# yang-song/score_sde_pytorch

Hardware: AMD Instinct MI355X
Metric: pc_sampler_images_per_sec (higher is better)
Workload: dtype f32 via 3-way bf16 split, fp32 accumulate (the 1x1 / NIN / Linear GEMMs and the attention forward as exact-fp32 products on the BF16 matrix pipe, fp32 softmax; 3x3 convolutions and the attention backward on the fp32-MFMA kernels); 1 GPU; configs/ve/cifar10_ncsnpp_continuous PC sampler (reverse_diffusion+langevin), batch 256/GPU, N=1000, 32x32; 1 step = 1 PC iteration = 2 U-Net evaluations; batch_per_gpu=256, sde_steps=1000, state_finite=True, matrix_mode=bf16x6, parallelism=replicas x1 (no collectives)

## Files before the change

include/ssde.h:

```cpp
#ifndef SSDE_H_
#define SSDE_H_

#include <stddef.h>
#include <stdint.h>

#ifdef __cplusplus
extern "C" {
#endif

#define SSDE_ABI_VERSION 13

enum {
  SSDE_PRO_NONE = 0,
  SSDE_PRO_GN = 1,
  SSDE_PRO_GN_SILU = 2,
  SSDE_PRO_SILU = 3
};

typedef struct ssde_src {
  const float* p0;
  const float* p1;
  int32_t c0, c1;
  int32_t pro_mode;
  int32_t gn_groups;
// ... 38 lines not shown
  int64_t wino_ws_floats;
} ssde_conv_args;

enum { SSDE_CONVF_V_GIVEN = 1u,
       SSDE_CONVF_BF16X6 = 2u,
       SSDE_CONVF_NO_KSPLIT = 4u,
       SSDE_CONVF_BKC8 = 8u,
       SSDE_CONVF_GEMM_PIPE = 16u,
       SSDE_CONVF_NO_GEMM_PIPE = 32u,
       SSDE_CONVF_X6_BM64 = 64u,
       SSDE_CONVF_X6_PF2 = 128u,
       SSDE_CONVF_NO_SMALL_COUT = 256u,
       SSDE_CONVF_X6_WIDE = 512u,
       SSDE_CONVF_X6_NO_WIDE = 1024u,
       SSDE_CONVF_KSPLIT2 = 2048u,
       SSDE_CONVF_KSPLIT4 = 4096u };
enum { SSDE_TILE_AUTO = 0, SSDE_TILE_256x64 = 1, SSDE_TILE_128x64 = 2, SSDE_TILE_64x64 = 3, SSDE_TILE_256x32 = 4,
       SSDE_TILE_WINOGRAD = 5,
       SSDE_TILE_WINOGRAD4 = 6,
       SSDE_TILE_WINOGRAD4R = 9,
       SSDE_TILE_WINOGRAD4P = 10 };

typedef struct ssde_gn_stats_args {
  const float* p0; const float* p1; int32_t c0, c1;
  int32_t n, hw, groups; float eps;
  float* mean; float* rstd;
  float* scratch;
  int32_t slices;
  uint32_t flags;
} ssde_gn_stats_args;
enum { SSDE_GNSTATF_ANY_WIDTH = 1u };

typedef struct ssde_gn_apply_args {
  ssde_src src;
  int32_t n, hw;
  float* dst;
} ssde_gn_apply_args;

typedef struct ssde_gn_apply_bwd_args {
  ssde_src src;
  const float* dy;
  int32_t n, hw;
  float* sums;
  float* dgamma; float* dbeta;
  float* scratch;
  int32_t slices; int32_t _pad0;
  float* g0; float* g1;
  int32_t acc0, acc1;
} ssde_gn_apply_bwd_args;

typedef struct ssde_gn_finalize_args {
  const float* part0; const float* part1;
  int32_t c0, c1, slices0, slices1;
  int32_t n, groups; float eps; int32_t _pad0;
  float* mean; float* rstd;
} ssde_gn_finalize_args;

#define SSDE_FIR_MAX_TAPS 16
enum {
  SSDE_FIRF_GENERAL = 1,
  SSDE_FIRF_TILED = 2
};
typedef struct ssde_upfirdn_args {
  ssde_src src;
  int32_t n, h_in, w_in, c;
  int32_t h_out, w_out;
  int32_t up, down, pad0, pad1;
  int32_t kh, kw;
  float k[16];
  float* dst;
  int32_t accumulate;
  uint32_t flags;
  float* dst2;
  const float* taps;
} ssde_upfirdn_args;

#define SSDE_ATTN_L_MAX 16384
typedef struct ssde_attn_args {
  const float* qkv; float* dst;
  int32_t n, l, c; float scale;
  uint32_t flags;
  int32_t _pad0;
} ssde_attn_args;
enum { SSDE_ATTNF_BF16X6 = 1u,
       SSDE_ATTNF_STREAM = 2u };
enum { SSDE_ATTN_ROUTE_F32 = 0, SSDE_ATTN_ROUTE_X6 = 1, SSDE_ATTN_ROUTE_STREAM = 2 };

typedef struct ssde_embed_args {
  const float* cond;
  const float* w;
  float* dst;
  int32_t n, dim, kind, _pad0;
} ssde_embed_args;

typedef struct ssde_to_nhwc_args {
  const float* src; float* dst; int32_t n, c, h, w, c_pad; float a, b;
  int32_t mode;
  const float* v;
} ssde_to_nhwc_args;
typedef struct ssde_to_nchw_args {
  const float* src; float* dst; int32_t n, c, h, w, c_src;
  int32_t mode;
  const float* v;
  float alpha;
  int32_t accumulate;
} ssde_to_nchw_args;

typedef struct ssde_bias_act_args {
  const float* src; const float* bias; float* dst;
  int64_t numel; int32_t channels; int32_t inner;
  int32_t act;
  float alpha, scale;
  int32_t grad;
  const float* ref;
} ssde_bias_act_args;

typedef struct ssde_sumsq_args {
  const float* a; const float* b; float* out_a; float* out_b; int32_t n, per;
} ssde_sumsq_args;
typedef struct ssde_randn_args {
  float* dst; int64_t numel; uint64_t seed; const int32_t* step_ptr; int32_t stream_id; int32_t _pad0;
  const uint64_t* seed_ptr;
} ssde_randn_args;
typedef struct ssde_langevin_args {
  float* x; float* x_mean; const float* grad; const float* noise;
  const float* grad_sumsq; const float* noise_sumsq;
  const float* alpha_tab; const int32_t* step_ptr;
  int32_t n, per; float snr; int32_t _pad0;
} ssde_langevin_args;
typedef struct ssde_predictor_args {
  float* x; float* x_mean; const float* score; const float* noise;
  const float* coef; const int32_t* step_ptr;
  int64_t numel;
} ssde_predictor_args;
typedef struct ssde_sample_update_args {
  const float* x; const float* y; const float* z; const float* a; const float* b; const float* c;
  float* x_mean; float* x_out; int32_t n; int32_t per;
} ssde_sample_update_args;
typedef struct ssde_fill_args {
  float* dst; const float* tab; const int32_t* step_ptr; int32_t n; int32_t _pad0;
} ssde_fill_args;
typedef struct ssde_step_inc_args { int32_t* step_ptr; int32_t delta; int32_t _pad0; } ssde_step_inc_args;
typedef struct ssde_project_args {
  float* x; float* x_mean; const float* data; const float* mask; const float* noise;
  const float* coef; const int32_t* step_ptr;
  int32_t n, c, hw;
  int32_t use_matrix;
  float M[9], invM[9];
} ssde_project_args;



typedef struct ssde_wgrad_args {
  ssde_src src;
  const float* g;
  int32_t g_ld, g_off;
  int32_t n, h_in, w_in, h_out, w_out;
  int32_t c_out;
  int32_t ksize;
  int32_t stride, pad;
  int32_t cin_store;
  int32_t transpose_out;
  int32_t splits;
  float scale;
  uint32_t flags;
  float* dw;
// ... 24 lines not shown
  uint32_t flags;
  int32_t _pad0;
} ssde_colsum_args;
enum { SSDE_COLSUMF_DEFER = 1u };

#define SSDE_FINISH_JOBS 16
typedef struct ssde_colsum_job {
  const float* part;
  float* per_sample;
  float* total; float* total2;
  int32_t n, slices, c, ps_ld, ps_off, _pad0;
} ssde_colsum_job;
typedef struct ssde_colsum_finish_args { int32_t count, _pad0; ssde_colsum_job job[SSDE_FINISH_JOBS]; } ssde_colsum_finish_args;
typedef struct ssde_gn_bwd_job {
  const float* scratch;
  float* dgamma; float* dbeta;
  int32_t rows, c;
} ssde_gn_bwd_job;
typedef struct ssde_gn_bwd_finish_args { int32_t count, _pad0; ssde_gn_bwd_job job[SSDE_FINISH_JOBS]; } ssde_gn_bwd_finish_args;

typedef struct ssde_gn_bwd_reduce_args {
  ssde_src src;
  const float* dp;
  int32_t n, hw;
  float* sums;
  float* dgamma; float* dbeta;
  float* scratch;
  int32_t slices;
  uint32_t flags;
  float* g0; float* g1;
  int32_t acc0, acc1;
  float scale; int32_t _pad1;
} ssde_gn_bwd_reduce_args;

enum { SSDE_GNBWDF_THREE_KERNELS = 1u,
       SSDE_GNBWDF_DEFER_PARAMS = 2u };

typedef struct ssde_prologue_bwd_args {
  ssde_src src;
  const float* dp;
  int32_t dp_ld, dp_off;
  int32_t n, hw;
  const float* sums;
  float scale;
  int32_t acc0, acc1;
  float* g0; float* g1;
} ssde_prologue_bwd_args;

typedef struct ssde_attn_bwd_args {
  const float* qkv;
  const float* o;
  const float* d_o;
  float* dqkv;
  float* stats;
  int32_t n, l, c; float scale;
} ssde_attn_bwd_args;

typedef struct ssde_perturb_args {
  const float* x; const float* z; const float* a; const float* s; float* dst; int32_t n, per;
} ssde_perturb_args;
typedef struct ssde_dsm_loss_args {
  const float* score; const float* z; const float* s; const float* g2;
  float* dscore;
  float* losses;
  float* loss;
  int32_t n, per; int32_t reduce_mean; int32_t likelihood_weighting;
  float grad_scale;
  int32_t _pad0;
} ssde_dsm_loss_args;

typedef struct ssde_sumsq_flat_args { const float* x; int64_t numel; float* partial; float* out; } ssde_sumsq_flat_args;
typedef struct ssde_adam_args {
  float* p; const float* g; float* m; float* v; float* ema;
  int64_t numel;
  const float* hyper;
  const float* gnorm_sq;
} ssde_adam_args;

typedef struct ssde_memset_args { void* dst; int64_t bytes; int32_t value; int32_t _pad0; } ssde_memset_args;

enum { SSDE_PACK_CONV3 = 1, SSDE_PACK_WINO3 = 2, SSDE_PACK_MATRIX = 3, SSDE_PACK_VECTOR = 4,
       SSDE_PACK_WINO4 = 5 ,
       SSDE_PACK_WINO4R = 6 ,
       SSDE_PACK_WINO4P = 7  };
typedef struct ssde_pack_desc {
  const float* src;
  const float* src2;
  float* dst;
  int32_t kind;
  int32_t cout, cin;
  int32_t cout_l, cin_l;
  int32_t flags;
  int32_t r_off, c_off;
  int64_t n;
} ssde_pack_desc;
typedef struct ssde_pack_args { const ssde_pack_desc* table; int32_t count; int32_t kind; int64_t max_n; } ssde_pack_args;
typedef struct ssde_axpy_args {
  const float* x; const float* gate; float* dst; int64_t numel; float alpha; int32_t acc;
} ssde_axpy_args;

typedef struct ssde_rk_coefs { double v[7]; } ssde_rk_coefs;
typedef struct ssde_rk_combine_args {
  const double* y; const double* k; int64_t n; int32_t terms; int32_t _pad0; ssde_rk_coefs coef; double* dst; float* dst32;
  int64_t n32;
} ssde_rk_combine_args;
typedef struct ssde_rk_error_args {
  const double* y; const double* y_new; const double* k; int64_t n; ssde_rk_coefs coef; double atol, rtol;
  double* partial; int32_t partial_len; int32_t _pad0; double* out;
} ssde_rk_error_args;
#define SSDE_RK_MAX_TERMS 12
#define SSDE_RK_MAX_ROWS 13
typedef struct ssde_rk_combine_rows_args {
  const double* y; const double* k; int64_t n; int32_t terms; int32_t _pad0; double coef[SSDE_RK_MAX_TERMS]; double* dst; float* dst32;
  int64_t n32;
} ssde_rk_combine_rows_args;
typedef struct ssde_rk_error_rows_args {
  const double* y; const double* y_new; const double* k; int64_t n; int32_t rows; int32_t pair;
  double coef[SSDE_RK_MAX_ROWS]; double coef2[SSDE_RK_MAX_ROWS]; double h_abs; double atol, rtol;
  double* partial; int32_t partial_len; int32_t _pad0; double* out;
} ssde_rk_error_rows_args;
typedef struct ssde_ode_dyn {
  float label, std;
  float a, g2;
  double* dst;
} ssde_ode_dyn;
typedef struct ssde_pf_drift_args {
  const float* x; const float* score; double* dst; int64_t numel; float a, g2;
  const ssde_ode_dyn* dyn;
} ssde_pf_drift_args;
typedef struct ssde_hutch_div_args {
  const float* gx; const float* eps; double* dst; int64_t dst_off; int32_t n; int32_t per; float a, g2;
  const ssde_ode_dyn* dyn;
} ssde_hutch_div_args;

int ssde_conv2d(const ssde_conv_args* a, void* stream);
int ssde_groupnorm_stats(const ssde_gn_stats_args* a, void* stream);
int ssde_gn_finalize(const ssde_gn_finalize_args* a, void* stream);
int ssde_gn_apply(const ssde_gn_apply_args* a, void* stream);
int ssde_gn_apply_bwd(const ssde_gn_apply_bwd_args* a, void* stream);
int ssde_conv_gn_slices(const ssde_conv_args* a);
int64_t ssde_conv_ws_floats(const ssde_conv_args* a);
int ssde_upfirdn2d(const ssde_upfirdn_args* a, void* stream);
int ssde_attention(const ssde_attn_args* a, void* stream);
int ssde_attention_route(const ssde_attn_args* a);
int ssde_embed(const ssde_embed_args* a, void* stream);
int ssde_to_nhwc(const ssde_to_nhwc_args* a, void* stream);
int ssde_to_nchw(const ssde_to_nchw_args* a, void* stream);
int ssde_fused_bias_act(const ssde_bias_act_args* a, void* stream);
int ssde_sumsq(const ssde_sumsq_args* a, void* stream);
int ssde_randn(const ssde_randn_args* a, void* stream);
int ssde_langevin_update(const ssde_langevin_args* a, void* stream);
int ssde_predictor_update(const ssde_predictor_args* a, void* stream);
int ssde_sample_update(const ssde_sample_update_args* a, void* stream);
int ssde_fill_from_table(const ssde_fill_args* a, void* stream);
int ssde_step_inc(const ssde_step_inc_args* a, void* stream);
int ssde_project_update(const ssde_project_args* a, void* stream);
int ssde_rk_combine(const ssde_rk_combine_args* a, void* stream);
int ssde_rk_error_norm(const ssde_rk_error_args* a, void* stream);
int ssde_rk_combine_rows(const ssde_rk_combine_rows_args* a, void* stream);
int ssde_rk_error_norm_rows(const ssde_rk_error_rows_args* a, void* stream);
int ssde_pf_drift(const ssde_pf_drift_args* a, void* stream);
int ssde_hutch_div(const ssde_hutch_div_args* a, void* stream);
int ssde_conv_wgrad(const ssde_wgrad_args* a, void* stream);
int ssde_wgrad_wants_winograd4(const ssde_wgrad_args* a);
int ssde_colsum(const ssde_colsum_args* a, void* stream);
int ssde_colsum_finish(const ssde_colsum_finish_args* a, void* stream);
int ssde_gn_bwd_finish(const ssde_gn_bwd_finish_args* a, void* stream);
int ssde_gn_bwd_scratch_rows(const ssde_gn_bwd_reduce_args* a);
int ssde_gn_bwd_reduce(const ssde_gn_bwd_reduce_args* a, void* stream);
int ssde_prologue_bwd(const ssde_prologue_bwd_args* a, void* stream);
int ssde_attention_bwd(const ssde_attn_bwd_args* a, void* stream);
int ssde_perturb(const ssde_perturb_args* a, void* stream);
int ssde_dsm_loss(const ssde_dsm_loss_args* a, void* stream);
int ssde_sumsq_flat(const ssde_sumsq_flat_args* a, void* stream);
int ssde_adam_clip_ema(const ssde_adam_args* a, void* stream);
int ssde_memset(const ssde_memset_args* a, void* stream);
int ssde_axpy(const ssde_axpy_args* a, void* stream);
int ssde_pack_weights(const ssde_pack_args* a, void* stream);

enum {
  SSDE_OP_CONV = 1, SSDE_OP_GN_STATS = 2, SSDE_OP_UPFIRDN = 3, SSDE_OP_ATTN = 4, SSDE_OP_EMBED = 5,
  SSDE_OP_TO_NHWC = 6, SSDE_OP_TO_NCHW = 7, SSDE_OP_BIAS_ACT = 8, SSDE_OP_SUMSQ = 9, SSDE_OP_RANDN = 10,
  SSDE_OP_LANGEVIN = 11, SSDE_OP_PREDICTOR = 12, SSDE_OP_FILL = 13, SSDE_OP_STEP_INC = 14,
  SSDE_OP_WGRAD = 15, SSDE_OP_COLSUM = 16, SSDE_OP_GN_BWD_REDUCE = 17, SSDE_OP_PROLOGUE_BWD = 18,
  SSDE_OP_ATTN_BWD = 19, SSDE_OP_PERTURB = 20, SSDE_OP_DSM_LOSS = 21, SSDE_OP_SUMSQ_FLAT = 22,
  SSDE_OP_ADAM = 23, SSDE_OP_MEMSET = 24, SSDE_OP_AXPY = 25, SSDE_OP_PACK = 26, SSDE_OP_PROJECT = 27,
  SSDE_OP_GN_FINALIZE = 28, SSDE_OP_PF_DRIFT = 29, SSDE_OP_HUTCH_DIV = 30, SSDE_OP_COLSUM_FINISH = 31, SSDE_OP_GN_BWD_FINISH = 32,
  SSDE_OP_GN_APPLY = 33, SSDE_OP_GN_APPLY_BWD = 34
};
typedef struct ssde_op {
  int32_t kind; int32_t flops_class;
  union {
    ssde_conv_args conv; ssde_gn_stats_args gn; ssde_upfirdn_args fir; ssde_attn_args attn;
    ssde_embed_args embed; ssde_to_nhwc_args to_nhwc; ssde_to_nchw_args to_nchw;
    ssde_bias_act_args bias_act; ssde_sumsq_args sumsq; ssde_randn_args randn;
    ssde_langevin_args langevin; ssde_predictor_args predictor; ssde_fill_args fill;
    ssde_step_inc_args step_inc;
    ssde_wgrad_args wgrad; ssde_colsum_args colsum; ssde_gn_bwd_reduce_args gn_bwd; ssde_prologue_bwd_args pro_bwd;
    ssde_attn_bwd_args attn_bwd; ssde_perturb_args perturb; ssde_dsm_loss_args dsm_loss;
    ssde_sumsq_flat_args sumsq_flat; ssde_adam_args adam; ssde_memset_args memset; ssde_axpy_args axpy;
    ssde_pack_args pack; ssde_project_args project; ssde_gn_finalize_args gn_fin;
    ssde_pf_drift_args pf_drift; ssde_hutch_div_args hutch_div;
    ssde_colsum_finish_args colsum_fin; ssde_gn_bwd_finish_args gn_bwd_fin;
    ssde_gn_apply_args gn_apply; ssde_gn_apply_bwd_args gn_apply_bwd;
  } u;
} ssde_op;

int ssde_program_run(const ssde_op* ops, int32_t n_ops, void* stream);
int ssde_program_run_timed(const ssde_op* ops, int32_t n_ops, void* stream, float* ms);
int ssde_graph_capture(const ssde_op* ops, int32_t n_ops, void* stream, void** graph_out);
int ssde_graph_launch(void* graph, void* stream);
int ssde_graph_destroy(void* graph);

enum { SSDE_REGION_ZERO = 0,
       SSDE_REGION_CONST = 1 };
enum { SSDE_RELOC_OP = 0, SSDE_RELOC_REFRESH_OP = 1, SSDE_RELOC_REGION = 2 };
enum { SSDE_PLAN_UNET = 0, SSDE_PLAN_PC = 1, SSDE_PLAN_TRAIN = 2,
       SSDE_PLAN_ODE = 3,
       SSDE_PLAN_LIKELIHOOD = 4 };
enum { SSDE_IO_X = 0, SSDE_IO_COND = 1, SSDE_IO_SIGMA = 2, SSDE_IO_STD = 3, SSDE_IO_OUT = 4, SSDE_IO_XMEAN = 5,
       SSDE_IO_STEP = 6, SSDE_IO_SEED = 7,
       SSDE_IO_BATCH = 8, SSDE_IO_Z = 9, SSDE_IO_A = 10, SSDE_IO_S = 11, SSDE_IO_G2 = 12, SSDE_IO_LOSS = 13, SSDE_IO_HYPER = 14,
       SSDE_IO_DROP_SEED = 15, SSDE_IO_GOUT = 16, SSDE_IO_GX = 17, SSDE_IO_GRAD = 18, SSDE_IO_PARAMS = 19,
       SSDE_IO_ODE_DYN = 20, SSDE_IO_ODE_K = 21, SSDE_IO_ODE_STATE = 22, SSDE_IO_ODE_PROBE = 23, SSDE_IO_SLOTS = 24 };
#define SSDE_ODE_PARTIALS 1024
typedef struct ssde_plan_header {
  char magic[8];
  int32_t abi_version, sizeof_op;
  int32_t n_regions, n_ops, n_refresh_ops, n_relocs, n_params;
  int32_t kind;
  int32_t batch, channels, height, width;
  int32_t nfe_per_iteration;
  int32_t sde_steps;
  int32_t io[SSDE_IO_SLOTS];
  int32_t seg[4];
  int64_t n_flat;
  int64_t data_bytes;
} ssde_plan_header;
typedef struct ssde_plan_region { int64_t bytes; int64_t data_offset; int32_t kind; int32_t _pad0; char name[32]; } ssde_plan_region;
typedef struct ssde_plan_reloc {
  int32_t target_kind;
  int32_t target;
  int64_t byte_offset;
  int32_t region; int32_t _pad0;
  int64_t offset;
} ssde_plan_reloc;
typedef struct ssde_plan_param_entry { char name[96]; int32_t region; int32_t _pad0; int64_t offset; int64_t numel; } ssde_plan_param_entry;
typedef struct ssde_plan ssde_plan;

int ssde_plan_load(const void* blob, size_t bytes, ssde_plan** out);
int ssde_plan_load_file(const char* path, ssde_plan** out);
int ssde_plan_destroy(ssde_plan* p);
int ssde_plan_info(const ssde_plan* p, ssde_plan_header* out);
int ssde_plan_param(const ssde_plan* p, const char* name, int32_t index, float** dev, int64_t* numel, const char** name_out);
int ssde_plan_refresh_weights(ssde_plan* p, void* stream);
int ssde_unet_forward(ssde_plan* p, const float* x, const float* cond, const float* sigma, const float* std_, float* out, void* stream);
int ssde_pc_reset(ssde_plan* p, const float* x_T, uint64_t seed, void* stream);
int ssde_pc_run(ssde_plan* p, int32_t n_iterations, int32_t use_graph, void* stream);
int ssde_train_step(ssde_plan* p, const float* batch, const float* z, const float* a, const float* s, const float* labels,
                    const float* g2, const float* hyper, uint32_t dropout_seed, float* loss_out, void* stream);
int ssde_train_forward(ssde_plan* p, const float* x, const float* cond, const float* sigma, const float* std_, uint32_t dropout_seed,
                       float* out, void* stream);
int ssde_unet_backward(ssde_plan* p, const float* dout, float* dx, float* dparams, void* stream);
int ssde_plan_copy_io(ssde_plan* p, int32_t slot, void* buf, int64_t bytes, int32_t to_plan, void* stream);
int ssde_pc_state(ssde_plan* p, float* x, float* x_mean, void* stream);
enum { SSDE_ODE_RK45 = 0, SSDE_ODE_RK23 = 1, SSDE_ODE_DOP853 = 2 };
typedef int (*ssde_ode_scalars_fn)(double t, void* user, float out[4]);
int ssde_ode_reset(ssde_plan* p, const float* x0, const float* probe, void* stream);
int ssde_ode_eval(ssde_plan* p, double t, ssde_ode_scalars_fn scalars, void* user, double* slope, void* stream);
int ssde_ode_solve(ssde_plan* p, double t0, double t1, double rtol, double atol, ssde_ode_scalars_fn scalars, void* user,
                   int32_t use_graph, int32_t max_nfev, int32_t* nfev, void* stream);
int ssde_ode_solve_method(ssde_plan* p, int32_t method, double t0, double t1, double rtol, double atol, ssde_ode_scalars_fn scalars,
                          void* user, int32_t use_graph, int32_t max_nfev, int32_t* nfev, void* stream);
int ssde_ode_state(ssde_plan* p, float* x, double* delta_logp, void* stream);

int ssde_abi_version(void);
int ssde_sizeof_op(void);
const char* ssde_last_error(void);
int ssde_conv_lds_bytes(const ssde_conv_args* a);
int64_t ssde_wgrad_scratch_floats(const ssde_wgrad_args* a);
int ssde_mfma_probe(int32_t workgroups, int32_t iters, float* sink, void* stream);

#ifdef __cplusplus
}
#endif
#endif
```

score_sde_pytorch_amd/_lib.py:

```python
import ctypes as C
import os

_HERE = os.path.dirname(os.path.abspath(__file__))
LIB_PATH = os.environ.get("SSDE_LIB_PATH") or os.path.join(_HERE, "libssde_hip.so")
ABI_VERSION = 13

PRO_NONE, PRO_GN, PRO_GN_SILU, PRO_SILU = 0, 1, 2, 3
TILE_AUTO, TILE_256x64, TILE_128x64, TILE_64x64, TILE_256x32, TILE_WINOGRAD, TILE_WINOGRAD4 = 0, 1, 2, 3, 4, 5, 6
TILE_WINOGRAD4R = 9
TILE_WINOGRAD4P = 10
TILES_WINOGRAD4 = (TILE_WINOGRAD4, TILE_WINOGRAD4R, TILE_WINOGRAD4P)
CONVF_V_GIVEN, CONVF_BF16X6, CONVF_NO_KSPLIT, CONVF_BKC8, CONVF_GEMM_PIPE, CONVF_NO_GEMM_PIPE, CONVF_X6_BM64, CONVF_X6_PF2, \
    CONVF_NO_SMALL_COUT, CONVF_X6_WIDE, CONVF_X6_NO_WIDE, CONVF_KSPLIT2, CONVF_KSPLIT4 = 1, 2, 4, 8, 16, 32, 64, 128, 256, 512, 1024, 2048, 4096
WGRADF_DIRECT, WGRADF_F2, WGRADF_F4_FORCE, WGRADF_NO_STREAMK, WGRADF_NO_XCD_ORDER, WGRADF_1X1_CHUNKED, WGRADF_XVEC1 = 1, 2, 4, 8, 16, 32, 64
GNBWDF_THREE_KERNELS, GNBWDF_DEFER_PARAMS = 1, 2
(OP_CONV, OP_GN_STATS, OP_UPFIRDN, OP_ATTN, OP_EMBED, OP_TO_NHWC, OP_TO_NCHW, OP_BIAS_ACT, OP_SUMSQ,
 OP_RANDN, OP_LANGEVIN, OP_PREDICTOR, OP_FILL, OP_STEP_INC, OP_WGRAD, OP_COLSUM, OP_GN_BWD_REDUCE, OP_PROLOGUE_BWD,
 OP_ATTN_BWD, OP_PERTURB, OP_DSM_LOSS, OP_SUMSQ_FLAT, OP_ADAM, OP_MEMSET, OP_AXPY, OP_PACK, OP_PROJECT,
 OP_GN_FINALIZE, OP_PF_DRIFT, OP_HUTCH_DIV, OP_COLSUM_FINISH, OP_GN_BWD_FINISH, OP_GN_APPLY, OP_GN_APPLY_BWD) = range(1, 35)
GNSTATF_ANY_WIDTH = 1
FIRF_GENERAL, FIRF_TILED = 1, 2
FIR_MAX_TAPS = 16
FINISH_JOBS = 16
COLSUMF_DEFER = 1
PACK_CONV3, PACK_WINO3, PACK_MATRIX, PACK_VECTOR, PACK_WINO4, PACK_WINO4R, PACK_WINO4P = 1, 2, 3, 4, 5, 6, 7

_fp = C.c_void_p


class Src(C.Structure):
    _fields_ = [("p0", _fp), ("p1", _fp), ("c0", C.c_int32), ("c1", C.c_int32),
                ("pro_mode", C.c_int32), ("gn_groups", C.c_int32),
                ("gn_mean", _fp), ("gn_rstd", _fp), ("gn_gamma", _fp), ("gn_beta", _fp),
                ("drop_thresh", C.c_uint32), ("drop_scale", C.c_float), ("drop_seed", _fp),
                ("drop_salt", C.c_uint32), ("_pad", C.c_int32)]


class ConvArgs(C.Structure):
    _fields_ = [("main", Src), ("aux", Src), ("w_main", _fp), ("w_aux", _fp),
                ("n", C.c_int32), ("h_in", C.c_int32), ("w_in", C.c_int32),
                ("h_out", C.c_int32), ("w_out", C.c_int32), ("c_out", C.c_int32),
                ("ksize", C.c_int32), ("stride", C.c_int32), ("pad", C.c_int32), ("tile", C.c_int32),
                ("bias", _fp), ("chan_add", _fp), ("chan_add_ld", C.c_int32), ("resid_post", C.c_int32),
                ("resid", _fp), ("out_scale", C.c_float), ("flags", C.c_uint32), ("dst", _fp), ("gn_part", _fp), ("wino_v", _fp),
                ("gn_in_part0", _fp), ("gn_in_part1", _fp), ("gn_in_slices0", C.c_int32), ("gn_in_slices1", C.c_int32),
                ("gn_in_eps", C.c_float), ("pad_end", C.c_int32), ("wino_ws", _fp), ("wino_ws_floats", C.c_int64)]


class GnStatsArgs(C.Structure):
    _fields_ = [("p0", _fp), ("p1", _fp), ("c0", C.c_int32), ("c1", C.c_int32),
                ("n", C.c_int32), ("hw", C.c_int32), ("groups", C.c_int32), ("eps", C.c_float),
                ("mean", _fp), ("rstd", _fp), ("scratch", _fp), ("slices", C.c_int32), ("flags", C.c_uint32)]


class GnApplyArgs(C.Structure):
    _fields_ = [("src", Src), ("n", C.c_int32), ("hw", C.c_int32), ("dst", _fp)]


class GnApplyBwdArgs(C.Structure):
    _fields_ = [("src", Src), ("dy", _fp), ("n", C.c_int32), ("hw", C.c_int32), ("sums", _fp), ("dgamma", _fp), ("dbeta", _fp),
                ("scratch", _fp), ("slices", C.c_int32), ("_pad0", C.c_int32), ("g0", _fp), ("g1", _fp),
                ("acc0", C.c_int32), ("acc1", C.c_int32)]


class RkCombineArgs(C.Structure):
    _fields_ = [("y", _fp), ("k", _fp), ("n", C.c_int64), ("terms", C.c_int32), ("_pad0", C.c_int32), ("coef", C.c_double * 7),
                ("dst", _fp), ("dst32", _fp), ("n32", C.c_int64)]


class RkErrorArgs(C.Structure):
    _fields_ = [("y", _fp), ("y_new", _fp), ("k", _fp), ("n", C.c_int64), ("coef", C.c_double * 7), ("atol", C.c_double),
                ("rtol", C.c_double), ("partial", _fp), ("partial_len", C.c_int32), ("_pad0", C.c_int32), ("out", _fp)]


class RkCombineRowsArgs(C.Structure):
    _fields_ = [("y", _fp), ("k", _fp), ("n", C.c_int64), ("terms", C.c_int32), ("_pad0", C.c_int32), ("coef", C.c_double * 12),
                ("dst", _fp), ("dst32", _fp), ("n32", C.c_int64)]


class RkErrorRowsArgs(C.Structure):
    _fields_ = [("y", _fp), ("y_new", _fp), ("k", _fp), ("n", C.c_int64), ("rows", C.c_int32), ("pair", C.c_int32),
                ("coef", C.c_double * 13), ("coef2", C.c_double * 13), ("h_abs", C.c_double), ("atol", C.c_double), ("rtol", C.c_double),
                ("partial", _fp), ("partial_len", C.c_int32), ("_pad0", C.c_int32), ("out", _fp)]


class PfDriftArgs(C.Structure):
    _fields_ = [("x", _fp), ("score", _fp), ("dst", _fp), ("numel", C.c_int64), ("a", C.c_float), ("g2", C.c_float), ("dyn", _fp)]


class OdeDyn(C.Structure):
    _fields_ = [("label", C.c_float), ("std", C.c_float), ("a", C.c_float), ("g2", C.c_float), ("dst", _fp)]


class HutchDivArgs(C.Structure):
    _fields_ = [("gx", _fp), ("eps", _fp), ("dst", _fp), ("dst_off", C.c_int64), ("n", C.c_int32), ("per", C.c_int32),
                ("a", C.c_float), ("g2", C.c_float), ("dyn", _fp)]


class GnFinalizeArgs(C.Structure):
    _fields_ = [("part0", _fp), ("part1", _fp), ("c0", C.c_int32), ("c1", C.c_int32), ("slices0", C.c_int32), ("slices1", C.c_int32),
                ("n", C.c_int32), ("groups", C.c_int32), ("eps", C.c_float), ("_pad0", C.c_int32), ("mean", _fp), ("rstd", _fp)]


class UpfirdnArgs(C.Structure):
    _fields_ = [("src", Src), ("n", C.c_int32), ("h_in", C.c_int32), ("w_in", C.c_int32), ("c", C.c_int32),
                ("h_out", C.c_int32), ("w_out", C.c_int32),
                ("up", C.c_int32), ("down", C.c_int32), ("pad0", C.c_int32), ("pad1", C.c_int32),
                ("kh", C.c_int32), ("kw", C.c_int32), ("k", C.c_float * 16), ("dst", _fp),
                ("accumulate", C.c_int32), ("flags", C.c_uint32), ("dst2", _fp), ("taps", _fp)]


class AttnArgs(C.Structure):
    _fields_ = [("qkv", _fp), ("dst", _fp), ("n", C.c_int32), ("l", C.c_int32), ("c", C.c_int32), ("scale", C.c_float),
                ("flags", C.c_uint32), ("_pad0", C.c_int32)]


class EmbedArgs(C.Structure):
    _fields_ = [("cond", _fp), ("w", _fp), ("dst", _fp), ("n", C.c_int32), ("dim", C.c_int32),
                ("kind", C.c_int32), ("_pad0", C.c_int32)]


class ToNhwcArgs(C.Structure):
    _fields_ = [("src", _fp), ("dst", _fp), ("n", C.c_int32), ("c", C.c_int32), ("h", C.c_int32), ("w", C.c_int32),
                ("c_pad", C.c_int32), ("a", C.c_float), ("b", C.c_float), ("mode", C.c_int32), ("v", _fp)]


class ToNchwArgs(C.Structure):
    _fields_ = [("src", _fp), ("dst", _fp), ("n", C.c_int32), ("c", C.c_int32), ("h", C.c_int32), ("w", C.c_int32),
                ("c_src", C.c_int32), ("mode", C.c_int32), ("v", _fp), ("alpha", C.c_float), ("accumulate", C.c_int32)]


class BiasActArgs(C.Structure):
    _fields_ = [("src", _fp), ("bias", _fp), ("dst", _fp), ("numel", C.c_int64), ("channels", C.c_int32),
                ("inner", C.c_int32), ("act", C.c_int32), ("alpha", C.c_float), ("scale", C.c_float), ("grad", C.c_int32),
                ("ref", _fp)]


class SumsqArgs(C.Structure):
    _fields_ = [("a", _fp), ("b", _fp), ("out_a", _fp), ("out_b", _fp), ("n", C.c_int32), ("per", C.c_int32)]


class RandnArgs(C.Structure):
    _fields_ = [("dst", _fp), ("numel", C.c_int64), ("seed", C.c_uint64), ("step_ptr", _fp),
                ("stream_id", C.c_int32), ("_pad0", C.c_int32), ("seed_ptr", _fp)]


class LangevinArgs(C.Structure):
    _fields_ = [("x", _fp), ("x_mean", _fp), ("grad", _fp), ("noise", _fp), ("grad_sumsq", _fp), ("noise_sumsq", _fp),
                ("alpha_tab", _fp), ("step_ptr", _fp), ("n", C.c_int32), ("per", C.c_int32), ("snr", C.c_float),
                ("_pad0", C.c_int32)]


class PredictorArgs(C.Structure):
    _fields_ = [("x", _fp), ("x_mean", _fp), ("score", _fp), ("noise", _fp), ("coef", _fp), ("step_ptr", _fp),
                ("numel", C.c_int64)]


class SampleUpdateArgs(C.Structure):
    _fields_ = [("x", _fp), ("y", _fp), ("z", _fp), ("a", _fp), ("b", _fp), ("c", _fp), ("x_mean", _fp), ("x_out", _fp),
                ("n", C.c_int32), ("per", C.c_int32)]


class FillArgs(C.Structure):
    _fields_ = [("dst", _fp), ("tab", _fp), ("step_ptr", _fp), ("n", C.c_int32), ("_pad0", C.c_int32)]


class StepIncArgs(C.Structure):
    _fields_ = [("step_ptr", _fp), ("delta", C.c_int32), ("_pad0", C.c_int32)]


class ProjectArgs(C.Structure):
    _fields_ = [("x", _fp), ("x_mean", _fp), ("data", _fp), ("mask", _fp), ("noise", _fp), ("coef", _fp), ("step_ptr", _fp),
                ("n", C.c_int32), ("c", C.c_int32), ("hw", C.c_int32), ("use_matrix", C.c_int32),
                ("M", C.c_float * 9), ("invM", C.c_float * 9)]


class WgradArgs(C.Structure):
    _fields_ = [("src", Src), ("g", _fp), ("g_ld", C.c_int32), ("g_off", C.c_int32),
                ("n", C.c_int32), ("h_in", C.c_int32), ("w_in", C.c_int32), ("h_out", C.c_int32), ("w_out", C.c_int32),
                ("c_out", C.c_int32), ("ksize", C.c_int32), ("stride", C.c_int32), ("pad", C.c_int32),
                ("cin_store", C.c_int32), ("transpose_out", C.c_int32), ("splits", C.c_int32), ("scale", C.c_float),
                ("flags", C.c_uint32), ("dw", _fp), ("scratch", _fp), ("scratch_floats", C.c_int64), ("v_pre", _fp),
                ("pad_end", C.c_int32), ("_pad0", C.c_int32)]


class ColsumArgs(C.Structure):
    _fields_ = [("g", _fp), ("g_ld", C.c_int32), ("g_off", C.c_int32), ("n", C.c_int32), ("hw", C.c_int32),
                ("c", C.c_int32), ("scale", C.c_float), ("per_sample", _fp), ("ps_ld", C.c_int32), ("ps_off", C.c_int32),
                ("total", _fp), ("total2", _fp), ("scratch", _fp), ("flags", C.c_uint32), ("_pad0", C.c_int32)]


class ColsumJob(C.Structure):
    _fields_ = [("part", _fp), ("per_sample", _fp), ("total", _fp), ("total2", _fp), ("n", C.c_int32), ("slices", C.c_int32),
                ("c", C.c_int32), ("ps_ld", C.c_int32), ("ps_off", C.c_int32), ("_pad0", C.c_int32)]


class ColsumFinishArgs(C.Structure):
# ... 12 lines not shown
    _fields_ = [("src", Src), ("dp", _fp), ("n", C.c_int32), ("hw", C.c_int32), ("sums", _fp),
                ("dgamma", _fp), ("dbeta", _fp), ("scratch", _fp), ("slices", C.c_int32), ("flags", C.c_uint32),
                ("g0", _fp), ("g1", _fp), ("acc0", C.c_int32), ("acc1", C.c_int32), ("scale", C.c_float), ("_pad1", C.c_int32)]


class PrologueBwdArgs(C.Structure):
    _fields_ = [("src", Src), ("dp", _fp), ("dp_ld", C.c_int32), ("dp_off", C.c_int32), ("n", C.c_int32), ("hw", C.c_int32),
                ("sums", _fp), ("scale", C.c_float), ("acc0", C.c_int32), ("acc1", C.c_int32), ("g0", _fp), ("g1", _fp)]


class AttnBwdArgs(C.Structure):
    _fields_ = [("qkv", _fp), ("o", _fp), ("d_o", _fp), ("dqkv", _fp), ("stats", _fp),
                ("n", C.c_int32), ("l", C.c_int32), ("c", C.c_int32), ("scale", C.c_float)]


class PerturbArgs(C.Structure):
    _fields_ = [("x", _fp), ("z", _fp), ("a", _fp), ("s", _fp), ("dst", _fp), ("n", C.c_int32), ("per", C.c_int32)]


class DsmLossArgs(C.Structure):
    _fields_ = [("score", _fp), ("z", _fp), ("s", _fp), ("g2", _fp), ("dscore", _fp), ("losses", _fp), ("loss", _fp),
                ("n", C.c_int32), ("per", C.c_int32), ("reduce_mean", C.c_int32), ("likelihood_weighting", C.c_int32),
                ("grad_scale", C.c_float), ("_pad0", C.c_int32)]


class SumsqFlatArgs(C.Structure):
    _fields_ = [("x", _fp), ("numel", C.c_int64), ("partial", _fp), ("out", _fp)]


class AdamArgs(C.Structure):
    _fields_ = [("p", _fp), ("g", _fp), ("m", _fp), ("v", _fp), ("ema", _fp), ("numel", C.c_int64),
                ("hyper", _fp), ("gnorm_sq", _fp)]


class MemsetArgs(C.Structure):
    _fields_ = [("dst", _fp), ("bytes", C.c_int64), ("value", C.c_int32), ("_pad0", C.c_int32)]


class AxpyArgs(C.Structure):
    _fields_ = [("x", _fp), ("gate", _fp), ("dst", _fp), ("numel", C.c_int64), ("alpha", C.c_float), ("acc", C.c_int32)]


class PackDesc(C.Structure):
    _fields_ = [("src", _fp), ("src2", _fp), ("dst", _fp), ("kind", C.c_int32), ("cout", C.c_int32), ("cin", C.c_int32),
                ("cout_l", C.c_int32), ("cin_l", C.c_int32), ("flags", C.c_int32), ("r_off", C.c_int32), ("c_off", C.c_int32),
                ("n", C.c_int64)]


class PackArgs(C.Structure):
    _fields_ = [("table", _fp), ("count", C.c_int32), ("kind", C.c_int32), ("max_n", C.c_int64)]


OPS = [(OP_CONV, "conv", ConvArgs, "ssde_conv2d"), (OP_GN_STATS, "gn", GnStatsArgs, "ssde_groupnorm_stats"),
       (OP_UPFIRDN, "fir", UpfirdnArgs, "ssde_upfirdn2d"), (OP_ATTN, "attn", AttnArgs, "ssde_attention"),
       (OP_EMBED, "embed", EmbedArgs, "ssde_embed"), (OP_TO_NHWC, "to_nhwc", ToNhwcArgs, "ssde_to_nhwc"),
       (OP_TO_NCHW, "to_nchw", ToNchwArgs, "ssde_to_nchw"), (OP_BIAS_ACT, "bias_act", BiasActArgs, "ssde_fused_bias_act"),
       (OP_SUMSQ, "sumsq", SumsqArgs, "ssde_sumsq"), (OP_RANDN, "randn", RandnArgs, "ssde_randn"),
       (OP_LANGEVIN, "langevin", LangevinArgs, "ssde_langevin_update"),
       (OP_PREDICTOR, "predictor", PredictorArgs, "ssde_predictor_update"), (OP_FILL, "fill", FillArgs, "ssde_fill_from_table"),
       (OP_STEP_INC, "step_inc", StepIncArgs, "ssde_step_inc"), (OP_WGRAD, "wgrad", WgradArgs, "ssde_conv_wgrad"),
       (OP_COLSUM, "colsum", ColsumArgs, "ssde_colsum"), (OP_GN_BWD_REDUCE, "gn_bwd", GnBwdReduceArgs, "ssde_gn_bwd_reduce"),
       (OP_PROLOGUE_BWD, "pro_bwd", PrologueBwdArgs, "ssde_prologue_bwd"), (OP_ATTN_BWD, "attn_bwd", AttnBwdArgs, "ssde_attention_bwd"),
       (OP_PERTURB, "perturb", PerturbArgs, "ssde_perturb"), (OP_DSM_LOSS, "dsm_loss", DsmLossArgs, "ssde_dsm_loss"),
       (OP_SUMSQ_FLAT, "sumsq_flat", SumsqFlatArgs, "ssde_sumsq_flat"), (OP_ADAM, "adam", AdamArgs, "ssde_adam_clip_ema"),
       (OP_MEMSET, "memset", MemsetArgs, "ssde_memset"), (OP_AXPY, "axpy", AxpyArgs, "ssde_axpy"),
       (OP_PACK, "pack", PackArgs, "ssde_pack_weights"), (OP_PROJECT, "project", ProjectArgs, "ssde_project_update"),
       (OP_GN_FINALIZE, "gn_fin", GnFinalizeArgs, "ssde_gn_finalize"), (OP_PF_DRIFT, "pf_drift", PfDriftArgs, "ssde_pf_drift"),
       (OP_HUTCH_DIV, "hutch_div", HutchDivArgs, "ssde_hutch_div"), (OP_COLSUM_FINISH, "colsum_fin", ColsumFinishArgs, "ssde_colsum_finish"),
       (OP_GN_BWD_FINISH, "gn_bwd_fin", GnBwdFinishArgs, "ssde_gn_bwd_finish"), (OP_GN_APPLY, "gn_apply", GnApplyArgs, "ssde_gn_apply"),
       (OP_GN_APPLY_BWD, "gn_apply_bwd", GnApplyBwdArgs, "ssde_gn_apply_bwd")]


class _OpUnion(C.Union):
    _fields_ = [(member, args) for _, member, args, _ in OPS]


class Op(C.Structure):
    _fields_ = [("kind", C.c_int32), ("flops_class", C.c_int32), ("u", _OpUnion)]


_UNION_FIELD = {kind: member for kind, member, _, _ in OPS}
ARGS = {kind: args for kind, _, args, _ in OPS}

EXPORTS = ["ssde_conv2d", "ssde_groupnorm_stats", "ssde_upfirdn2d", "ssde_attention", "ssde_attention_route", "ssde_embed", "ssde_to_nhwc",
           "ssde_to_nchw", "ssde_fused_bias_act", "ssde_sumsq", "ssde_randn", "ssde_langevin_update",
           "ssde_predictor_update", "ssde_fill_from_table", "ssde_step_inc", "ssde_program_run",
           "ssde_program_run_timed", "ssde_graph_capture", "ssde_graph_launch", "ssde_graph_destroy",
           "ssde_abi_version", "ssde_sizeof_op", "ssde_last_error", "ssde_conv_lds_bytes",
           "ssde_conv_wgrad", "ssde_colsum", "ssde_gn_bwd_reduce", "ssde_prologue_bwd", "ssde_attention_bwd",
           "ssde_perturb", "ssde_dsm_loss", "ssde_sumsq_flat", "ssde_adam_clip_ema", "ssde_memset", "ssde_axpy",
           "ssde_wgrad_scratch_floats", "ssde_wgrad_wants_winograd4", "ssde_pack_weights", "ssde_project_update", "ssde_gn_finalize", "ssde_conv_gn_slices", "ssde_conv_ws_floats", "ssde_rk_combine", "ssde_rk_error_norm", "ssde_rk_combine_rows", "ssde_rk_error_norm_rows", "ssde_pf_drift", "ssde_hutch_div", "ssde_sample_update", "ssde_mfma_probe", "ssde_colsum_finish", "ssde_gn_bwd_finish", "ssde_gn_bwd_scratch_rows",
           "ssde_gn_apply", "ssde_gn_apply_bwd",
           "ssde_plan_load", "ssde_plan_load_file", "ssde_plan_destroy", "ssde_plan_info", "ssde_plan_param",
           "ssde_plan_refresh_weights", "ssde_unet_forward", "ssde_pc_reset", "ssde_pc_run", "ssde_pc_state",
           "ssde_train_step", "ssde_train_forward", "ssde_unet_backward", "ssde_plan_copy_io",
           "ssde_ode_reset", "ssde_ode_eval", "ssde_ode_solve", "ssde_ode_solve_method", "ssde_ode_state"]

_lib = None


def conv_route_flags(env=None):
    e = os.environ if env is None else env
    f = 0
    if e.get("SSDE_MATRIX", "").startswith("b"):
        f |= CONVF_BF16X6
    if e.get("SSDE_CONV_KSPLIT", "1") == "0":
        f |= CONVF_NO_KSPLIT
    if e.get("SSDE_CONV_BKC64", "") == "8":
        f |= CONVF_BKC8
    if e.get("SSDE_GEMM_PIPE", "") == "0":
        f |= CONVF_NO_GEMM_PIPE
    if e.get("SSDE_GEMM_PIPE", "") == "2":
        f |= CONVF_GEMM_PIPE
    if e.get("SSDE_X6_BM", "") == "64":
        f |= CONVF_X6_BM64
    if e.get("SSDE_X6_PF", "") == "2":
        f |= CONVF_X6_PF2
    if e.get("SSDE_CONV_SMALL", "1") == "0":
        f |= CONVF_NO_SMALL_COUT
    if e.get("SSDE_X6_WIDE", "") == "1":
        f |= CONVF_X6_WIDE
    if e.get("SSDE_X6_WIDE", "") == "0":
        f |= CONVF_X6_NO_WIDE
    return f


ATTNF_BF16X6, ATTNF_STREAM = 1, 2
ATTN_ROUTE_F32, ATTN_ROUTE_X6, ATTN_ROUTE_STREAM = 0, 1, 2
ATTN_L_MAX = 16384


def attn_route_flags(env=None):
    e = os.environ if env is None else env
    x6 = ATTNF_BF16X6 if e.get("SSDE_MATRIX", "").startswith("b") and e.get("SSDE_ATTN_X6", "1") != "0" else 0
    return x6 | (ATTNF_STREAM if e.get("SSDE_ATTN_STREAM", "0") == "1" else 0)


def wgrad_route_flags(env=None):
    e = os.environ if env is None else env
    f = {"0": WGRADF_DIRECT, "2": WGRADF_F2, "44": WGRADF_F4_FORCE}.get(e.get("SSDE_WGRAD_WINOGRAD", ""), 0)
    if e.get("SSDE_WGRAD4_STREAMK", "1") == "0":
        f |= WGRADF_NO_STREAMK
    if e.get("SSDE_WGRAD4_XCD", "1") == "0":
        f |= WGRADF_NO_XCD_ORDER
    if e.get("SSDE_WGRAD_1X1_PIPELINED", "1") == "0":
        f |= WGRADF_1X1_CHUNKED
    if e.get("SSDE_WGRAD4_XVEC", "2") == "1":
        f |= WGRADF_XVEC1
    return f


def gn_bwd_route_flags(env=None):
    e = os.environ if env is None else env
    return GNBWDF_THREE_KERNELS if e.get("SSDE_GN_BWD_FUSED", "1") == "0" else 0


class SsdeError(RuntimeError):
    pass


def bind(lib):
    for name in EXPORTS:
        if not hasattr(lib, name):
            raise SsdeError("libssde_hip.so does not export %s" % name)
    lib.ssde_last_error.restype = C.c_char_p
    lib.ssde_program_run.argtypes = [C.POINTER(Op), C.c_int32, C.c_void_p]
    lib.ssde_program_run_timed.argtypes = [C.POINTER(Op), C.c_int32, C.c_void_p, C.POINTER(C.c_float)]
    lib.ssde_graph_capture.argtypes = [C.POINTER(Op), C.c_int32, C.c_void_p, C.POINTER(C.c_void_p)]
    lib.ssde_graph_launch.argtypes = [C.c_void_p, C.c_void_p]
    lib.ssde_graph_destroy.argtypes = [C.c_void_p]
    for _, _, typ, name in OPS:
        if name is not None:
            getattr(lib, name).argtypes = [C.POINTER(typ), C.c_void_p]
    lib.ssde_rk_combine.argtypes = [C.POINTER(RkCombineArgs), C.c_void_p]
    lib.ssde_rk_error_norm.argtypes = [C.POINTER(RkErrorArgs), C.c_void_p]
    lib.ssde_rk_combine_rows.argtypes = [C.POINTER(RkCombineRowsArgs), C.c_void_p]
    lib.ssde_rk_error_norm_rows.argtypes = [C.POINTER(RkErrorRowsArgs), C.c_void_p]
    lib.ssde_sample_update.argtypes = [C.POINTER(SampleUpdateArgs), C.c_void_p]
    lib.ssde_conv_lds_bytes.argtypes = [C.POINTER(ConvArgs)]
    lib.ssde_attention_route.argtypes = [C.POINTER(AttnArgs)]
    lib.ssde_conv_gn_slices.argtypes = [C.POINTER(ConvArgs)]
    lib.ssde_conv_ws_floats.argtypes = [C.POINTER(ConvArgs)]
    lib.ssde_conv_ws_floats.restype = C.c_int64
    lib.ssde_wgrad_scratch_floats.argtypes = [C.POINTER(WgradArgs)]
    lib.ssde_wgrad_scratch_floats.restype = C.c_int64
    lib.ssde_wgrad_wants_winograd4.argtypes = [C.POINTER(WgradArgs)]
    lib.ssde_gn_bwd_scratch_rows.argtypes = [C.POINTER(GnBwdReduceArgs)]
    if lib.ssde_abi_version() != ABI_VERSION:
        raise SsdeError("ABI mismatch: library %d, binding %d" % (lib.ssde_abi_version(), ABI_VERSION))
    if lib.ssde_sizeof_op() != C.sizeof(Op):
        raise SsdeError("struct layout mismatch: sizeof(ssde_op) library %d, ctypes %d" % (lib.ssde_sizeof_op(), C.sizeof(Op)))
    return lib


def load():
    global _lib
    if _lib is not None:
        return _lib
    if not os.path.exists(LIB_PATH):
        raise SsdeError(
            "libssde_hip.so not found at %s -- build it with `python -c 'import __graft_entry__ as g; g.build()'` "
            "(score_sde_pytorch_amd has no CPU/eager fallback)" % LIB_PATH)
    lib = bind(C.CDLL(LIB_PATH))
    _lib = lib
    return lib


def check(rc, what=""):
    if rc != 0:
        msg = load().ssde_last_error()
        raise SsdeError("%s failed (%d): %s" % (what or "libssde_hip call", rc, msg.decode() if msg else "?"))


def pointer_offsets(struct_cls, base=0):
    out = []
    for name, typ in struct_cls._fields_:
        off = base + getattr(struct_cls, name).offset
        if typ is C.c_void_p:
            out.append(off)
        elif isinstance(typ, type) and issubclass(typ, C.Structure):
            out.extend(pointer_offsets(typ, off))
        elif isinstance(typ, type) and issubclass(typ, C.Array) and issubclass(typ._type_, C.Structure):
            for i in range(typ._length_):
                out.extend(pointer_offsets(typ._type_, off + i * C.sizeof(typ._type_)))
    return out


_OP_PTRS = {}


def _op_pointer_offsets(kind):
    if kind not in _OP_PTRS:
        _OP_PTRS[kind] = pointer_offsets(ARGS[kind], Op.u.offset)
    return _OP_PTRS[kind]


def pointers_at(raw, offsets, base=0):
    for off in offsets:
        addr = int.from_bytes(raw[base + off:base + off + 8], "little")
        if addr:
            yield base + off, addr


def op_pointers(op):
    return pointers_at(bytes(op), _op_pointer_offsets(int(op.kind)))


def make_op(kind, args, flops_class=0):
    op = Op()
    op.kind = kind
    op.flops_class = flops_class
    setattr(op.u, _UNION_FIELD[kind], args)
    return op


def make(kind, **fields):
    args = ARGS[kind]()
    for k, v in fields.items():
        if isinstance(v, (list, tuple)):
            v = (C.c_float * len(v))(*v)
        setattr(args, k, v.data_ptr() if hasattr(v, "data_ptr") else v)
    return make_op(kind, args)

# ... 7 lines not shown
```

score_sde_pytorch_amd/csrc/attention.hip:

```cpp
#include "ssde_common.h"
#include <type_traits>

typedef float f32x16 __attribute__((ext_vector_type(16)));

namespace {

constexpr int kQB = 64;
constexpr int kLMax = 256;
constexpr int kKB = kLMax;
constexpr int kLDC = 36;
constexpr int kLDP = 260;
constexpr int kTileFloats = kQB * kLDP;
constexpr int kStageFloats = (kQB + kLMax) * kLDC;
constexpr int kFwdVch = 8;
constexpr int kAttnLdsFloats = kQB * kLDP + kFwdVch * kLDP;
constexpr int kBwdLdsFloats = kTileFloats + kStageFloats + 3 * kLMax;

__device__ __forceinline__ void zero_acc(f32x16 (&acc)[2][2]) {
#pragma unroll
  for (int a = 0; a < 2; ++a)
#pragma unroll
    for (int b = 0; b < 2; ++b)
#pragma unroll
      for (int r = 0; r < 16; ++r) acc[a][b][r] = 0.f;
// ... 131 lines not shown
}

__device__ __forceinline__ void store_acc(const f32x16 (&acc)[2][2], float* __restrict__ out, size_t ldo, int out_valid, int cp, int C,
                                          float mul) {
  const int wave = threadIdx.x >> 6, lane = threadIdx.x & 63;
  const int li = lane & 31, lh = lane >> 5;
#pragma unroll
  for (int a = 0; a < 2; ++a)
#pragma unroll
    for (int b = 0; b < 2; ++b) {
      const int col = acc_col(cp + wave * 64, b, li);
      if (col >= C) continue;
#pragma unroll
      for (int r = 0; r < 16; ++r) {
        const int row = acc_row(a, r, lh);
        if (row < out_valid) out[(size_t)row * ldo + col] = acc[a][b][r] * mul;
      }
    }
}

template <int VCH = 32>
__device__ __forceinline__ void gemm_pv(const float* Ps, int Lp, const float* __restrict__ Bm, int b_valid, size_t ldb, int C,
                                        float* Vs, float* __restrict__ out, size_t ldo, int out_valid, float out_scale) {
  f32x16 acc[2][2];
  for (int cp = 0; cp < C; cp += 256) {
    zero_acc(acc);
    pv_pass<VCH>(Ps, Lp, Bm, b_valid, ldb, cp, min(256, C - cp), Vs, acc);
    store_acc(acc, out, ldo, out_valid, cp, C, out_scale);
  }
}

__device__ __forceinline__ void acc_to_tile(const f32x16 (&acc)[2][2], float* Ps, int Lk, float mul) {
  const int wave = threadIdx.x >> 6, lane = threadIdx.x & 63;
  const int li = lane & 31, lh = lane >> 5, kb = wave * 64;
  if (kb < Lk) {
#pragma unroll
    for (int a = 0; a < 2; ++a)
#pragma unroll
      for (int b = 0; b < 2; ++b)
#pragma unroll
        for (int r = 0; r < 16; ++r) {
          const int row = acc_row(a, r, lh), col = acc_col(kb, b, li);
          Ps[row * kLDP + col] = acc[a][b][r] * mul;
        }
  }
}

template <bool kWriteP>
__device__ __forceinline__ float online_softmax(float* Ps, int Lb, float& m_run, float& l_run) {
  const int tid = threadIdx.x;
  const int row = tid >> 2, sub = tid & 3;
  float* prow = Ps + row * kLDP;
  float m = -INFINITY;
  for (int j = sub; j < Lb; j += 4) m = fmaxf(m, prow[j]);
  m = fmaxf(m, __shfl_xor(m, 1, 64));
  m = fmaxf(m, __shfl_xor(m, 2, 64));
  m = fmaxf(m, m_run);
  const float alpha = __expf(m_run - m);
  float sum = 0.f;
  for (int j = sub; j < Lb; j += 4) {
    const float e = __expf(prow[j] - m);
    if (kWriteP) prow[j] = e;
    sum += e;
  }
  sum += __shfl_xor(sum, 1, 64);
  sum += __shfl_xor(sum, 2, 64);
  if (kWriteP) {
    const int Lp = (Lb + 31) & ~31;
    for (int j = Lb + sub; j < Lp; j += 4) prow[j] = 0.f;
  }
  l_run = l_run * alpha + sum;
  m_run = m;
  return alpha;
}

__device__ __forceinline__ void softmax_rows(float* Ps, int L, float& m, float& l) {
  m = -INFINITY; l = 0.f;
  online_softmax<true>(Ps, L, m, l);
  float* prow = Ps + (threadIdx.x >> 2) * kLDP;
  const float inv = 1.0f / l;
  for (int j = threadIdx.x & 3; j < L; j += 4) prow[j] *= inv;
}

__global__ __launch_bounds__(256) void attn_kernel(const float* __restrict__ qkv, float* __restrict__ dst,
                                                   int N, int L, int C, float scale) {
  SSDE_LDS(smem);
  float* Qs = smem;
  float* Ks = smem + kQB * kLDC;
  float* Ps = smem;
  float* Vs = smem + kQB * kLDP;
  const int n = blockIdx.y, q0 = blockIdx.x * kQB;
  const int C3 = 3 * C;
  const float* base = qkv + (size_t)n * L * C3;
  const int Lk = (L + 63) & ~63;
  const int Lp = (L + 31) & ~31;

  f32x16 acc[2][2];
  gemm_nt(base + (size_t)q0 * C3, L - q0, C3, base + C, L, C3, C, Lk, Qs, Ks, acc);
  __syncthreads();
  acc_to_tile(acc, Ps, Lk, scale);
  __syncthreads();
  float m, l;
  softmax_rows(Ps, L, m, l);
  gemm_pv<kFwdVch>(Ps, Lp, base + 2 * C, L, C3, C, Vs, dst + ((size_t)n * L + q0) * C, C, L - q0, 1.0f);
}

namespace x6 {
constexpr int kT = 512, kRows = 64, kL = 256;
constexpr int kKStage = 3 * kL * 32;
constexpr int kPPlane = kL * kRows * 2;
constexpr int kMain = 3 * kPPlane;
constexpr int kLds = kMain + 2 * kKStage;
static_assert(kRows * kLDP * 4 <= kMain, "score tile");

__device__ __forceinline__ void split_hi(float x, uint32_t& a, uint32_t& b, uint32_t& c) {
  a = __builtin_bit_cast(uint32_t, x);
  const float r = x - __builtin_bit_cast(float, a & 0xffff0000u);
  b = __builtin_bit_cast(uint32_t, r);
  c = __builtin_bit_cast(uint32_t, r - __builtin_bit_cast(float, b & 0xffff0000u));
}
}

template <int kNst>
__global__ __launch_bounds__(x6::kT) void attn_x6_kernel(const float* __restrict__ qkv, float* __restrict__ dst, int N, float scale) {
  using namespace x6;
  constexpr int C = 16 * kNst;
  SSDE_LDS(smem);
  char* lds = reinterpret_cast<char*>(smem);
  char* stage0 = lds + kMain;
  char* stage1 = stage0 + kKStage;
  const int tid = threadIdx.x, lane = tid & 63;
  const int wave = __builtin_amdgcn_readfirstlane(tid >> 6);
  const int li = lane & 31, lh = lane >> 5;
  const int xcd = blockIdx.x & 7, k_in = blockIdx.x >> 3;
  const int n = (k_in >> 2) * 8 + xcd, q0 = (k_in & 3) * kRows;
  if (n >= N) return;
  const int C3 = 3 * C;
  const float* base = qkv + (size_t)n * kL * C3;
  const int qplane = C * kRows * 2;
  constexpr int nst = kNst;

  const bool consumer = wave < 4;
  f32x16 acc[2][2];
  auto zero = [&]() {
#pragma unroll
    for (int a = 0; a < 2; ++a)
#pragma unroll
      for (int b = 0; b < 2; ++b)
#pragma unroll
        for (int r = 0; r < 16; ++r) acc[a][b][r] = 0.f;
  };
  struct Frags { ssde_u32x4 A[2][3], B[2][3]; };
  auto read_frags = [&](Frags& f, const char* ap, int a_pitch, const char* bp, int b_pitch) __attribute__((always_inline)) {
#pragma unroll
    for (int q = 0; q < 3; ++q) {
#pragma unroll
      for (int a = 0; a < 2; ++a) f.A[a][q] = *reinterpret_cast<const ssde_u32x4*>(ap + q * a_pitch + (a * 32 + li) * 32 + lh * 16);
#pragma unroll
      for (int b = 0; b < 2; ++b) f.B[b][q] = *reinterpret_cast<const ssde_u32x4*>(bp + q * b_pitch + (wave * 64 + b * 32 + li) * 32 + lh * 16);
    }
  };
  auto mfmas = [&](auto Terms, const Frags& f) __attribute__((always_inline)) {
    constexpr int kTerms = decltype(Terms)::value;
    constexpr int TI[8] = {1, 2, 0, 2, 1, 0, 1, 0}, TJ[8] = {2, 1, 2, 0, 1, 1, 0, 0};
#pragma unroll
    for (int t = 8 - kTerms; t < 8; ++t)
#pragma unroll
      for (int a = 0; a < 2; ++a)
#pragma unroll
        for (int b = 0; b < 2; ++b)
          acc[a][b] = __builtin_amdgcn_mfma_f32_32x32x16_bf16(__builtin_bit_cast(ssde_bf16x8, f.A[a][TI[t]]),
                                                              __builtin_bit_cast(ssde_bf16x8, f.B[b][TJ[t]]), acc[a][b], 0, 0, 0);
  };
  using Six = std::integral_constant<int, 6>;
  using Eight = std::integral_constant<int, 8>;

  const int ptid = tid & 255;
  const float* kbase = base + C;
  const float* vbase = base + 2 * C;
  const int krow = ptid >> 2, kf = ptid & 3;
  const uint32_t koff = (uint32_t)((krow * C3 + kf * 4) * 4), kstep = (uint32_t)(64 * C3 * 4);
  const int tp = ptid & 7, fq0 = ptid >> 3;
  const bool v_on0 = fq0 * 4 < C, v_on1 = (fq0 + 32) * 4 < C;
  const uint32_t voff = (uint32_t)((2 * tp * C3 + (v_on0 ? fq0 * 4 : 0)) * 4), vtok = (uint32_t)(C3 * 4), vquad = v_on1 ? 512u : 0u;
  const int vpitch = C * 32;
  auto request = [&](int u, ssde_f32x4 (&Rs)[4]) __attribute__((always_inline)) {
    const bool is_k = u < nst;
    const float* sb = is_k ? kbase + u * 16 : vbase + (size_t)(u - nst) * 16 * C3;
    const uint32_t o0 = is_k ? koff : voff;
    const uint32_t o1 = o0 + (is_k ? kstep : vtok);
    const uint32_t o2 = is_k ? o0 + 2 * kstep : o0 + vquad;
    const uint32_t o3 = is_k ? o0 + 3 * kstep : o2 + vtok;
    SSDE_GLOAD16_I_SAFE(Rs[0], o0, sb, 0);
    SSDE_GLOAD16_I_SAFE(Rs[1], o1, sb, 0);
    SSDE_GLOAD16_I_SAFE(Rs[2], o2, sb, 0);
    SSDE_GLOAD16_I_SAFE(Rs[3], o3, sb, 0);
  };
#ifdef SSDE_EMULATED
#define SSDE_X6_WAIT(n, Rs) ((void)0)
#else
#define SSDE_X6_WAIT(n, Rs) asm volatile("s_waitcnt vmcnt(%4)" : "+v"((Rs)[0]), "+v"((Rs)[1]), "+v"((Rs)[2]), "+v"((Rs)[3]) : "n"(n) : "memory")
#endif
  auto park_k = [&](const ssde_f32x4 (&Rs)[4], char* buf) __attribute__((always_inline)) {
#pragma unroll
    for (int i = 0; i < 4; ++i) {
      uint2 p0, p1, p2;
      ssde_split3(make_float4(Rs[i].x, Rs[i].y, Rs[i].z, Rs[i].w), p0, p1, p2);
// ... 68 lines not shown
  if (consumer) {
    SSDE_LDS_BARRIER();
    for (int u = 0; u < nst; ++u) {
      Frags f;
      read_frags(f, lds + u * (kRows * 32), qplane, (u & 1) ? stage1 : stage0, kL * 32);
      mfmas(Eight{}, f);
      SSDE_LDS_BARRIER();
    }
  } else {
    SSDE_X6_WAIT(12, R[0]);
    park_k(R[0], stage0);
    SSDE_LDS_BARRIER();
#pragma unroll
    for (int u = 0; u < nst; ++u) {
      const int j = u & 3;
      request(u + 4, R[j]);
      SSDE_X6_WAIT(12, R[(j + 1) & 3]);
      if (u + 1 < nst) park_k(R[(j + 1) & 3], (j & 1) ? stage0 : stage1);
      SSDE_LDS_BARRIER();
    }
    SSDE_X6_WAIT(8, R[1]); SSDE_X6_WAIT(4, R[2]); SSDE_X6_WAIT(0, R[3]);
  }

  {
    float* tile = smem;
    if (consumer) {
#pragma unroll
      for (int a = 0; a < 2; ++a)
#pragma unroll
        for (int b = 0; b < 2; ++b)
#pragma unroll
          for (int r = 0; r < 16; ++r) {
            const int row = a * 32 + (r & 3) + 8 * (r >> 2) + 4 * lh;
            tile[row * kLDP + wave * 64 + b * 32 + li] = acc[a][b][r] * scale;
          }
    }
    SSDE_LDS_BARRIER();
    const int row = tid >> 3, sub = tid & 7;
    float x[32];
#pragma unroll
    for (int i = 0; i < 8; ++i) {
      const float4 v = *reinterpret_cast<const float4*>(tile + row * kLDP + sub * 32 + i * 4);
      x[4 * i] = v.x; x[4 * i + 1] = v.y; x[4 * i + 2] = v.z; x[4 * i + 3] = v.w;
    }
    SSDE_LDS_BARRIER();
    float m = x[0];
#pragma unroll
    for (int i = 1; i < 32; ++i) m = fmaxf(m, x[i]);
    m = fmaxf(m, __shfl_xor(m, 1, 64));
    m = fmaxf(m, __shfl_xor(m, 2, 64));
    m = fmaxf(m, __shfl_xor(m, 4, 64));
    float sum = 0.f;
#pragma unroll
    for (int i = 0; i < 32; ++i) { x[i] = __expf(x[i] - m); sum += x[i]; }
    sum += __shfl_xor(sum, 1, 64);
    sum += __shfl_xor(sum, 2, 64);
    sum += __shfl_xor(sum, 4, 64);
    const float inv = 1.0f / sum;
#pragma unroll
    for (int u = 0; u < 4; ++u) {
      uint2 a0, a1, a2, b0, b1, b2;
      ssde_split3(make_float4(x[8 * u] * inv, x[8 * u + 1] * inv, x[8 * u + 2] * inv, x[8 * u + 3] * inv), a0, a1, a2);
      ssde_split3(make_float4(x[8 * u + 4] * inv, x[8 * u + 5] * inv, x[8 * u + 6] * inv, x[8 * u + 7] * inv), b0, b1, b2);
      char* d = lds + (2 * sub + (u >> 1)) * (kRows * 32) + row * 32 + (u & 1) * 16;
      *reinterpret_cast<uint4*>(d) = make_uint4(a0.x, a0.y, b0.x, b0.y);
      *reinterpret_cast<uint4*>(d + kPPlane) = make_uint4(a1.x, a1.y, b1.x, b1.y);
      *reinterpret_cast<uint4*>(d + 2 * kPPlane) = make_uint4(a2.x, a2.y, b2.x, b2.y);
    }
  }

  if (consumer) {
    const bool w_on = wave * 64 < C;
    zero();
    SSDE_LDS_BARRIER();
    for (int v = 0; v < 16; ++v) {
      if (w_on) {
        Frags f;
        read_frags(f, lds + v * (kRows * 32), kPPlane, (v & 1) ? stage1 : stage0, vpitch);
        mfmas(Six{}, f);
      }
      SSDE_LDS_BARRIER();
    }
    if (w_on) {
#pragma unroll
      for (int b = 0; b < 2; ++b) {
        float* out = dst + ((size_t)n * kL + q0) * C + wave * 64 + b * 32 + li;
#pragma unroll
        for (int a = 0; a < 2; ++a)
#pragma unroll
          for (int r = 0; r < 16; ++r) {
            const int row = a * 32 + (r & 3) + 8 * (r >> 2) + 4 * lh;
            out[(size_t)row * C] = acc[a][b][r];
          }
      }
    }
  } else {
    park_v(R[0], stage0);
    SSDE_LDS_BARRIER();
#pragma unroll
    for (int v = 0; v < 16; ++v) {
      const int j = v & 3;
      if (v + 4 < 16) request(nst + v + 4, R[j]);
      if (v + 1 < 16) {
        if (v + 1 >= 4) {
          if (v + 4 < 16) SSDE_X6_WAIT(12, R[(j + 1) & 3]);
          else if (v + 3 < 16) SSDE_X6_WAIT(8, R[(j + 1) & 3]);
          else if (v + 2 < 16) SSDE_X6_WAIT(4, R[(j + 1) & 3]);
          else SSDE_X6_WAIT(0, R[(j + 1) & 3]);
        }
        park_v(R[(j + 1) & 3], (j & 1) ? stage0 : stage1);
      }
      SSDE_LDS_BARRIER();
    }
  }
#undef SSDE_X6_WAIT
}


__device__ __forceinline__ float row_dot(const float* __restrict__ o, const float* __restrict__ d_o, size_t first, int C, int valid) {
  const int row = threadIdx.x >> 2, sub = threadIdx.x & 3;
  float d = 0.f;
  if (row < valid) {
    const float* po = o + (first + row) * C;
    const float* pd = d_o + (first + row) * C;
    for (int c = sub * 4; c < C; c += 16) {
      const float4 a = *reinterpret_cast<const float4*>(po + c);
      const float4 b = *reinterpret_cast<const float4*>(pd + c);
      d += (a.x * b.x + a.y * b.y) + (a.z * b.z + a.w * b.w);
    }
  }
  d += __shfl_xor(d, 1, 64);
  d += __shfl_xor(d, 2, 64);
  return d;
}

__device__ __forceinline__ void load_stats(float* St, const float* __restrict__ stats, size_t first, int count) {
  const int j = threadIdx.x;
  float m = 0.f, l = 1.f, d = 0.f;
  if (j < count) { const float* st = stats + (first + j) * 4; m = st[0]; l = st[1]; d = st[2]; }
  St[j] = m; St[kKB + j] = l; St[2 * kKB + j] = d;
}

template <bool kRowStats>
__device__ __forceinline__ void acc_to_probs(const f32x16 (&acc)[2][2], float* Ps, const float* St, int Lk, int rows_valid, int cols_valid,
                                             float scale) {
  const int wave = threadIdx.x >> 6, lane = threadIdx.x & 63;
  const int li = lane & 31, lh = lane >> 5, kb = wave * 64;
  if (kb < Lk) {
#pragma unroll
    for (int a = 0; a < 2; ++a)
#pragma unroll
      for (int b = 0; b < 2; ++b)
#pragma unroll
        for (int r = 0; r < 16; ++r) {
          const int row = acc_row(a, r, lh), col = acc_col(kb, b, li);
          const int s = kRowStats ? row : col;
          float pv = 0.f;
          if (row < rows_valid && col < cols_valid) pv = __expf(acc[a][b][r] * scale - St[s]) / St[kKB + s];
          Ps[row * kLDP + col] = pv;
        }
  }
}

template <bool kRowStats>
__device__ __forceinline__ void probs_to_ds(const f32x16 (&acc)[2][2], float* Ps, const float* St, int Lk, int Lp) {
  const int wave = threadIdx.x >> 6, lane = threadIdx.x & 63;
  const int li = lane & 31, lh = lane >> 5, kb = wave * 64;
  if (kb < Lk) {
#pragma unroll
    for (int a = 0; a < 2; ++a)
#pragma unroll
      for (int b = 0; b < 2; ++b)
#pragma unroll
        for (int r = 0; r < 16; ++r) {
          const int row = acc_row(a, r, lh), col = acc_col(kb, b, li);
          if (col < Lp) Ps[row * kLDP + col] *= (acc[a][b][r] - St[2 * kKB + (kRowStats ? row : col)]);
        }
  }
}

__global__ __launch_bounds__(256) void attn_bwd_q_kernel(const float* __restrict__ qkv, const float* __restrict__ o,
                                                         const float* __restrict__ d_o, float* __restrict__ dqkv,
                                                         float* __restrict__ stats, int N, int L, int C, float scale) {
  SSDE_LDS(smem);
  float* Ps = smem;
  float* Qs = smem + kTileFloats;
  float* Ks = Qs + kQB * kLDC;
  float* Vs = Qs;
  float* St = smem + kTileFloats + kStageFloats;
  const int n = blockIdx.y, q0 = blockIdx.x * kQB, tid = threadIdx.x;
  const int C3 = 3 * C;
  const float* base = qkv + (size_t)n * L * C3;
  const int Lk = (L + 63) & ~63, Lp = (L + 31) & ~31;
  const int valid = L - q0;

  f32x16 acc[2][2];
  gemm_nt(base + (size_t)q0 * C3, valid, C3, base + C, L, C3, C, Lk, Qs, Ks, acc);
  __syncthreads();
// ... 130 lines not shown
template <int NCP>
__global__ __launch_bounds__(256) void attn_stream_bwd_q_kernel(const float* __restrict__ qkv, const float* __restrict__ d_o,
                                                                float* __restrict__ dqkv, const float* __restrict__ stats,
                                                                int N, int L, int C, float scale) {
  SSDE_LDS(smem);
  float* Ps = smem;
  float* Qs = smem + kTileFloats;
  float* Ks = Qs + kQB * kLDC;
  float* Vs = Qs;
  float* St = smem + kTileFloats + kStageFloats;
  const int n = blockIdx.y, q0 = blockIdx.x * kQB, tid = threadIdx.x;
  const int C3 = 3 * C;
  const float* base = qkv + (size_t)n * L * C3;
  const int valid = L - q0;
  if (tid < kQB) load_stats(St, stats, (size_t)n * L + q0, valid);
  f32x16 dq[NCP][2][2];
#pragma unroll
  for (int p = 0; p < NCP; ++p) zero_acc(dq[p]);
  for (int kb0 = 0; kb0 < L; kb0 += kKB) {
    const int Lb = min(kKB, L - kb0);
    const int Lk = (Lb + 63) & ~63, Lp = (Lb + 31) & ~31;
    f32x16 acc[2][2];
    gemm_nt(base + (size_t)q0 * C3, valid, C3, base + (size_t)kb0 * C3 + C, Lb, C3, C, Lk, Qs, Ks, acc);
    __syncthreads();
    acc_to_probs<true>(acc, Ps, St, Lk, valid, Lb, scale);
    gemm_nt(d_o + ((size_t)n * L + q0) * C, valid, C, base + (size_t)kb0 * C3 + 2 * C, Lb, C3, C, Lk, Qs, Ks, acc);
    __syncthreads();
    probs_to_ds<true>(acc, Ps, St, Lk, Lp);
#pragma unroll
    for (int p = 0; p < NCP; ++p)
      if (p * 256 < C) pv_pass<32>(Ps, Lp, base + (size_t)kb0 * C3 + C, Lb, C3, p * 256, min(256, C - p * 256), Vs, dq[p]);
  }
#pragma unroll
  for (int p = 0; p < NCP; ++p)
    if (p * 256 < C) store_acc(dq[p], dqkv + ((size_t)n * L + q0) * C3, C3, valid, p * 256, C, scale);
}

__global__ __launch_bounds__(256) void attn_stream_bwd_kv_kernel(const float* __restrict__ qkv, const float* __restrict__ d_o,
                                                                 float* __restrict__ dqkv, const float* __restrict__ stats,
                                                                 int N, int L, int C, float scale) {
  SSDE_LDS(smem);
  float* Ps = smem;
  float* Qs = smem + kTileFloats;
  float* Ks = Qs + kQB * kLDC;
  float* Vs = Qs;
  float* St = smem + kTileFloats + kStageFloats;
  const int n = blockIdx.y, k0 = blockIdx.x * kQB;
  const int cp = blockIdx.z * 256, Cw = min(256, C - cp);
  const int C3 = 3 * C;
  const float* base = qkv + (size_t)n * L * C3;
  const float* dob = d_o + (size_t)n * L * C;
  const int valid = L - k0;
  f32x16 dv[2][2], dk[2][2];
  zero_acc(dv);
  zero_acc(dk);
  for (int qb0 = 0; qb0 < L; qb0 += kKB) {
    const int Lb = min(kKB, L - qb0);
    const int Lk = (Lb + 63) & ~63, Lp = (Lb + 31) & ~31;
    __syncthreads();
    load_stats(St, stats, (size_t)n * L + qb0, Lb);
    f32x16 acc[2][2];
    gemm_nt(base + (size_t)k0 * C3 + C, valid, C3, base + (size_t)qb0 * C3, Lb, C3, C, Lk, Qs, Ks, acc);
    __syncthreads();
    acc_to_probs<false>(acc, Ps, St, Lk, valid, Lb, scale);
    pv_pass<32>(Ps, Lp, dob + (size_t)qb0 * C, Lb, C, cp, Cw, Vs, dv);
    gemm_nt(base + (size_t)k0 * C3 + 2 * C, valid, C3, dob + (size_t)qb0 * C, Lb, C, C, Lk, Qs, Ks, acc);
    __syncthreads();
    probs_to_ds<false>(acc, Ps, St, Lk, Lp);
    pv_pass<32>(Ps, Lp, base + (size_t)qb0 * C3, Lb, C3, cp, Cw, Vs, dk);
  }
  float* out = dqkv + ((size_t)n * L + k0) * C3;
  store_acc(dv, out + 2 * C, C3, valid, cp, C, 1.0f);
  store_acc(dk, out + C, C3, valid, cp, C, scale);
}

int check_shape(const char* what, int n, int l, int c) {
  SSDE_REQUIRE(n > 0 && l > 0 && l <= SSDE_ATTN_L_MAX, "%s: token count %d outside 1..%d", what, l, SSDE_ATTN_L_MAX);
  SSDE_REQUIRE(c > 0 && c % 32 == 0, "%s: channels must be a multiple of 32 (got %d)", what, c);
  return SSDE_OK;
}

}

static int attn_route(const ssde_attn_args* a) {
  SSDE_REQUIRE(a, "attention: null args");
  if (int rc = check_shape("attention", a->n, a->l, a->c)) return rc;
  if (a->l > kLMax || (a->flags & SSDE_ATTNF_STREAM)) {
    SSDE_REQUIRE(a->c <= kStreamCMax, "attention: the streaming kernels (more than %d tokens, or SSDE_ATTNF_STREAM) take at most %d channels (got %d)",
                 kLMax, kStreamCMax, a->c);
    return SSDE_ATTN_ROUTE_STREAM;
  }
  if ((a->flags & SSDE_ATTNF_BF16X6) && a->l == x6::kL && a->c <= 256 && a->c % 64 == 0) return SSDE_ATTN_ROUTE_X6;
  return SSDE_ATTN_ROUTE_F32;
}

extern "C" int ssde_attention_route(const ssde_attn_args* a) { return attn_route(a); }

extern "C" int ssde_attention(const ssde_attn_args* a, void* stream) {
  SSDE_REQUIRE(a && a->qkv && a->dst, "attention: null args");
  const int route = attn_route(a);
  if (route < 0) return route;
  hipStream_t st = static_cast<hipStream_t>(stream);
  const dim3 grid(ssde_cdiv(a->l, kQB), a->n);
  if (route == SSDE_ATTN_ROUTE_STREAM) {
    if (a->c <= 256) return ssde_launch_lds<attn_stream_kernel<1>>("attention", grid, 256, kStreamLdsFloats * 4, st, a->qkv, a->dst, a->n, a->l, a->c, a->scale);
    return ssde_launch_lds<attn_stream_kernel<2>>("attention", grid, 256, kStreamLdsFloats * 4, st, a->qkv, a->dst, a->n, a->l, a->c, a->scale);
  }
  if (route == SSDE_ATTN_ROUTE_X6) {
    const dim3 grid_x6(ssde_cdiv(a->n, 8) * 8 * 4);
    switch (a->c) {
      case 64: return ssde_launch_lds<attn_x6_kernel<4>>("attention", grid_x6, x6::kT, x6::kLds, st, a->qkv, a->dst, a->n, a->scale);
      case 128: return ssde_launch_lds<attn_x6_kernel<8>>("attention", grid_x6, x6::kT, x6::kLds, st, a->qkv, a->dst, a->n, a->scale);
      case 192: return ssde_launch_lds<attn_x6_kernel<12>>("attention", grid_x6, x6::kT, x6::kLds, st, a->qkv, a->dst, a->n, a->scale);
      default: return ssde_launch_lds<attn_x6_kernel<16>>("attention", grid_x6, x6::kT, x6::kLds, st, a->qkv, a->dst, a->n, a->scale);
    }
  }
  return ssde_launch_lds<attn_kernel>("attention", grid, 256, kAttnLdsFloats * 4, st, a->qkv, a->dst, a->n, a->l, a->c, a->scale);
}

extern "C" int ssde_attention_bwd(const ssde_attn_bwd_args* a, void* stream) {
  SSDE_REQUIRE(a && a->qkv && a->o && a->d_o && a->dqkv && a->stats, "attention_bwd: null args");
  if (int rc = check_shape("attention_bwd", a->n, a->l, a->c)) return rc;
  hipStream_t st = static_cast<hipStream_t>(stream);
  const dim3 grid(ssde_cdiv(a->l, kQB), a->n);
  const int lds = kBwdLdsFloats * 4;
  if (a->l > kLMax) {
    SSDE_REQUIRE(a->c <= kStreamCMax, "attention_bwd: the streaming kernels (more than %d tokens) take at most %d channels (got %d)", kLMax,
                 kStreamCMax, a->c);
    if (int rc = ssde_launch_lds<attn_stream_stats_kernel>("attention_bwd", grid, 256, kStreamLdsFloats * 4, st, a->qkv, a->o, a->d_o, a->stats, a->n, a->l,
                            a->c, a->scale))
      return rc;
    if (int rc = a->c <= 256 ? ssde_launch_lds<attn_stream_bwd_q_kernel<1>>("attention_bwd", grid, 256, lds, st, a->qkv, a->d_o, a->dqkv, a->stats, a->n, a->l, a->c, a->scale)
                             : ssde_launch_lds<attn_stream_bwd_q_kernel<2>>("attention_bwd", grid, 256, lds, st, a->qkv, a->d_o, a->dqkv, a->stats, a->n, a->l, a->c, a->scale))
      return rc;
    return ssde_launch_lds<attn_stream_bwd_kv_kernel>("attention_bwd", dim3(grid.x, grid.y, ssde_cdiv(a->c, 256)), 256, lds, st, a->qkv, a->d_o, a->dqkv,
                      a->stats, a->n, a->l, a->c, a->scale);
  }
  if (int rc = ssde_launch_lds<attn_bwd_q_kernel>("attention_bwd", grid, 256, lds, st, a->qkv, a->o, a->d_o, a->dqkv, a->stats, a->n, a->l, a->c, a->scale)) return rc;
  return ssde_launch_lds<attn_bwd_kv_kernel>("attention_bwd", grid, 256, lds, st, a->qkv, a->d_o, a->dqkv, a->stats, a->n, a->l, a->c, a->scale);
}
```

score_sde_pytorch_amd/csrc/backward.hip:

```cpp
#include "ssde_common.h"

namespace {

inline unsigned grid_for(size_t total, int block = 256, unsigned cap = 256 * 16) {
  size_t b = (total + block - 1) / block;
  if (b < 1) b = 1;
  return (unsigned)(b > cap ? cap : b);
}

__global__ __launch_bounds__(256) void colsum_kernel(const float* __restrict__ g, int g_ld, int g_off, int hw, int c,
                                                     float scale, float* __restrict__ out, int out_ld, int out_off) {
  SSDE_LDS(smem);
  float4* red = reinterpret_cast<float4*>(smem);
  const int n = blockIdx.z, slices = gridDim.y, slice = blockIdx.y;
  const int cl = blockIdx.x * 64 + (threadIdx.x & 63);
  const int pl = threadIdx.x >> 6;
  const int col = g_off + cl * 4;
  const int per_slice = (hw + slices - 1) / slices;
  const int p0 = slice * per_slice, p1 = min(hw, p0 + per_slice);
  float4 s = make_float4(0.f, 0.f, 0.f, 0.f);
  if (cl * 4 < c && col + 4 <= g_ld) {
    const float* base = g + (size_t)n * hw * g_ld + col;
    int px = p0 + pl;
    for (; px + 12 < p1; px += 16) {
// ... 819 lines not shown
      for (int k = 0; k < 3; ++k)
#pragma unroll
        for (int l = 0; l < 3; ++l) w[k][l] = pack_w3(d, co, ci, k, l);
#pragma unroll
      for (int pa = 0; pa < 4; ++pa)
#pragma unroll
        for (int pb = 0; pb < 4; ++pb) {
          float acc = 0.f;
#pragma unroll
          for (int k = 0; k < 3; ++k) {
            float t = 0.f;
#pragma unroll
            for (int l = 0; l < 3; ++l) t += w[k][l] * G[pb][l];
            acc += G[pa][k] * t;
          }
          u[e][pa * 4 + pb] = acc;
        }
    }
#pragma unroll
    for (int pos = 0; pos < 16; ++pos)
      *reinterpret_cast<float2*>(d.dst + ((((r * 16 + pos) * 4 + q) * 64 + cs) << 1)) = make_float2(u[0][pos], u[1][pos]);
  }
}

template <int kForm>
__global__ __launch_bounds__(256) void pack_wino4_kernel(const ssde_pack_desc* __restrict__ table) {
  const ssde_pack_desc d = table[blockIdx.y];
  const int ntl = (d.cout_l + 63) / 64;
  const size_t nq = (size_t)d.n / ((size_t)36 * ntl * 256);
  const double G[6][3] = {{0.25, 0.0, 0.0}, {-1.0 / 6, -1.0 / 6, -1.0 / 6}, {-1.0 / 6, 1.0 / 6, -1.0 / 6},
                          {1.0 / 24, 1.0 / 12, 1.0 / 6}, {1.0 / 24, -1.0 / 12, 1.0 / 6}, {0.0, 0.0, 1.0}};
  const size_t items = (size_t)d.n / 36;
  for (size_t it = (size_t)blockIdx.x * 256 + threadIdx.x; it < items; it += (size_t)gridDim.x * 256) {
    const int e = (int)(it & 3), cs = (int)((it >> 2) & 63);
    const size_t r = it >> 8;
    const int nt = (int)(r % ntl), c4 = (int)(r / ntl);
    const int co = nt * 64 + cs, ci = c4 * 4 + e;
    double w[3][3], t[6][3];
#pragma unroll
    for (int k = 0; k < 3; ++k)
#pragma unroll
      for (int l = 0; l < 3; ++l) w[k][l] = (double)pack_w3(d, co, ci, k, l);
#pragma unroll
    for (int a = 0; a < 6; ++a)
#pragma unroll
      for (int l = 0; l < 3; ++l) t[a][l] = G[a][0] * w[0][l] + G[a][1] * w[1][l] + G[a][2] * w[2][l];
#pragma unroll
    for (int a = 0; a < 6; ++a)
#pragma unroll
      for (int b = 0; b < 6; ++b)
      {
        const int pos = a * 6 + b, wv = (pos & 3) * 2 + (cs >> 5), j = pos >> 2;
        const float u = (float)(t[a][0] * G[b][0] + t[a][1] * G[b][1] + t[a][2] * G[b][2]);
        if (kForm == 0) {
          d.dst[(((r * 8 + wv) * 9 + j) * 32 + (cs & 31)) * 4 + e] = u;
        } else if (kForm == 2) {
          d.dst[(((size_t)pos * nq + c4) * ((size_t)ntl * 64) + co) * 4 + e] = u;
        } else {
          const int lane = (e >> 1) * 32 + (cs & 31), half = cs >> 5;
          const int w = pos < 32 ? (pos >> 2) : 2 * (pos - 32) + half;
          const size_t base = (r * 8 + w) * (size_t)(9 * 32 * 4);
          d.dst[base + (pos < 32 ? ((pos & 3) * 64 + lane) * 4 + half * 2 + (e & 1) : 1024 + lane * 2 + (e & 1))] = u;
        }
      }
  }
}

__global__ __launch_bounds__(256) void pack_matrix_kernel(const ssde_pack_desc* __restrict__ table) {
  const ssde_pack_desc d = table[blockIdx.y];
  const int ld = (d.cout_l + 63) / 64 * 64;
  for (size_t idx = (size_t)blockIdx.x * 256 + threadIdx.x; idx < (size_t)d.n; idx += (size_t)gridDim.x * 256) {
    const int i = (int)(idx / d.cin), j = (int)(idx % d.cin);
    const int row = ((d.flags & 1) ? j : i) + d.r_off, col = ((d.flags & 1) ? i : j) + d.c_off;
    d.dst[((size_t)(col >> 3) * ld + row) * 8 + (col & 7)] = d.src[idx];
  }
}

__global__ __launch_bounds__(256) void pack_vector_kernel(const ssde_pack_desc* __restrict__ table) {
  const ssde_pack_desc d = table[blockIdx.y];
  for (size_t idx = (size_t)blockIdx.x * 256 + threadIdx.x; idx < (size_t)d.n; idx += (size_t)gridDim.x * 256)
    d.dst[d.r_off + idx] = d.src[idx] + (d.src2 ? d.src2[idx] : 0.f);
}

}

extern "C" int ssde_pack_weights(const ssde_pack_args* a, void* stream) {
  SSDE_REQUIRE(a && a->table && a->count > 0 && a->max_n > 0, "pack_weights: bad args");
  size_t bx = ((size_t)a->max_n + 255) / 256;
  if (bx > 256) bx = 256;
  const dim3 grid((unsigned)bx, (unsigned)a->count);
  hipStream_t st = static_cast<hipStream_t>(stream);
  switch (a->kind) {
    case SSDE_PACK_CONV3: hipLaunchKernelGGL(pack_conv3_kernel, grid, dim3(256), 0, st, a->table); break;
    case SSDE_PACK_WINO3: hipLaunchKernelGGL(pack_wino3_kernel, grid, dim3(256), 0, st, a->table); break;
    case SSDE_PACK_WINO4: hipLaunchKernelGGL(pack_wino4_kernel<0>, grid, dim3(256), 0, st, a->table); break;
    case SSDE_PACK_WINO4R: hipLaunchKernelGGL(pack_wino4_kernel<1>, grid, dim3(256), 0, st, a->table); break;
    case SSDE_PACK_WINO4P: hipLaunchKernelGGL(pack_wino4_kernel<2>, grid, dim3(256), 0, st, a->table); break;
    case SSDE_PACK_MATRIX: hipLaunchKernelGGL(pack_matrix_kernel, grid, dim3(256), 0, st, a->table); break;
    case SSDE_PACK_VECTOR: hipLaunchKernelGGL(pack_vector_kernel, grid, dim3(256), 0, st, a->table); break;
    default: ssde_set_error("pack_weights: unknown kind %d", a->kind); return SSDE_EINVAL;
  }
  SSDE_LAUNCH_CHECK();
  return SSDE_OK;
}
```

score_sde_pytorch_amd/csrc/runtime.hip:

```cpp
#include "ssde_common.h"
#include <string.h>
#include <vector>

static thread_local char g_err[512] = "";

void ssde_set_error(const char* fmt, ...) {
  va_list ap;
  va_start(ap, fmt);
  vsnprintf(g_err, sizeof(g_err), fmt, ap);
  va_end(ap);
}

extern "C" const char* ssde_last_error(void) { return g_err; }

int ssde_num_cus() {
  if (const char* e = getenv("SSDE_NUM_CUS")) { const int v = atoi(e); if (v > 0) return v; }
  constexpr int kMaxDev = 64;
  static std::atomic<int> cus[kMaxDev];
  int dev = 0;
  if (hipGetDevice(&dev) != hipSuccess || dev < 0 || dev >= kMaxDev) dev = 0;
  int c = cus[dev].load(std::memory_order_relaxed);
  if (c <= 0) {
    int v = 0;
    if (hipDeviceGetAttribute(&v, hipDeviceAttributeMultiprocessorCount, dev) != hipSuccess || v <= 0) v = 256;
    cus[dev].store(c = v, std::memory_order_relaxed);
  }
  return c;
}
extern "C" int ssde_abi_version(void) { return SSDE_ABI_VERSION; }
extern "C" int ssde_sizeof_op(void) { return (int)sizeof(ssde_op); }

typedef float probe_f32x16 __attribute__((ext_vector_type(16)));
__global__ __launch_bounds__(256) void mfma_probe_kernel(int iters, float* sink) {
  probe_f32x16 acc[8];
#pragma unroll
  for (int j = 0; j < 8; ++j)
#pragma unroll
    for (int r = 0; r < 16; ++r) acc[j][r] = 0.f;
  const float a = 1.0f + (float)(threadIdx.x & 7) * 0.125f, b = 0.5f;
  for (int i = 0; i < iters; ++i) {
#pragma unroll
    for (int j = 0; j < 8; ++j) acc[j] = __builtin_amdgcn_mfma_f32_32x32x2f32(a, b, acc[j], 0, 0, 0);
  }
  float t = 0.f;
#pragma unroll
  for (int j = 0; j < 8; ++j) t += acc[j][0];
  if (t == -1.f) sink[threadIdx.x & 63] = t;
}

extern "C" int ssde_mfma_probe(int32_t workgroups, int32_t iters, float* sink, void* stream) {
  SSDE_REQUIRE(workgroups > 0 && iters > 0 && sink, "mfma_probe: bad args");
  hipLaunchKernelGGL(mfma_probe_kernel, dim3(workgroups), dim3(256), 0, static_cast<hipStream_t>(stream), iters, sink);
  SSDE_LAUNCH_CHECK();
  return SSDE_OK;
}

static int run_one(const ssde_op& op, void* stream) {
  switch (op.kind) {
    case SSDE_OP_CONV: return ssde_conv2d(&op.u.conv, stream);
    case SSDE_OP_GN_STATS: return ssde_groupnorm_stats(&op.u.gn, stream);
    case SSDE_OP_UPFIRDN: return ssde_upfirdn2d(&op.u.fir, stream);
    case SSDE_OP_ATTN: return ssde_attention(&op.u.attn, stream);
    case SSDE_OP_EMBED: return ssde_embed(&op.u.embed, stream);
    case SSDE_OP_TO_NHWC: return ssde_to_nhwc(&op.u.to_nhwc, stream);
    case SSDE_OP_TO_NCHW: return ssde_to_nchw(&op.u.to_nchw, stream);
    case SSDE_OP_BIAS_ACT: return ssde_fused_bias_act(&op.u.bias_act, stream);
    case SSDE_OP_SUMSQ: return ssde_sumsq(&op.u.sumsq, stream);
    case SSDE_OP_RANDN: return ssde_randn(&op.u.randn, stream);
    case SSDE_OP_LANGEVIN: return ssde_langevin_update(&op.u.langevin, stream);
    case SSDE_OP_PROJECT: return ssde_project_update(&op.u.project, stream);
    case SSDE_OP_PREDICTOR: return ssde_predictor_update(&op.u.predictor, stream);
    case SSDE_OP_FILL: return ssde_fill_from_table(&op.u.fill, stream);
    case SSDE_OP_STEP_INC: return ssde_step_inc(&op.u.step_inc, stream);
    case SSDE_OP_WGRAD: return ssde_conv_wgrad(&op.u.wgrad, stream);
    case SSDE_OP_COLSUM: return ssde_colsum(&op.u.colsum, stream);
    case SSDE_OP_GN_BWD_REDUCE: return ssde_gn_bwd_reduce(&op.u.gn_bwd, stream);
    case SSDE_OP_PROLOGUE_BWD: return ssde_prologue_bwd(&op.u.pro_bwd, stream);
    case SSDE_OP_ATTN_BWD: return ssde_attention_bwd(&op.u.attn_bwd, stream);
    case SSDE_OP_PERTURB: return ssde_perturb(&op.u.perturb, stream);
    case SSDE_OP_DSM_LOSS: return ssde_dsm_loss(&op.u.dsm_loss, stream);
    case SSDE_OP_SUMSQ_FLAT: return ssde_sumsq_flat(&op.u.sumsq_flat, stream);
    case SSDE_OP_ADAM: return ssde_adam_clip_ema(&op.u.adam, stream);
    case SSDE_OP_MEMSET: return ssde_memset(&op.u.memset, stream);
    case SSDE_OP_AXPY: return ssde_axpy(&op.u.axpy, stream);
    case SSDE_OP_PACK: return ssde_pack_weights(&op.u.pack, stream);
    case SSDE_OP_GN_FINALIZE: return ssde_gn_finalize(&op.u.gn_fin, stream);
    case SSDE_OP_PF_DRIFT: return ssde_pf_drift(&op.u.pf_drift, stream);
    case SSDE_OP_HUTCH_DIV: return ssde_hutch_div(&op.u.hutch_div, stream);
    case SSDE_OP_COLSUM_FINISH: return ssde_colsum_finish(&op.u.colsum_fin, stream);
    case SSDE_OP_GN_BWD_FINISH: return ssde_gn_bwd_finish(&op.u.gn_bwd_fin, stream);
    case SSDE_OP_GN_APPLY: return ssde_gn_apply(&op.u.gn_apply, stream);
    case SSDE_OP_GN_APPLY_BWD: return ssde_gn_apply_bwd(&op.u.gn_apply_bwd, stream);
  }
  ssde_set_error("program: unknown op kind %d", op.kind);
  return SSDE_EINVAL;
}

extern "C" int ssde_program_run(const ssde_op* ops, int32_t n_ops, void* stream) {
  SSDE_REQUIRE(ops && n_ops >= 0, "program: null ops");
  for (int i = 0; i < n_ops; ++i) {
    if (int rc = run_one(ops[i], stream)) {
      char tmp[400];
      strncpy(tmp, g_err, sizeof(tmp) - 1); tmp[sizeof(tmp) - 1] = 0;
      ssde_set_error("op %d (kind %d): %s", i, ops[i].kind, tmp);
      return rc;
    }
  }
  return SSDE_OK;
}

extern "C" int ssde_program_run_timed(const ssde_op* ops, int32_t n_ops, void* stream, float* ms) {
  SSDE_REQUIRE(ops && n_ops >= 0 && ms, "program: null args");
  hipStream_t st = static_cast<hipStream_t>(stream);
  std::vector<hipEvent_t> ev(n_ops + 1);
  for (auto& e : ev) SSDE_HIP_CHECK(hipEventCreate(&e));
  int rc = SSDE_OK;
  SSDE_HIP_CHECK(hipEventRecord(ev[0], st));
  for (int i = 0; i < n_ops && rc == SSDE_OK; ++i) {
    rc = run_one(ops[i], stream);
    if (rc == SSDE_OK && hipEventRecord(ev[i + 1], st) != hipSuccess) { ssde_set_error("hipEventRecord failed"); rc = SSDE_EHIP; }
  }
  if (rc == SSDE_OK) {
    if (hipStreamSynchronize(st) != hipSuccess) { ssde_set_error("hipStreamSynchronize failed"); rc = SSDE_EHIP; }
    for (int i = 0; i < n_ops && rc == SSDE_OK; ++i)
      if (hipEventElapsedTime(&ms[i], ev[i], ev[i + 1]) != hipSuccess) { ssde_set_error("hipEventElapsedTime failed"); rc = SSDE_EHIP; }
  }
  for (auto& e : ev) hipEventDestroy(e);
  return rc;
}

struct SsdeGraph { hipGraph_t graph; hipGraphExec_t exec; };

extern "C" int ssde_graph_capture(const ssde_op* ops, int32_t n_ops, void* stream, void** graph_out) {
  SSDE_REQUIRE(ops && graph_out, "graph: null args");
  hipStream_t st = static_cast<hipStream_t>(stream);
  SSDE_REQUIRE(st != nullptr, "graph: capture needs a non-default stream");
  SSDE_HIP_CHECK(hipStreamBeginCapture(st, hipStreamCaptureModeThreadLocal));
  int rc = ssde_program_run(ops, n_ops, stream);
  hipGraph_t graph = nullptr;
  hipError_t e = hipStreamEndCapture(st, &graph);
  if (rc != SSDE_OK) { if (graph) hipGraphDestroy(graph); return rc; }
  if (e != hipSuccess) { ssde_set_error("hipStreamEndCapture failed: %s", hipGetErrorString(e)); return SSDE_EHIP; }
  hipGraphExec_t exec = nullptr;
  e = hipGraphInstantiate(&exec, graph, nullptr, nullptr, 0);
  if (e != hipSuccess) { hipGraphDestroy(graph); ssde_set_error("hipGraphInstantiate failed: %s", hipGetErrorString(e)); return SSDE_EHIP; }
// ... 21 lines not shown
```

score_sde_pytorch_amd/engine.py:

```python
import ctypes as C
import math
import os
from typing import Callable, NamedTuple

import numpy as np
import torch

from . import _lib as L

_FLT = 4
INV_SQRT2 = float(1.0 / np.sqrt(2.0))

FC_OTHER, FC_CONV3, FC_CONV1, FC_ATTN, FC_GN, FC_FIR = 0, 1, 2, 3, 4, 5

W4P_MIN_BATCH = 16


class Buf:
    __slots__ = ("shape", "numel", "name", "persistent", "tensor", "first", "last")

    def __init__(self, shape, name="", persistent=False):
        self.shape = tuple(int(s) for s in shape)
        self.numel = int(np.prod(self.shape))
        self.name = name
# ... 368 lines not shown
    def __init__(self, device):
        self.device = device
        self.entries = []
        self.meta = {}
        self._tables = None

    def add(self, sources, fn, meta=None, recipe=None):
        lazy = recipe is not None and self._on_device() and os.environ.get("SSDE_TORCH_PACK", "0") != "1"
        with torch.no_grad():
            if lazy:
                try:
                    shape = fn(*[torch.empty(s.shape, dtype=s.dtype, device="meta") for s in sources]).shape
                except Exception:
                    shape = fn(*[torch.zeros(s.shape, dtype=s.dtype) for s in sources]).shape
                packed = torch.zeros(tuple(shape), dtype=torch.float32, device=self.device)
            else:
                packed = fn(*[s.detach() for s in sources]).to(self.device).contiguous()
        self.entries.append(_Entry(packed, list(sources), fn, None if lazy else self._stamp(sources), recipe))
        if meta is not None:
            self.meta[id(packed)] = meta
        self._tables = None
        return packed

    def _on_device(self):
        return self.device.type == "cuda" if isinstance(self.device, torch.device) else str(self.device).startswith("cuda")

    def conv3(self, param, cin_pad=None, cout_pad=None, route=DIRECT):
        def logical(w):
            w = w.to(torch.float32)
            if cin_pad and w.shape[1] < cin_pad:
                w = torch.nn.functional.pad(w, (0, 0, 0, 0, 0, cin_pad - w.shape[1]))
            if cout_pad and w.shape[0] < cout_pad:
                w = torch.nn.functional.pad(w, (0, 0, 0, 0, 0, 0, 0, cout_pad - w.shape[0]))
            return w
        cout_l, cin_l = max(param.shape[0], cout_pad or 0), max(param.shape[1], cin_pad or 0)
        meta = dict(kind="conv3", sources=[param], logical=logical, dims=(cout_l, cin_l),
                    parts=[dict(param=param, row0=0, rows=param.shape[0], transpose=False)], cin_store=param.shape[1])
        recipe = [dict(kind=route.pack_kind, src=param, cout=param.shape[0], cin=param.shape[1], cout_l=cout_l, cin_l=cin_l, flags=0, n="dst")]
        return self.add([param], lambda w: route.pack(logical(w)), meta, recipe)

    def matrix(self, parts, cin_pad=None):
        params = [p for p, _ in parts]

        def logical(*ws):
            ms = []
            for w, (_, tr) in zip(ws, parts):
                w = w.to(torch.float32)
                w = w.t() if tr else w.reshape(w.shape[0], -1)
                ms.append(w)
            m = torch.cat(ms, dim=0) if len(ms) > 1 else ms[0]
            if cin_pad and m.shape[1] < cin_pad:
                m = torch.nn.functional.pad(m, (0, cin_pad - m.shape[1]))
            return m
        rows, desc = 0, []
        for p_, tr in parts:
            n_rows = p_.shape[1] if tr else p_.shape[0]
            cin = p_.shape[0] if tr else int(np.prod(p_.shape[1:]))
            desc.append(dict(param=p_, row0=rows, rows=n_rows, transpose=tr))
            rows += n_rows
        meta = dict(kind="matrix", sources=params, logical=logical, parts=desc, cin_store=cin,
                    dims=(rows, max(cin, cin_pad or 0)))
        recipe = [dict(kind=L.PACK_MATRIX, src=d["param"], cout=d["param"].shape[0], cin=int(np.prod(d["param"].shape[1:])),
                       cout_l=rows, cin_l=0, flags=int(d["transpose"]), r_off=d["row0"], c_off=0, n="src") for d in desc]
        return self.add(params, lambda *ws: pack_matrix(logical(*ws)), meta, recipe)

    def vector(self, params, mode="cat", pad_to=None):
        def fn(*vs):
            vs = [v.to(torch.float32) for v in vs]
            x = torch.cat(vs) if mode == "cat" else sum(vs[1:], vs[0])
            if pad_to and x.numel() < pad_to:
                x = torch.nn.functional.pad(x, (0, pad_to - x.numel()))
            return x.clone()
        off, desc = 0, []
        for p_ in params:
            desc.append(dict(param=p_, off=0 if mode == "sum" else off, n=p_.numel()))
            off += p_.numel()
        if mode == "sum":
            assert len(params) == 2
            recipe = [dict(kind=L.PACK_VECTOR, src=params[0], src2=params[1], r_off=0, n="src")]
        else:
            recipe = [dict(kind=L.PACK_VECTOR, src=d["param"], r_off=d["off"], n="src") for d in desc]
        return self.add(params, fn, dict(kind="vector", mode=mode, sources=list(params), parts=desc), recipe)

    def derived(self, packed, route=None):
        meta = self.meta[id(packed)]
        key = (id(packed), route)
        if key not in self.meta:
            cout_l, cin_l = meta["dims"]
            if meta["kind"] == "conv3":
                p_ = meta["sources"][0]
                fn = lambda w: route.pack(w.permute(1, 0, 2, 3).flip(2, 3))
                recipe = [dict(kind=route.pack_kind, src=p_, cout=p_.shape[0], cin=p_.shape[1],
                               cout_l=cin_l, cin_l=cout_l, flags=1, n="dst")]
            else:
                fn = lambda m: pack_matrix(m.t().contiguous())
                recipe = [dict(kind=L.PACK_MATRIX, src=d["param"], cout=d["param"].shape[0], cin=int(np.prod(d["param"].shape[1:])),
                               cout_l=cin_l, cin_l=0, flags=int(not d["transpose"]), r_off=0, c_off=d["row0"], n="src")
                          for d in meta["parts"]]
            self.meta[key] = self.add(meta["sources"], lambda *ws: fn(meta["logical"](*ws)), None, recipe)
        return self.meta[key]

    def _source_addresses(self):
        return tuple(s.data_ptr() for e in self.entries if e.recipe is not None for s in e.sources)

    def _build_tables(self):
        descs = {}
        for e in self.entries:
            packed, recipe = e.packed, e.recipe
            if recipe is None:
                continue
            for r in recipe:
                d = L.PackDesc()
                src = r["src"]
                d.src, d.dst, d.kind = src.data_ptr(), packed.data_ptr(), r["kind"]
                d.src2 = r["src2"].data_ptr() if r.get("src2") is not None else None
                d.cout, d.cin = r.get("cout", 0), r.get("cin", 0)
                d.cout_l, d.cin_l, d.flags = r.get("cout_l", 0), r.get("cin_l", 0), r.get("flags", 0)
                d.r_off, d.c_off = r.get("r_off", 0), r.get("c_off", 0)
                d.n = packed.numel() if r["n"] == "dst" else src.numel()
                descs.setdefault(r["kind"], []).append(d)
        tables = []
        for kind, ds in sorted(descs.items()):
            arr = (L.PackDesc * len(ds))(*ds)
            raw = torch.frombuffer(bytearray(bytes(arr)), dtype=torch.uint8).to(self.device)
            args = L.PackArgs()
            args.table, args.count, args.kind, args.max_n = raw.data_ptr(), len(ds), kind, max(int(x.n) for x in ds)
            tables.append((args, raw))
        self._tables = (tables, self._source_addresses())

    def pack_tables(self):
        if self._tables is None or self._tables[1] != self._source_addresses():
            self._build_tables()
        return self._tables[0]

    def pack_ops(self):
        return [L.make_op(L.OP_PACK, args) for args, _ in self.pack_tables()]

    def device_refresh(self):
        from . import hipops
        tables = self.pack_tables()
        lib = L.load()
        for args, _ in tables:
            L.check(lib.ssde_pack_weights(C.byref(args), hipops._stream()), "ssde_pack_weights")
        return bool(tables)

    @staticmethod
    def _stamp(sources):
        return tuple((s.data_ptr(), s._version, getattr(getattr(s, "_ssde_flat", None), "generation", 0)) for s in sources)

    def mark_fresh(self):
        for e in self.entries:
            st = self._stamp(e.sources)
            if e.recipe is None and st != e.stamp:
                self._torch_pack(e)
            e.stamp = st

    def _torch_pack(self, e):
        with torch.no_grad():
            e.packed.copy_(e.fn(*[s.detach() for s in e.sources]).to(self.device))

    def refresh(self, force=False, on_device=None):
        if on_device is None:
            on_device = self._on_device()
        stamps = [self._stamp(e.sources) for e in self.entries]
        stale = [force or st != e.stamp for e, st in zip(self.entries, stamps)]
        done_on_device = on_device and any(old and e.recipe is not None for e, old in zip(self.entries, stale)) and self.device_refresh()
        for e, st, old in zip(self.entries, stamps, stale):
            if old and not (done_on_device and e.recipe is not None):
                self._torch_pack(e)
            e.stamp = st


def _src(t, c, t2=None, c2=0, pro=L.PRO_NONE, gn=None, drop=None):
    d = dict(p0=t, p1=t2, c0=c, c1=c2, pro_mode=pro, gn_groups=0, gn_mean=None, gn_rstd=None, gn_gamma=None, gn_beta=None,
             drop_thresh=0, drop_scale=1.0, drop_seed=None, drop_salt=0)
    if gn is not None:
        d.update(gn_groups=gn["groups"], gn_mean=gn["mean"], gn_rstd=gn["rstd"], gn_gamma=gn["gamma"], gn_beta=gn["beta"])
        d["_gn"] = gn
    if drop is not None:
        p, seed_t, salt = drop
        d.update(drop_thresh=min(int(round(p * 2.0 ** 32)), 2 ** 32 - 1), drop_scale=1.0 / (1.0 - p), drop_seed=seed_t,
                 drop_salt=salt & 0xFFFFFFFF)
    return d


_NOSRC = dict(p0=None, p1=None, c0=0, c1=0, pro_mode=0, gn_groups=0, gn_mean=None, gn_rstd=None, gn_gamma=None, gn_beta=None,
              drop_thresh=0, drop_scale=1.0, drop_seed=None, drop_salt=0)


def fir_taps(k, gain=1.0):
    k = np.asarray(k, dtype=np.float32)
    if k.ndim == 1:
        k = np.outer(k, k)
    k = k / np.sum(k)
    return (k * gain).astype(np.float32)


class Lowering:

    def __init__(self, builder, weights, batch):
        self.b, self.w, self.n = builder, weights, batch
        self.parts = {}
# ... 116 lines not shown
                fields["gn_part"] = part
                self.parts[id(dst)] = (part, slices, c_out)
        self.b.add(L.OP_CONV, fields, FC_CONV3 if main is not None else FC_CONV1, flops)

    def _wino4_two_kernels(self, h, w, c_out, c_in):
        return os.environ.get("SSDE_WINO4_TWO", "2") != "0" and wino4_v_floats(self.n, h, w, c_in) * 4 < 2 ** 32 and c_in % 8 == 0

    def _wgrad_takes_wino4(self, f):
        if os.environ.get("SSDE_WINO_V_FROM_FORWARD", "1") == "0":
            return False
        meta = self.w.meta.get(id(f["w_main"]))
        if meta is None or len(meta["parts"]) != 1 or meta["parts"][0]["transpose"]:
            return False
        a = L.WgradArgs()
        s = f["main"]
        a.src.c0, a.src.c1, a.src.pro_mode, a.src.gn_groups = s["c0"], s["c1"], s["pro_mode"], s["gn_groups"]
        a.g_ld, a.g_off = f["c_out"], meta["parts"][0]["row0"]
        a.n, a.h_in, a.w_in, a.h_out, a.w_out = f["n"], f["h_in"], f["w_in"], f["h_out"], f["w_out"]
        a.c_out, a.ksize, a.stride, a.pad = meta["parts"][0]["rows"], 3, f["stride"], f["pad"]
        a.pad_end = f.get("pad_end", 0)
        a.cin_store, a.transpose_out = meta["cin_store"], 0
        a.flags = L.wgrad_route_flags()
        return bool(L.load().ssde_wgrad_wants_winograd4(C.byref(a)))

    def conv3_route(self, h, w, c_out, c_in, aux=False):
        mode = os.environ.get("SSDE_WINOGRAD", "1")
        if mode == "0":
            return DIRECT
        if mode == "1" and h == 4 and w == 4 and not aux and c_in % 32 == 0 and c_out % 64 == 0 and self.n >= W4P_MIN_BATCH:
            return F4P
        legal2 = h % 2 == 0 and w % 2 == 0 and h >= 8 and w >= 8 and c_out >= 32 and c_in >= 8 and c_in % 8 == 0
        legal4 = h % 4 == 0 and w % 4 == 0 and h >= 8 and w >= 8 and c_out >= 32 and c_in >= 8 and c_in % 4 == 0
        two = lambda: self._wino4_two_kernels(h, w, c_out, c_in)
        if mode == "4" and legal4:
            return F4R if two() else F4
        if mode == "2" or mode == "4":
            return F2 if legal2 else DIRECT
        n_tiles = -(-c_out // 64)
        if mode != "3" and legal4 and h >= 16 and w >= 16 and -(-(self.n * h * w) // 512) * n_tiles >= self.cus:
            return F4R if two() else F4
        if mode != "3" and legal4 and c_in % 16 == 0 and c_in >= 256 and c_out % 4 == 0 and os.environ.get("SSDE_CONV_KSPLIT", "1") != "0":
            wgs4 = -(-(-(-(self.n * h * w) // 512)) // 8) * 8 * n_tiles
            if self.cus // 2 < wgs4 * 2 <= self.cus and two():
                return F4R
            if c_in % 32 == 0 and self.cus // 2 < wgs4 * 4 <= self.cus and two():
                return F4R
        return F2 if legal2 and -(-(self.n * h * w) // 256) * n_tiles >= self.cus // 2 else DIRECT

    def upfirdn(self, src, n_ch, h_in, w_in, taps, up=1, down=1, pad=(0, 0), name="fir"):
        kh, kw = taps.shape
        h_out = (h_in * up + pad[0] + pad[1] - kh) // down + 1
        w_out = (w_in * up + pad[0] + pad[1] - kw) // down + 1
        dst = self.b.buf(self.n, h_out, w_out, n_ch, name=name)
        self._materialize_stats(src.get("_gn"))
        self.b.add(L.OP_UPFIRDN, dict(src=src, n=self.n, h_in=h_in, w_in=w_in, c=n_ch, h_out=h_out, w_out=w_out,
                                      up=up, down=down, pad0=pad[0], pad1=pad[1], dst=dst, **self.fir_kernel_fields(taps)), FC_FIR)
        return dst, h_out, w_out

    def fir_kernel_fields(self, taps):
        taps = np.ascontiguousarray(taps, dtype=np.float32)
        kh, kw = taps.shape
        if not (1 <= kh <= L.FIR_MAX_TAPS and 1 <= kw <= L.FIR_MAX_TAPS):
            raise ValueError("upfirdn2d: a %dx%d kernel (fir_kernel of %d taps); at most %d taps per axis"
                             % (kh, kw, max(kh, kw), L.FIR_MAX_TAPS))
        k16, t = [0.0] * 16, None
        if kh <= 4 and kw <= 4:
            k16[:kh * kw] = [float(v) for v in taps.reshape(-1).tolist()]
        else:
            key = (kh, kw, taps.tobytes())
            t = self.b.fir_taps.get(key)
            if t is None:
                t = self.b.fir_taps[key] = self.b.tensor(torch.from_numpy(taps.copy()).to(self.b.device))
        return dict(kh=kh, kw=kw, k=k16, taps=t)


def fir_pads(n_taps, up=False, conv=1):
    p = n_taps - 2 + (conv - 1)
    return ((p + 1) // 2 + (1 if up else 0), p // 2)


class UNetEngine:

    def __init__(self, model, batch, height, width, device, vp_score=False, train=False, input_grad=False,
                 finalize=True):
        L.load()
        self.train, self.input_grad = train, input_grad
        self.model, self.n, self.h, self.w, self.device = model, batch, height, width, device
        cfg = model.config
        self.cfg = cfg
        self.b = ProgramBuilder(device)
        self.weights = WeightStore(device)
        self.low = Lowering(self.b, self.weights, batch)
        self.low.emit_wino_v = bool(getattr(self, "param_grads", False))
        self.channels = model.channels
        self.x_in = self.b.buf(batch, self.channels, height, width, name="x_in", persistent=True)
        self.cond = self.b.buf(batch, name="cond", persistent=True)
        self.sig = self.b.buf(batch, name="sigma", persistent=True) \
            if (model.embedding_type == "positional" and cfg.model.scale_by_sigma) else self.cond
        self.out = self.b.buf(batch, self.channels, height, width, name="out", persistent=True)
        self.vp_score = vp_score
        self.std = self.b.buf(batch, name="std", persistent=True) if vp_score else None
        if vp_score and cfg.model.scale_by_sigma:
            raise NotImplementedError("scale_by_sigma together with a VP score head is not lowered")
        self.drop_seed = None
        if train and float(cfg.model.dropout) > 0:
            self.drop_seed = torch.zeros(1, dtype=torch.int32, device=device)
            self.b.tensor(self.drop_seed)
        self._n_res = 0
        self._emb = self._tproj = None
        self._lower()
        if finalize:
            self.program = self.b.finalize()

    @property
    def cond_only_ops(self):
        return int(self.program.spec_start[getattr(self, "_cond_specs", 0)])

    def _lower(self):
        idx = self._lower_cond()
        body = {"ncsnpp": self._lower_ncsnpp, "ddpm": self._lower_ddpm}[getattr(self.model, "family", "ncsnpp")]
        o, hh, ww = body(idx)
        mode = 2 if self.vp_score else (1 if self.cfg.model.scale_by_sigma else 0)
        vec = self.std if mode == 2 else (self.sig if mode == 1 else None)
        self.b.add(L.OP_TO_NCHW, dict(src=o, dst=self.out, n=self.n, c=self.channels, h=hh, w=ww, c_src=4, mode=mode, v=vec))

    def _lower_cond(self):
        model, b, low, n = self.model, self.b, self.low, self.n
        mods = list(model.all_modules)
        nf = model.nf
        idx = 0
        if not model.conditional and getattr(model, "family", "ncsnpp") == "ddpm":
            self._cond_specs = 0
            self.cond.tensor = torch.zeros((n + 1023) // 1024 * 1024, dtype=torch.float32, device=self.device)
            return idx

        if model.embedding_type == "fourier":
            emb_dim = 2 * nf
            table = self.weights.add([mods[idx].W], lambda w: w.to(torch.float32).clone()); idx += 1
            kind = 0
        else:
            emb_dim = nf
            half = nf // 2
            e = math.log(10000) / (half - 1)
            freqs = torch.exp(torch.arange(half, dtype=torch.float32) * -e)
            table = b.tensor(freqs.to(self.device))
            kind = 1
        emb = b.buf(n, emb_dim, name="emb", persistent=True)
        self._emb = emb
        b.add(L.OP_EMBED, dict(cond=self.cond, w=table, dst=emb, n=n, dim=emb_dim, kind=kind))
        temb = None
        if model.conditional:
            lin0, lin1 = mods[idx], mods[idx + 1]; idx += 2
            t0 = b.buf(n, 4 * nf, name="temb0", persistent=True)
            low.conv(t0, 1, 1, 4 * nf, aux=_src(emb, emb_dim), w_aux=self.weights.matrix([(lin0.weight, False)]),
                     bias=self.weights.vector([lin0.bias]))
            temb = b.buf(n, 4 * nf, name="temb", persistent=True)
            low.conv(temb, 1, 1, 4 * nf, aux=_src(t0, 4 * nf, pro=L.PRO_SILU),
                     w_aux=self.weights.matrix([(lin1.weight, False)]),
                     bias=self.weights.vector([lin1.bias]))
            dense = [m.Dense_0 for m in mods if getattr(m, "kind", "") == "res"]
            self._tproj_off, off = {}, 0
            for d in dense:
                self._tproj_off[id(d)] = off
                off += d.out_features
            self._tproj_ld = off
            wd = self.weights.matrix([(d.weight, False) for d in dense])
            bd = self.weights.vector([d.bias for d in dense])
            self._tproj = b.buf(n, off, name="tproj", persistent=True)
            low.conv(self._tproj, 1, 1, off, aux=_src(temb, 4 * nf, pro=L.PRO_SILU), w_aux=wd, bias=bd)
# ... 157 lines not shown
                up = mods[idx]; idx += 1
                h, hh, ww = low.upfirdn(_src(h, cur_c), cur_c, hh, ww, fir_taps([1, 1], gain=4.0), up=2, pad=(1, 0), name="up")
                if up.with_conv:
                    hn = b.buf(n, hh, ww, cur_c, name="up_conv")
                    route = low.conv3_route(hh, ww, cur_c, cur_c)
                    low.conv(hn, hh, ww, cur_c, main=_src(h, cur_c), w_main=self._w3(up.Conv_0, route=route), h_in=hh, w_in=ww,
                             bias=self._bias(up.Conv_0), route=route, stats=True)
                    h = hn
        assert not hs

        gn_m, conv_m = mods[idx], mods[idx + 1]; idx += 2
        o = self._lower_head(gn_m, conv_m, h, cur_c, hh, ww)
        assert idx == len(mods), (idx, len(mods))
        return o, hh, ww

    def _w3(self, m, cin_pad=None, cout_pad=None, route=DIRECT):
        return self.weights.conv3(m.weight, cin_pad, cout_pad, route=route)

    def _w1(self, m, cin_pad=None):
        return self.weights.matrix([(m.weight, False)], cin_pad=cin_pad)

    def _bias(self, m, pad_to=None):
        return self.weights.vector([m.bias], pad_to=pad_to)

    def _shortcut(self, m):
        conv, nin = getattr(m, "Conv_2", None), getattr(m, "NIN_0", None)
        if conv is not None:
            if tuple(conv.weight.shape[2:]) != (1, 1):
                raise NotImplementedError("ResnetBlockDDPM(conv_shortcut=True): the 3x3 shortcut is not lowered (DDPM never sets it)")
            return self._w1(conv), conv.bias
        if nin is not None:
            return self.weights.matrix([(nin.W, True)]), nin.b
        return None, None

    def _res(self, m, t, c, hh, ww, t2=None, c2=0):
        b, low, n = self.b, self.low, self.n
        cin, cout = c + c2, m.out_ch
        assert cin == m.in_ch, (cin, m.in_ch)
        scale = INV_SQRT2 if m.skip_rescale else 1.0
        gn0 = low.gn_stats(t, c, hh * ww, m.GroupNorm_0, t2, c2)
        chan_add, ld = None, 0
        if hasattr(m, "Dense_0") and self._tproj is not None:
            chan_add, ld = (self._tproj, self._tproj_off[id(m.Dense_0)]), self._tproj_ld
        if m.up or m.down:
            assert t2 is None
            if m.up:
                taps = fir_taps(m.fir_kernel, gain=4.0) if m.fir else fir_taps([1, 1], gain=4.0)
                kw = dict(up=2, pad=fir_pads(taps.shape[0], up=True))
            else:
                taps = fir_taps(m.fir_kernel) if m.fir else fir_taps([1, 1])
                kw = dict(down=2, pad=fir_pads(taps.shape[0]))
            hr, ho, wo = low.upfirdn(low.src(t, c, hh * ww, pro=L.PRO_GN_SILU, gn=gn0), c, hh, ww, taps, name="res_h_rs", **kw)
            xr, _, _ = low.upfirdn(_src(t, c), c, hh, ww, taps, name="res_x_rs", **kw)
            main0, skip_t, skip_c, skip_t2, skip_c2 = _src(hr, c), xr, c, None, 0
            hh, ww = ho, wo
        else:
            main0 = low.src(t, c, hh * ww, t2, c2, pro=L.PRO_GN_SILU, gn=gn0)
            skip_t, skip_c, skip_t2, skip_c2 = t, c, t2, c2
        h1 = b.buf(n, hh, ww, cout, name="res_h1")
        route0 = low.conv3_route(hh, ww, cout, main0["c0"] + main0["c1"])
        w_short, b_short = self._shortcut(m)
        route1 = low.conv3_route(hh, ww, cout, cout, aux=w_short is not None)
        low.conv(h1, hh, ww, cout, main=main0, w_main=self._w3(m.Conv_0, route=route0), h_in=hh, w_in=ww, bias=self._bias(m.Conv_0),
                 chan_add=chan_add, chan_add_ld=ld, route=route0, stats=True)
        gn1 = low.gn_stats(h1, cout, hh * ww, m.GroupNorm_1)
        out = b.buf(n, hh, ww, cout, name="res_out")
        self._n_res += 1
        drop = (float(m.dropout), self.drop_seed, 0x9E3779B1 * self._n_res) if self.drop_seed is not None else None
        main1 = low.src(h1, cout, hh * ww, pro=L.PRO_GN_SILU, gn=gn1, drop=drop)
        if w_short is not None:
            bsum = self.weights.vector([m.Conv_1.bias, b_short], mode="sum")
            low.conv(out, hh, ww, cout, main=main1, w_main=self._w3(m.Conv_1, route=route1), h_in=hh, w_in=ww,
                     aux=low.src(skip_t, skip_c, hh * ww, skip_t2, skip_c2), w_aux=w_short, bias=bsum, scale=scale, route=route1,
                     stats=True)
        else:
            assert skip_t2 is None
            low.conv(out, hh, ww, cout, main=main1, w_main=self._w3(m.Conv_1, route=route1), h_in=hh, w_in=ww,
                     bias=self._bias(m.Conv_1), resid=skip_t, scale=scale, route=route1, stats=True)
        return out, cout

    def _attn(self, m, t, c, hh, ww):
        b, low, n = self.b, self.low, self.n
        gn = low.gn_stats(t, c, hh * ww, m.GroupNorm_0)
        wqkv = self.weights.matrix([(m.NIN_0.W, True), (m.NIN_1.W, True), (m.NIN_2.W, True)])
        bqkv = self.weights.vector([m.NIN_0.b, m.NIN_1.b, m.NIN_2.b])
        qkv = b.buf(n, hh, ww, 3 * c, name="qkv")
        low.conv(qkv, hh, ww, 3 * c, aux=low.src(t, c, hh * ww, pro=L.PRO_GN, gn=gn), w_aux=wqkv, bias=bqkv)
        ao = b.buf(n, hh, ww, c, name="attn_o")
        L_ = hh * ww
        b.add(L.OP_ATTN, dict(qkv=qkv, dst=ao, n=n, l=L_, c=c, scale=float(int(c) ** (-0.5))), FC_ATTN,
              4.0 * n * L_ * L_ * c)
        out = b.buf(n, hh, ww, c, name="attn_out")
        low.conv(out, hh, ww, c, aux=_src(ao, c), w_aux=self.weights.matrix([(m.NIN_3.W, True)]),
                 bias=self.weights.vector([m.NIN_3.b]), resid=t,
                 scale=INV_SQRT2 if m.skip_rescale else 1.0, stats=True)
        return out

    def load_inputs(self, x, cond):
        self.x_in.tensor[: x.numel()].copy_(x.reshape(-1))
        self.cond.tensor[: self.n].copy_(cond.reshape(-1).to(torch.float32))
        if self.sig is not self.cond and self.sig.tensor is not None:
            self.sig.tensor[: self.n].copy_(self.model.sigmas.to(torch.float32)[cond.long()])

    def output_view(self):
        return self.out.tensor[: self.n * self.channels * self.h * self.w].view(self.n, self.channels, self.h, self.w)

    def forward(self, x, cond):
        if tuple(x.shape) != (self.n, self.channels, self.h, self.w):
            raise ValueError("engine built for %s, got %s" % ((self.n, self.channels, self.h, self.w), tuple(x.shape)))
        self.weights.refresh()
        self.load_inputs(x.contiguous(), cond)
        self.program.run()
        return self.output_view().clone()

    def flops_per_forward(self):
        return sum(self.program.flops)

    def validate_plans(self):
        lib = L.load()
        out = []
        for i in range(self.program.n):
            op = self.program.ops[i]
            if op.kind == L.OP_CONV:
                r = lib.ssde_conv_lds_bytes(C.byref(op.u.conv))
                if r < 0:
                    raise L.SsdeError("op %d: %s" % (i, lib.ssde_last_error().decode()))
                out.append(r)
            elif op.kind == L.OP_ATTN:
                if lib.ssde_attention_route(C.byref(op.u.attn)) < 0:
                    raise L.SsdeError("op %d: %s" % (i, lib.ssde_last_error().decode()))
        return out
```

score_sde_pytorch_amd/hipops.py:

```python
import ctypes as C

import numpy as np
import torch

from . import _lib as L
from .engine import F4R, conv3_route_of_tile, pack_conv_weight, pack_matrix, wino4_v_floats


def _stream():
    return C.c_void_p(torch.cuda.current_stream().cuda_stream)


def _need_cuda(*ts):
    for t in ts:
        if t is not None and not t.is_cuda:
            raise RuntimeError("score_sde_pytorch_amd HIP op called with a %s tensor (no CPU fallback)" % t.device.type)


def _p(t):
    return None if t is None else t.data_ptr()


def _fill_src(s, t, t2=None, pro=L.PRO_NONE, gn=None):
    s.p0, s.c0 = _p(t), t.shape[-1]
# ... 69 lines not shown
    keep = []
    route = conv3_route_of_tile(tile)
    if x is not None:
        n, h_in, w_in = x.shape[0], x.shape[1], x.shape[2]
        c_out = weight.shape[0]
        h_out = (h_in + 2 * pad + pad_end - 3) // stride + 1
        w_out = (w_in + 2 * pad + pad_end - 3) // stride + 1
        if out_hw is not None:
            h_out, w_out = out_hw
        _fill_src(a.main, x, x2, pro, gn)
        wp = route.pack(weight.to(x.device)); keep.append(wp)
        if route is F4R:
            wv = torch.empty(wino4_v_floats(n, h_in, w_in, x.shape[-1] + (x2.shape[-1] if x2 is not None else 0)), device=x.device)
            keep.append(wv)
            a.wino_v = _p(wv)
        a.w_main, a.ksize, a.stride, a.pad, a.h_in, a.w_in = _p(wp), 3, stride, pad, h_in, w_in
        a.pad_end = pad_end
    else:
        n, h_out, w_out = aux.shape[0], aux.shape[1], aux.shape[2]
        c_out = aux_weight.shape[0]
        a.ksize, a.stride, a.pad = 0, 1, 0
    if aux is not None:
        _fill_src(a.aux, aux, aux2, aux_pro, aux_gn)
        wa = pack_matrix(aux_weight.to(aux.device)); keep.append(wa)
        a.w_aux = _p(wa)
    dev = (x if x is not None else aux).device
    dst = torch.empty(n, h_out, w_out, c_out, device=dev)
    a.n, a.h_out, a.w_out, a.c_out, a.tile = n, h_out, w_out, c_out, tile
    a.bias = _p(bias)
    if chan_add is not None:
        a.chan_add, a.chan_add_ld = _p(chan_add), chan_add.shape[-1]
    a.resid, a.out_scale, a.dst = _p(resid), scale, _p(dst)
    a.flags = L.conv_route_flags() if flags is None else flags
    if route.needs_ws:
        need = int(L.load().ssde_conv_ws_floats(C.byref(a)))
        L.check(min(need, 0), "ssde_conv_ws_floats")
        ws = torch.empty(need, device=dev); keep.append(ws)
        a.wino_ws, a.wino_ws_floats = _p(ws), need
    L.check(L.load().ssde_conv2d(C.byref(a), _stream()), "ssde_conv2d")
    return dst


def upfirdn2d_nhwc(x, kernel, up=1, down=1, pad=(0, 0), pro=L.PRO_NONE, gn=None, dual=False, accumulate_into=None, flags=0):
    _need_cuda(x)
    n, h, w, c = x.shape
    kh, kw = kernel.shape
    if not (1 <= kh <= L.FIR_MAX_TAPS and 1 <= kw <= L.FIR_MAX_TAPS):
        raise ValueError("upfirdn2d: a %dx%d kernel; at most %d taps per axis" % (kh, kw, L.FIR_MAX_TAPS))
    h_out = (h * up + pad[0] + pad[1] - kh) // down + 1
    w_out = (w * up + pad[0] + pad[1] - kw) // down + 1
    if h_out < 1 or w_out < 1:
        raise ValueError("upfirdn2d: output size %dx%d is not positive" % (h_out, w_out))
    dst = torch.empty(n, h_out, w_out, c, device=x.device) if accumulate_into is None else accumulate_into
    dst2 = torch.empty(n, h_out, w_out, c, device=x.device) if dual else None
    a = L.UpfirdnArgs()
    _fill_src(a.src, x, None, pro, gn)
    a.accumulate = int(accumulate_into is not None)
    a.dst2 = _p(dst2) if dual else None
    a.n, a.h_in, a.w_in, a.c, a.h_out, a.w_out = n, h, w, c, h_out, w_out
    a.up, a.down, a.pad0, a.pad1, a.kh, a.kw, a.flags = up, down, pad[0], pad[1], kh, kw, flags
    taps = None
    if kh <= 4 and kw <= 4:
        for i, v in enumerate(np.asarray(kernel.detach().cpu(), dtype=np.float32).reshape(-1).tolist()):
            a.k[i] = v
    else:
        taps = kernel.detach().to(x.device, torch.float32).contiguous()
        a.taps = _p(taps)
    a.dst = _p(dst)
    L.check(L.load().ssde_upfirdn2d(C.byref(a), _stream()), "ssde_upfirdn2d")
    return (dst, dst2) if dual else dst


def attention(qkv, channels):
    _need_cuda(qkv)
    n, l = qkv.shape[0], qkv.shape[1]
    dst = torch.empty(n, l, channels, device=qkv.device)
    a = L.AttnArgs()
    a.qkv, a.dst, a.n, a.l, a.c, a.scale = _p(qkv), _p(dst), n, l, channels, float(int(channels) ** (-0.5))
    a.flags = L.attn_route_flags()
    L.check(L.load().ssde_attention(C.byref(a), _stream()), "ssde_attention")
    return dst


def attention_route(n, l, channels, flags=None):
    a = L.AttnArgs()
    a.n, a.l, a.c, a.scale = n, l, channels, float(max(int(channels), 1) ** (-0.5))
    a.flags = L.attn_route_flags() if flags is None else flags
    lib = L.load()
    r = lib.ssde_attention_route(C.byref(a))
    if r < 0:
        raise L.SsdeError(lib.ssde_last_error().decode())
    return r


def embed(cond, table, dim, kind):
    _need_cuda(cond, table)
    dst = torch.empty(cond.shape[0], dim, device=cond.device)
    a = L.EmbedArgs()
    a.cond, a.w, a.dst, a.n, a.dim, a.kind = _p(cond), _p(table), _p(dst), cond.shape[0], dim, kind
    L.check(L.load().ssde_embed(C.byref(a), _stream()), "ssde_embed")
    return dst


def to_nhwc(x, c_pad=None, a=1.0, b=0.0):
    _need_cuda(x)
    n, c, h, w = x.shape
    c_pad = c_pad or c
    dst = torch.empty(n, h, w, c_pad, device=x.device)
    args = L.ToNhwcArgs()
    args.src, args.dst, args.n, args.c, args.h, args.w, args.c_pad, args.a, args.b = _p(x), _p(dst), n, c, h, w, c_pad, a, b
    L.check(L.load().ssde_to_nhwc(C.byref(args), _stream()), "ssde_to_nhwc")
    return dst


def to_nchw(x, c=None, mode=0, v=None):
    _need_cuda(x)
    n, h, w, c_src = x.shape
    c = c or c_src
    dst = torch.empty(n, c, h, w, device=x.device)
    args = L.ToNchwArgs()
    args.src, args.dst, args.n, args.c, args.h, args.w, args.c_src, args.mode, args.v = _p(x), _p(dst), n, c, h, w, c_src, mode, _p(v)
    L.check(L.load().ssde_to_nchw(C.byref(args), _stream()), "ssde_to_nchw")
    return dst


def fused_bias_act(x, bias=None, channels=1, inner=1, act=1, alpha=0.2, scale=1.0, grad=0, ref=None):
    _need_cuda(x)
    x = x.contiguous()
    dst = torch.empty_like(x)
    a = L.BiasActArgs()
    a.src, a.bias, a.dst, a.numel, a.channels, a.inner, a.act, a.alpha, a.scale = \
        _p(x), _p(bias), _p(dst), x.numel(), channels, inner, act, alpha, scale
    a.grad, a.ref = grad, _p(ref)
    L.check(L.load().ssde_fused_bias_act(C.byref(a), _stream()), "ssde_fused_bias_act")
    return dst


def randn(numel, seed, device, step_ptr=None, stream_id=0):
    dst = torch.empty(numel, device=device)
    a = L.RandnArgs()
    a.dst, a.numel, a.seed, a.step_ptr, a.stream_id = _p(dst), numel, seed, _p(step_ptr), stream_id
    L.check(L.load().ssde_randn(C.byref(a), _stream()), "ssde_randn")
    return dst


def set_dropout(s, p, seed_t, salt):
    s.drop_thresh = min(int(round(p * 2.0 ** 32)), 2 ** 32 - 1) if p > 0 else 0
    s.drop_scale = 1.0 / (1.0 - p) if p > 0 else 1.0
    s.drop_seed = _p(seed_t) if p > 0 else None
    s.drop_salt = salt & 0xFFFFFFFF


def conv_wgrad(x, g, ksize, dw, stride=1, pad=1, x2=None, pro=L.PRO_NONE, gn=None, g_off=0, c_out=None, cin_store=None,
               transpose_out=False, scale=1.0, splits=0, dropout=None, flags=None, pad_end=0):
    _need_cuda(x, g, dw)
    a = L.WgradArgs()
    a.flags = L.wgrad_route_flags() if flags is None else flags
    _fill_src(a.src, x, x2, pro, gn)
    if dropout is not None:
        set_dropout(a.src, *dropout)
    a.g, a.g_ld, a.g_off = _p(g), g.shape[-1], g_off
    a.n, a.h_in, a.w_in, a.h_out, a.w_out = x.shape[0], x.shape[1], x.shape[2], g.shape[1], g.shape[2]
    a.c_out = c_out if c_out is not None else g.shape[-1] - g_off
    ctot = x.shape[-1] + (x2.shape[-1] if x2 is not None else 0)
    a.ksize, a.stride, a.pad, a.pad_end = ksize, stride, pad, pad_end
    a.cin_store = cin_store if cin_store is not None else ctot
# ... 179 lines not shown
```

score_sde_pytorch_amd/models/ncsnpp.py:

```python
import math

import numpy as np
import torch
import torch.nn as nn

from . import utils


def _fan_avg_uniform_(tensor, scale=1.0, in_axis=1, out_axis=0):
    scale = 1e-10 if scale == 0 else scale
    shape = tensor.shape
    receptive = float(np.prod(shape)) / shape[in_axis] / shape[out_axis]
    fan_in, fan_out = shape[in_axis] * receptive, shape[out_axis] * receptive
    bound = math.sqrt(3.0 * scale / ((fan_in + fan_out) / 2.0))
    with torch.no_grad():
        tensor.copy_((torch.rand(*shape, dtype=tensor.dtype) * 2.0 - 1.0) * bound)
    return tensor


def _conv(in_ch, out_ch, k, init_scale=1.0, stride=1, padding=0):
    m = nn.Conv2d(in_ch, out_ch, kernel_size=k, stride=stride, padding=padding, bias=True)
    _fan_avg_uniform_(m.weight.data, init_scale)
    nn.init.zeros_(m.bias)
    return m
# ... 41 lines not shown


class ResnetBlockBigGANpp(nn.Module):
    kind = "res"

    def __init__(self, in_ch, out_ch=None, temb_dim=None, up=False, down=False, dropout=0.1, fir=False,
                 fir_kernel=(1, 3, 3, 1), skip_rescale=True, init_scale=0.0):
        super().__init__()
        out_ch = out_ch if out_ch else in_ch
        self.GroupNorm_0 = _group_norm(in_ch)
        self.Conv_0 = _conv(in_ch, out_ch, 3, padding=1)
        if temb_dim is not None:
            self.Dense_0 = _dense(temb_dim, out_ch)
        self.GroupNorm_1 = _group_norm(out_ch)
        self.Dropout_0 = nn.Dropout(dropout)
        self.Conv_1 = _conv(out_ch, out_ch, 3, init_scale=init_scale, padding=1)
        if in_ch != out_ch or up or down:
            self.Conv_2 = _conv(in_ch, out_ch, 1)
        self.in_ch, self.out_ch = in_ch, out_ch
        self.up, self.down, self.fir, self.fir_kernel = up, down, fir, tuple(fir_kernel)
        self.skip_rescale = skip_rescale
        self.dropout = dropout


class FirConv2d(nn.Module):

    def __init__(self, in_ch, out_ch):
        super().__init__()
        self.weight = nn.Parameter(_fan_avg_uniform_(torch.empty(out_ch, in_ch, 3, 3), 1.0))
        self.bias = nn.Parameter(torch.zeros(out_ch))


class Downsample(nn.Module):
    kind = "down"

    def __init__(self, in_ch=None, out_ch=None, with_conv=False, fir=False, fir_kernel=(1, 3, 3, 1)):
        super().__init__()
        out_ch = out_ch if out_ch else in_ch
        if with_conv:
            if fir:
                self.Conv2d_0 = FirConv2d(in_ch, out_ch)
            else:
                self.Conv_0 = _conv(in_ch, out_ch, 3, stride=2, padding=0)
        self.in_ch, self.out_ch, self.with_conv, self.fir, self.fir_kernel = in_ch, out_ch, with_conv, fir, tuple(fir_kernel)


class Upsample(nn.Module):
    kind = "up"

    def __init__(self, in_ch=None, out_ch=None, with_conv=False, fir=False, fir_kernel=(1, 3, 3, 1)):
        super().__init__()
        out_ch = out_ch if out_ch else in_ch
        if with_conv:
            if fir:
                raise NotImplementedError("Upsample(with_conv=True, fir=True) is dead code in the reference "
                                          "(upsample_conv_2d raises, models/up_or_down_sampling.py:126)")
            self.Conv_0 = _conv(in_ch, out_ch, 3, padding=1)
        self.in_ch, self.out_ch, self.with_conv, self.fir, self.fir_kernel = in_ch, out_ch, with_conv, fir, tuple(fir_kernel)


class Combine(nn.Module):
    kind = "combine"

    def __init__(self, dim1, dim2, method="cat"):
        super().__init__()
        self.Conv_0 = _conv(dim1, dim2, 1)
        self.method = method


class HipUNet(nn.Module):
    family = "ncsnpp"

    def flat_param_groups(self):
        if not self.conditional:
            return []
        dense = [m.Dense_0 for m in self.all_modules if getattr(m, "kind", "") == "res" and hasattr(m, "Dense_0")]
        return [[d.weight for d in dense], [d.bias for d in dense]] if dense else []

    def _engine_for(self, x):
        from .. import engine as _engine
        key = (x.device.index, x.shape[0], x.shape[2], x.shape[3])
        eng = self._engines.get(key)
        if eng is None:
            eng = _engine.UNetEngine(self, batch=x.shape[0], height=x.shape[2], width=x.shape[3], device=x.device)
            self._engines[key] = eng
        return eng

    def forward(self, x, time_cond):
        name = type(self).__name__
        if not x.is_cuda:
            raise RuntimeError("score_sde_pytorch_amd.%s runs on MI355X through libssde_hip.so only; "
                               "got a %s tensor (there is no CPU fallback)" % (name, x.device.type))
        if x.dtype != torch.float32 or x.dim() != 4:
            raise TypeError("%s.forward expects a float32 [B, C, H, W] tensor" % name)
        needs_grad = torch.is_grad_enabled() and (x.requires_grad or any(p.requires_grad for p in self.parameters()))
        if needs_grad:
            from .. import autograd as _autograd
            return _autograd.unet_apply(self, x, time_cond)
        return self._engine_for(x).forward(x, time_cond)


@utils.register_model(name="ncsnpp")
class NCSNpp(HipUNet):

    def __init__(self, config):
        super().__init__()
        self.config = config
        m = config.model
        if m.nonlinearity.lower() != "swish":
            raise NotImplementedError("the HIP path fuses SiLU; nonlinearity=%r is not built" % m.nonlinearity)
        if m.resblock_type.lower() != "biggan":
            raise NotImplementedError("resblock_type=%r: every shipped ncsnpp config uses 'biggan'" % m.resblock_type)
        self.register_buffer("sigmas", torch.tensor(utils.get_sigmas(config)))
        self.nf = nf = m.nf
        ch_mult = tuple(m.ch_mult)
        self.num_res_blocks = nrb = m.num_res_blocks
        self.attn_resolutions = tuple(m.attn_resolutions)
        self.num_resolutions = nres = len(ch_mult)
        self.all_resolutions = [config.data.image_size // (2 ** i) for i in range(nres)]
        self.conditional = m.conditional
        self.skip_rescale = m.skip_rescale
        self.resblock_type = "biggan"
        self.progressive = m.progressive.lower()
        self.progressive_input = m.progressive_input.lower()
        self.embedding_type = m.embedding_type.lower()
        self.combine_method = m.progressive_combine.lower()
        self.fir, self.fir_kernel = m.fir, tuple(m.fir_kernel)
        if self.progressive not in ("none", "output_skip", "residual"):
            raise ValueError("progressive=%r" % self.progressive)
        if self.progressive_input not in ("none", "input_skip", "residual"):
            raise ValueError("progressive_input=%r" % self.progressive_input)
        if self.embedding_type not in ("fourier", "positional"):
            raise ValueError("embedding type %s unknown." % self.embedding_type)
        if self.progressive == "residual":
            raise NotImplementedError("progressive='residual' needs Upsample(with_conv, fir) which the reference "
                                      "cannot run either (SURVEY F7)")

        mods = []
        add = mods.append
        if self.embedding_type == "fourier":
            if not config.training.continuous:
                raise AssertionError("Fourier features are only used for continuous training.")
            add(GaussianFourierProjection(embedding_size=nf, scale=m.fourier_scale))
            embed_dim = 2 * nf
        else:
            embed_dim = nf
        if self.conditional:
            add(_dense(embed_dim, nf * 4))
            add(_dense(nf * 4, nf * 4))

        def res_block(in_ch, out_ch=None, up=False, down=False):
            return ResnetBlockBigGANpp(in_ch, out_ch, temb_dim=nf * 4 if self.conditional else None, up=up, down=down,
                                       dropout=m.dropout, fir=self.fir, fir_kernel=self.fir_kernel,
                                       skip_rescale=self.skip_rescale, init_scale=m.init_scale)

        def attn_block(ch):
            return AttnBlockpp(ch, skip_rescale=self.skip_rescale, init_scale=m.init_scale)

        channels = config.data.num_channels
        self.channels = channels
        if self.progressive == "output_skip":
            self.pyramid_upsample = Upsample(fir=self.fir, fir_kernel=self.fir_kernel, with_conv=False)
        if self.progressive_input == "input_skip":
            self.pyramid_downsample = Downsample(fir=self.fir, fir_kernel=self.fir_kernel, with_conv=False)

        pyr_ch = channels
        add(_conv(channels, nf, 3, padding=1))
# ... 46 lines not shown
```

score_sde_pytorch_amd/ode.py:

```python
import ctypes as C
import math
import os
import struct

import numpy as np
import torch

from . import _lib as L
from . import engine as E
from . import hipops
from . import sde_lib

_DOP853_C = [0.0, 0.05260015195876773, 0.0789002279381516, 0.1183503419072274, 0.2816496580927726, 0.3333333333333333, 0.25, 0.3076923076923077, 0.6512820512820513, 0.6, 0.8571428571428571, 1.0]
_DOP853_A = [[],
             [0.05260015195876773],
             [0.0197250569845379, 0.0591751709536137],
             [0.02958758547680685, 0.0, 0.08876275643042054],
             [0.2413651341592667, 0.0, -0.8845494793282861, 0.924834003261792],
             [0.037037037037037035, 0.0, 0.0, 0.17082860872947386, 0.12546768756682242],
             [0.037109375, 0.0, 0.0, 0.17025221101954405, 0.06021653898045596, -0.017578125],
             [0.03709200011850479, 0.0, 0.0, 0.17038392571223998, 0.10726203044637328, -0.015319437748624402, 0.008273789163814023],
             [0.6241109587160757, 0.0, 0.0, -3.3608926294469414, -0.868219346841726, 27.59209969944671, 20.154067550477894, -43.48988418106996],
             [0.47766253643826434, 0.0, 0.0, -2.4881146199716677, -0.590290826836843, 21.230051448181193, 15.279233632882423, -33.28821096898486, -0.020331201708508627],
             [-0.9371424300859873, 0.0, 0.0, 5.186372428844064, 1.0914373489967295, -8.149787010746927, -18.52006565999696, 22.739487099350505, 2.4936055526796523, -3.0467644718982196],
# ... 185 lines not shown
        limit = max(1, int(os.environ.get("SSDE_ODE_RHS_CACHE", "4")))
    cache = model.__dict__.setdefault("_ode_rhs", {})
    rhs = cache.pop(key, None)
    fresh = rhs is None
    if fresh:
        rhs = make()
    cache[key] = rhs
    kind = key[0] if isinstance(key, tuple) and key else None
    same = [k for k in cache if (k[0] if isinstance(k, tuple) and k else None) == kind]
    for k in same[:max(0, len(same) - limit)]:
        cache.pop(k)
    return rhs, fresh


class _FusedRhs:
    writes_out = True
    _RING = 32

    def _init_dyn(self, device):
        self.device = torch.device(device)
        self.dyn = torch.zeros(24, dtype=torch.uint8, device=self.device)
        on_gpu = self.device.type == "cuda"
        self._ring = E.PinnedRing(self._RING if on_gpu else 1, 24, torch.uint8, pinned=on_gpu)
        self.use_graph = on_gpu and os.environ.get("SSDE_ODE_GRAPH", "1") != "0"
        self.graph_stream = torch.cuda.Stream(device=self.device) if self.use_graph else None
        self.nfev = 0
        self.last_path = None

    def _scalars(self, t):
        sde = self.sde
        tv = torch.full((1,), float(t), dtype=torch.float32)
        one = torch.ones(1, 1, 1, 1)
        drift1, diffusion = sde.sde(one, tv)
        std = sde.marginal_prob(torch.zeros(1, 1, 1, 1), tv)[1]
        label = tv * 999 if self.vp_like else std
        eng = self.unet
        second = float(std)
        if eng.sig is not eng.cond:
            second = float(eng.model.sigmas[int(label.reshape(-1)[0])])
        return float(label), second, float(drift1.reshape(-1)[0]), float((diffusion ** 2).reshape(-1)[0])

    def _upload(self, t, out):
        record = np.frombuffer(struct.pack("<ffffQ", *self._scalars(t), out.data_ptr()), dtype=np.uint8)

        def write(h):
            h.numpy()[:] = record
        self._ring.upload(self.dyn, write)

    def _head_ops(self):
        eng, n = self.unet, self.shape[0]
        p = self.dyn.data_ptr()
        ops = [L.make(L.OP_FILL, dst=eng.cond.tensor, tab=p, step_ptr=None, n=n)]
        if eng.sig is not eng.cond:
            ops.append(L.make(L.OP_FILL, dst=eng.sig.tensor, tab=p + 4, step_ptr=None, n=n))
        if self.vp_like:
            ops.append(L.make(L.OP_FILL, dst=eng.std.tensor, tab=p + 4, step_ptr=None, n=n))
        return ops

    def __call__(self, t, y, out):
        self.unet.weights.refresh()
        self._upload(t, out)
        if self.use_graph:
            cur = torch.cuda.current_stream()
            self.program.replay_from_current(cur if cur.cuda_stream != 0 else self.graph_stream)
            self.last_path = "graph"
        else:
            self.program.run()
            self.last_path = "eager"
        self.nfev += 1

    @staticmethod
    def applies(model, sde, x):
        from .models.ncsnpp import HipUNet
        if not isinstance(model, HipUNet) or not x.is_cuda or type(sde) not in (sde_lib.VESDE, sde_lib.VPSDE, sde_lib.subVPSDE):
            return False
        return not (type(sde) is not sde_lib.VESDE and model.config.model.scale_by_sigma)


class FusedDrift(_FusedRhs):

    def __init__(self, model, sde, shape, device):
        self.sde, self.shape = sde, tuple(shape)
        self.vp_like = isinstance(sde, (sde_lib.VPSDE, sde_lib.subVPSDE))
        self.unet = E.UNetEngine(model, shape[0], shape[2], shape[3], device, vp_score=self.vp_like)
        self.n = int(torch.tensor(self.shape).prod())
        self.x32, self.n32 = self.unet.x_in.tensor[: self.n], self.n
        self._init_dyn(device)
        drift = L.make(L.OP_PF_DRIFT, x=self.x32, score=self.unet.out.tensor, dst=None, numel=self.n, a=0.0, g2=0.0, dyn=self.dyn)
        self.program = E.Program.of([self._head_ops(), self.unet.program, drift], self)


class FusedLikelihoodRhs(_FusedRhs):

    def __init__(self, model, sde, shape, probe, device):
        from . import backward as B
        self.sde, self.shape = sde, tuple(shape)
        self.vp_like = isinstance(sde, (sde_lib.VPSDE, sde_lib.subVPSDE))
        eng = self.unet = B.TrainEngine(model, shape[0], shape[2], shape[3], device, vp_score=self.vp_like, input_grad=True,
                                        dropout=False, param_grads=False)
        self.n = int(torch.tensor(self.shape).prod())
        self.per = self.n // self.shape[0]
        self.x32, self.n32 = eng.x_in.tensor[: self.n], self.n
        self.eps = probe.detach().to(device=device, dtype=torch.float32).reshape(-1).contiguous()
        eng.gout.tensor[: self.n].copy_(self.eps)
        self._init_dyn(device)
        drift = L.make(L.OP_PF_DRIFT, x=self.x32, score=eng.out.tensor, dst=None, numel=self.n, a=0.0, g2=0.0, dyn=self.dyn)
        div = L.make(L.OP_HUTCH_DIV, gx=eng.gx.tensor, eps=self.eps, dst=None, dst_off=self.n, n=self.shape[0], per=self.per,
                     a=0.0, g2=0.0, dyn=self.dyn)
        self.program = E.Program.of([self._head_ops(), eng.program[:eng.n_fwd], drift, eng.program[eng.n_fwd:], div], self)

    def set_probe(self, probe):
        self.eps.copy_(probe.detach().to(self.eps.device, torch.float32).reshape(-1))
        self.unet.gout.tensor[: self.n].copy_(self.eps)


def scalars_fn(rhs):
    return rhs._scalars


def solve_host(fun, t_span, y0, rtol=1e-5, atol=1e-5, method="RK45"):
    from scipy import integrate
    dev = y0.device

    def rhs(t, y_np):
        y = torch.from_numpy(np.ascontiguousarray(y_np)).to(dev)
        return fun(float(t), y).detach().to("cpu", torch.float64).numpy()
    sol = integrate.solve_ivp(rhs, (float(t_span[0]), float(t_span[1])), y0.detach().to("cpu", torch.float64).numpy().reshape(-1),
                              rtol=rtol, atol=atol, method=method)
    return torch.from_numpy(sol.y[:, -1].copy()).to(dev), int(sol.nfev)


last_driver = None


def integrate_ode(fun, t_span, y0, rtol, atol, method):
    global last_driver
    if method in TABLEAUS and y0.is_cuda and os.environ.get("SSDE_HOST_ODE", "0") != "1":
        last_driver = "device"
        rows = TABLEAUS[method]["n_stages"] + 1
        side = getattr(fun, "graph_stream", None)
        if side is None:
            stages = _HipStages(y0.numel(), y0, x32=getattr(fun, "x32", None), n32=getattr(fun, "n32", 0), rows=rows)
            return solve_rk(fun, t_span, y0, rtol=rtol, atol=atol, method=method, stages=stages)
        side.wait_stream(torch.cuda.current_stream())
        with torch.cuda.stream(side):
            stages = _HipStages(y0.numel(), y0, x32=getattr(fun, "x32", None), n32=getattr(fun, "n32", 0), rows=rows)
            res = solve_rk(fun, t_span, y0, rtol=rtol, atol=atol, method=method, stages=stages)
        torch.cuda.current_stream().wait_stream(side)
        return res
    last_driver = "host"
    if getattr(fun, "writes_out", False):
        inner = fun

        def fun(t, y):
            inner.x32.copy_(y.to(torch.float32))
            out = torch.empty_like(y)
            inner(t, y, out=out)
            return out
    return solve_host(fun, t_span, y0, rtol=rtol, atol=atol, method=method)
```

score_sde_pytorch_amd/pc_engine.py:

```python
import os

import numpy as np
import torch

from . import _lib as L
from . import engine as E
from . import sde_lib


def plan_fused(sde, predictor, corrector, model, continuous, x, probability_flow=False):
    from . import sampling as S
    from .models.ncsnpp import HipUNet
    if not isinstance(model, HipUNet) or not x.is_cuda:
        return None
    if type(sde) not in (sde_lib.VESDE, sde_lib.VPSDE, sde_lib.subVPSDE):
        return None
    pred = {None: "none", S.NonePredictor: "none", S.ReverseDiffusionPredictor: "reverse_diffusion",
            S.EulerMaruyamaPredictor: "euler_maruyama", S.AncestralSamplingPredictor: "ancestral_sampling"}.get(predictor, "?")
    corr = {None: "none", S.NoneCorrector: "none", S.LangevinCorrector: "langevin",
            S.AnnealedLangevinDynamics: "ald"}.get(corrector, "?")
    if pred == "?" or corr == "?":
        return None
    if corr in ("langevin", "ald") and type(sde) is sde_lib.subVPSDE:
        return None
    if pred == "ancestral_sampling" and (type(sde) is sde_lib.subVPSDE or probability_flow):
        return None
    vp_like = type(sde) in (sde_lib.VPSDE, sde_lib.subVPSDE)
    if vp_like and model.config.model.scale_by_sigma:
        return None
    return dict(predictor=pred, corrector=corr, vp_like=vp_like, continuous=continuous)


def step_tables(sde, plan, eps, probability_flow):
    N = sde.N
    ts = torch.linspace(sde.T, eps, N)
    zeros = torch.zeros(N, 1, 1, 1)
    ones = torch.ones(N, 1, 1, 1)
    tabs = {"t": ts}
    if plan["vp_like"]:
        if plan["continuous"] or type(sde) is sde_lib.subVPSDE:
            tabs["label"] = ts * 999
            tabs["std"] = sde.marginal_prob(zeros, ts)[1]
        else:
            lab = ts * (N - 1)
            tabs["label"] = lab
            tabs["std"] = sde.sqrt_1m_alphas_cumprod[lab.long()]
    else:
        if plan["continuous"]:
            tabs["label"] = sde.marginal_prob(zeros, ts)[1]
        else:
            tabs["label"] = torch.round((sde.T - ts) * (N - 1)).long().float()
    half = 0.5 if probability_flow else 1.0
    if plan["predictor"] == "reverse_diffusion":
        f, G = sde.discretize(ones, ts)
        f_coef = f[:, 0, 0, 0]
        a = 1.0 - f_coef
        b = G ** 2 * half
        c = torch.zeros_like(G) if probability_flow else G
        tabs["coef"] = torch.stack([a, b, c], dim=1)
    elif plan["predictor"] == "euler_maruyama":
        dt = -1. / N
        drift, diffusion = sde.sde(ones, ts)
        d_coef = drift[:, 0, 0, 0]
        a = 1.0 + d_coef * dt
        b = -(diffusion ** 2) * half * dt
        c = torch.zeros_like(diffusion) if probability_flow else diffusion * np.sqrt(-dt)
        tabs["coef"] = torch.stack([a, b, c], dim=1)
    elif plan["predictor"] == "ancestral_sampling":
        idx = (ts * (N - 1) / sde.T).long()
        if plan["vp_like"]:
            beta = sde.discrete_betas[idx]
            a = 1.0 / torch.sqrt(1. - beta)
            b = beta / torch.sqrt(1. - beta)
            c = torch.sqrt(beta)
        else:
            sigma = sde.discrete_sigmas[idx]
            adj = torch.where(idx == 0, torch.zeros_like(ts), sde.discrete_sigmas[idx - 1])
            a = torch.ones_like(sigma)
            b = sigma ** 2 - adj ** 2
            c = torch.sqrt((adj ** 2 * (sigma ** 2 - adj ** 2)) / (sigma ** 2))
        tabs["coef"] = torch.stack([a, b, c], dim=1)
    if plan["corrector"] in ("langevin", "ald") and plan["vp_like"]:
        tabs["alpha"] = sde.alphas[(ts * (N - 1) / sde.T).long()]
    if plan["corrector"] == "ald":
        tabs["ald_std2"] = sde.marginal_prob(zeros, ts)[1] ** 2
        tabs["ald_one"] = torch.ones(N)
    return {k: v.to(torch.float32).contiguous() for k, v in tabs.items()}


class FusedPCSampler:
    def __init__(self, model, sde, plan, shape, snr, n_steps, probability_flow, eps, device, projection=None):
        if n_steps > 8:
            raise NotImplementedError("fused PC sampler supports n_steps <= 8 corrector steps")
        self.model, self.sde, self.plan, self.shape = model, sde, plan, tuple(shape)
        self.n_steps, self.device = n_steps, device
        B, Cc, H, W = self.shape
        self.unet = E.UNetEngine(model, B, H, W, device, vp_score=plan["vp_like"])
        tabs = step_tables(sde, plan, eps, probability_flow)
        self.tabs = {k: v.to(device) for k, v in tabs.items()}
        per = Cc * H * W
        self.x = self.unet.x_in.tensor[: B * per]
        self.x_mean = torch.zeros(B * per, device=device)
        self.z_c = torch.zeros(B * per, device=device)
        self.z_p = torch.zeros(B * per, device=device)
        self.gss = torch.zeros(B, device=device)
        self.zss = torch.zeros(B, device=device)
        self.step = torch.zeros(1, dtype=torch.int32, device=device)
        self.seed_word = torch.zeros(1, dtype=torch.int64, device=device)
        self.snr, self.B, self.per = float(snr), B, per
        self.projection = projection
        if projection is not None:
            ts = tabs["t"]
            mean1, std = sde.marginal_prob(torch.ones(sde.N, 1, 1, 1), ts)
            self.tabs["proj"] = torch.stack([mean1.reshape(-1), std], dim=1).to(torch.float32).contiguous().to(device)
            self.proj_data = torch.zeros(B * per, device=device)
            self.proj_mask = torch.zeros(B * per, device=device)
            self.z_pc = torch.zeros(B * per, device=device)
            self.z_pp = torch.zeros(B * per, device=device)
        self._programs = {}
        self.last_path = None
        self._stream = None

    def _assemble(self, with_rng):
        parts = []

        def emit(kind, **fields):
            parts.append(L.make(kind, **fields))

        def emit_projection(noise, stream_id):
            pj = self.projection
            if pj is None:
                return
            if with_rng:
                emit(L.OP_RANDN, dst=noise, numel=self.B * self.per, seed=0, seed_ptr=self.seed_word, step_ptr=self.step, stream_id=stream_id)
            Cc = self.shape[1]
            emit(L.OP_PROJECT, x=self.x, x_mean=self.x_mean, data=self.proj_data, mask=self.proj_mask, noise=noise,
                 coef=self.tabs["proj"], step_ptr=self.step, n=self.B, c=Cc, hw=self.per // Cc,
                 use_matrix=int(pj.get("M") is not None), M=list(pj.get("M") or [0.0] * 9), invM=list(pj.get("invM") or [0.0] * 9))

        share = os.environ.get("SSDE_PC_SHARE_COND", "0") == "1"
        n_cond = self.unet.cond_only_ops if share else 0
        unet = self.unet.program

        def emit_unet():
            parts.append(unet[n_cond:] if any(p is unet for p in parts) else unet)

        score = self.unet.out.tensor
        emit(L.OP_FILL, dst=self.unet.cond.tensor, tab=self.tabs["label"], step_ptr=self.step, n=self.B)
        if self.plan["vp_like"]:
            emit(L.OP_FILL, dst=self.unet.std.tensor, tab=self.tabs["std"], step_ptr=self.step, n=self.B)
        if self.plan["corrector"] == "ald":
            emit(L.OP_FILL, dst=self.gss, tab=self.tabs["ald_one"], step_ptr=self.step, n=self.B)
            emit(L.OP_FILL, dst=self.zss, tab=self.tabs["ald_std2"], step_ptr=self.step, n=self.B)
        if self.plan["corrector"] in ("langevin", "ald"):
            for k in range(self.n_steps):
                emit_unet()
                if with_rng:
                    emit(L.OP_RANDN, dst=self.z_c, numel=self.B * self.per, seed=0, seed_ptr=self.seed_word, step_ptr=self.step, stream_id=k)
                if self.plan["corrector"] == "langevin":
                    emit(L.OP_SUMSQ, a=score, b=self.z_c, out_a=self.gss, out_b=self.zss, n=self.B, per=self.per)
                emit(L.OP_LANGEVIN, x=self.x, x_mean=self.x_mean, grad=score, noise=self.z_c,
                     grad_sumsq=self.gss, noise_sumsq=self.zss, alpha_tab=self.tabs.get("alpha"), step_ptr=self.step,
                     n=self.B, per=self.per, snr=self.snr)
        emit_projection(self.z_pc if self.projection is not None else None, 9)
        if self.plan["predictor"] != "none":
            emit_unet()
            if with_rng:
                emit(L.OP_RANDN, dst=self.z_p, numel=self.B * self.per, seed=0, seed_ptr=self.seed_word, step_ptr=self.step, stream_id=8)
            emit(L.OP_PREDICTOR, x=self.x, x_mean=self.x_mean, score=score, noise=self.z_p,
                 coef=self.tabs["coef"], step_ptr=self.step, numel=self.B * self.per)
        emit_projection(self.z_pp if self.projection is not None else None, 10)
        emit(L.OP_STEP_INC, step_ptr=self.step, delta=1)
        return E.Program.of(parts, self)

    def step_program(self, with_rng=True):
        if with_rng not in self._programs:
            self._programs[with_rng] = self._assemble(with_rng)
        return self._programs[with_rng]

    def set_seed(self, seed=None):
# ... 50 lines not shown
```

Baseline: 5.739 images/s.

## Fold attention output projection into value weights and fuse residual epilogue

Precomputes W_v·W_out products (and the matching bias) at weight-pack time so the value projection already includes the NIN_3 output projection. The attention kernel then writes its result through a fused epilogue that adds bias and residual, applies the skip rescale, and emits GroupNorm partial statistics. This removes the separate output-projection GEMM and an intermediate buffer round-trip per attention block. In exchange it adds new packing kernels, the epilogue costs extra LDS staging, and folding the weights changes the rounding order.

```diff
diff --git a/include/ssde.h b/include/ssde.h
--- a/include/ssde.h
+++ b/include/ssde.h
@@ -144,6 +144,16 @@
   uint32_t flags;
   int32_t _pad0;
 } ssde_attn_args;
+typedef struct ssde_attn_fused_args {
+  const float* qkv; float* dst;
+  int32_t n, l, c; float scale;
+  uint32_t flags;
+  int32_t gn_slices;
+  const float* resid;
+  const float* bias;
+  float* gn_part;
+  float out_scale; int32_t _pad1;
+} ssde_attn_fused_args;
 enum { SSDE_ATTNF_BF16X6 = 1u,
        SSDE_ATTNF_STREAM = 2u };
 enum { SSDE_ATTN_ROUTE_F32 = 0, SSDE_ATTN_ROUTE_X6 = 1, SSDE_ATTN_ROUTE_STREAM = 2 };
@@ -334,7 +344,9 @@
 enum { SSDE_PACK_CONV3 = 1, SSDE_PACK_WINO3 = 2, SSDE_PACK_MATRIX = 3, SSDE_PACK_VECTOR = 4,
        SSDE_PACK_WINO4 = 5 ,
        SSDE_PACK_WINO4R = 6 ,
-       SSDE_PACK_WINO4P = 7  };
+       SSDE_PACK_WINO4P = 7 ,
+       SSDE_PACK_MATMUL = 8 ,
+       SSDE_PACK_VECMAT = 9  };
 typedef struct ssde_pack_desc {
   const float* src;
   const float* src2;
@@ -394,6 +406,8 @@
 int64_t ssde_conv_ws_floats(const ssde_conv_args* a);
 int ssde_upfirdn2d(const ssde_upfirdn_args* a, void* stream);
 int ssde_attention(const ssde_attn_args* a, void* stream);
+int ssde_attention_fused(const ssde_attn_fused_args* a, void* stream);
+int ssde_attention_fused_route(const ssde_attn_fused_args* a);
 int ssde_attention_route(const ssde_attn_args* a);
 int ssde_embed(const ssde_embed_args* a, void* stream);
 int ssde_to_nhwc(const ssde_to_nhwc_args* a, void* stream);
@@ -454,7 +468,8 @@
     ssde_pack_args pack; ssde_project_args project; ssde_gn_finalize_args gn_fin;
     ssde_pf_drift_args pf_drift; ssde_hutch_div_args hutch_div;
     ssde_colsum_finish_args colsum_fin; ssde_gn_bwd_finish_args gn_bwd_fin;
-    ssde_gn_apply_args gn_apply; ssde_gn_apply_bwd_args gn_apply_bwd;
+    ssde_gn_apply_args gn_apply; ssde_gn_apply_bwd_args gn_apply_bwd; 
+    ssde_attn_fused_args attn_fused;
   } u;
 } ssde_op;
 
diff --git a/score_sde_pytorch_amd/_lib.py b/score_sde_pytorch_amd/_lib.py
--- a/score_sde_pytorch_amd/_lib.py
+++ b/score_sde_pytorch_amd/_lib.py
@@ -24,6 +24,7 @@
 FINISH_JOBS = 16
 COLSUMF_DEFER = 1
 PACK_CONV3, PACK_WINO3, PACK_MATRIX, PACK_VECTOR, PACK_WINO4, PACK_WINO4R, PACK_WINO4P = 1, 2, 3, 4, 5, 6, 7
+PACK_MATMUL, PACK_VECMAT = 8, 9
 
 _fp = C.c_void_p
 
@@ -112,7 +113,8 @@
 
 class AttnArgs(C.Structure):
     _fields_ = [("qkv", _fp), ("dst", _fp), ("n", C.c_int32), ("l", C.c_int32), ("c", C.c_int32), ("scale", C.c_float),
-                ("flags", C.c_uint32), ("_pad0", C.c_int32)]
+                ("flags", C.c_uint32), ("gn_slices", C.c_int32), ("resid", _fp), ("bias", _fp), ("gn_part", _fp),
+                ("out_scale", C.c_float), ("_pad1", C.c_int32)]
 
 
 class EmbedArgs(C.Structure):
@@ -291,7 +293,7 @@
 _UNION_FIELD = {kind: member for kind, member, _, _ in OPS}
 ARGS = {kind: args for kind, _, args, _ in OPS}
 
-EXPORTS = ["ssde_conv2d", "ssde_groupnorm_stats", "ssde_upfirdn2d", "ssde_attention", "ssde_attention_route", "ssde_embed", "ssde_to_nhwc",
+EXPORTS = ["ssde_conv2d", "ssde_groupnorm_stats", "ssde_upfirdn2d", "ssde_attention", "ssde_attention_route", "ssde_attention_fused", "ssde_attention_fused_route", "ssde_embed", "ssde_to_nhwc",
            "ssde_to_nchw", "ssde_fused_bias_act", "ssde_sumsq", "ssde_randn", "ssde_langevin_update",
            "ssde_predictor_update", "ssde_fill_from_table", "ssde_step_inc", "ssde_program_run",
            "ssde_program_run_timed", "ssde_graph_capture", "ssde_graph_launch", "ssde_graph_destroy",
@@ -345,6 +347,16 @@
     return x6 | (ATTNF_STREAM if e.get("SSDE_ATTN_STREAM", "0") == "1" else 0)
 
 
+def attn_fused_slices(n, l, c, flags=None):
+    a = AttnArgs()
+    a.n, a.l, a.c, a.resid = n, l, c, 0x1000
+    a.flags = attn_route_flags() if flags is None else flags
+    r = load().ssde_attention_fused_route(C.byref(a))
+    if r < 0:
+        return 0
+    return -(-l // 64) * (8 if r == ATTN_ROUTE_X6 else 4)
+
+
 def wgrad_route_flags(env=None):
     e = os.environ if env is None else env
     f = {"0": WGRADF_DIRECT, "2": WGRADF_F2, "44": WGRADF_F4_FORCE}.get(e.get("SSDE_WGRAD_WINOGRAD", ""), 0)
@@ -388,6 +400,8 @@
     lib.ssde_sample_update.argtypes = [C.POINTER(SampleUpdateArgs), C.c_void_p]
     lib.ssde_conv_lds_bytes.argtypes = [C.POINTER(ConvArgs)]
     lib.ssde_attention_route.argtypes = [C.POINTER(AttnArgs)]
+    lib.ssde_attention_fused_route.argtypes = [C.POINTER(AttnArgs)]
+    lib.ssde_attention_fused.argtypes = [C.POINTER(AttnArgs), C.c_void_p]
     lib.ssde_conv_gn_slices.argtypes = [C.POINTER(ConvArgs)]
     lib.ssde_conv_ws_floats.argtypes = [C.POINTER(ConvArgs)]
     lib.ssde_conv_ws_floats.restype = C.c_int64
diff --git a/score_sde_pytorch_amd/csrc/attention.hip b/score_sde_pytorch_amd/csrc/attention.hip
--- a/score_sde_pytorch_amd/csrc/attention.hip
+++ b/score_sde_pytorch_amd/csrc/attention.hip
@@ -237,8 +237,22 @@
   for (int j = threadIdx.x & 3; j < L; j += 4) prow[j] *= inv;
 }
 
+struct AttnEpi { const float* resid; const float* bias; float* gn_part; float out_scale; };
+
+template <int NCOLS, int NT>
+__device__ __forceinline__ void attn_store_tile(float* tile, const AttnEpi& ep, float* __restrict__ dst, int n, int q0, int L, int C,
+                                                int blocks_per_img) {
+  const SsdeEpi e{ep.bias, nullptr, 0, ep.resid, 0, ep.out_scale, dst, C, ep.gn_part};
+  ssde_store_tile<kQB, NCOLS, NT>(tile, kLDP, 0, e, [&](int row, size_t& pix, int& img) {
+    if (q0 + row >= L) return false;
+    pix = (size_t)n * L + q0 + row;
+    img = n;
+    return true;
+  }, ep.gn_part ? n * blocks_per_img + q0 / kQB : -1);
+}
+
 __global__ __launch_bounds__(256) void attn_kernel(const float* __restrict__ qkv, float* __restrict__ dst,
-                                                   int N, int L, int C, float scale) {
+                                                   int N, int L, int C, float scale, const AttnEpi ep) {
   SSDE_LDS(smem);
   float* Qs = smem;
   float* Ks = smem + kQB * kLDC;
@@ -257,7 +271,16 @@
   __syncthreads();
   float m, l;
   softmax_rows(Ps, L, m, l);
-  gemm_pv<kFwdVch>(Ps, Lp, base + 2 * C, L, C3, C, Vs, dst + ((size_t)n * L + q0) * C, C, L - q0, 1.0f);
+  if (!ep.resid) {
+    gemm_pv<kFwdVch>(Ps, Lp, base + 2 * C, L, C3, C, Vs, dst + ((size_t)n * L + q0) * C, C, L - q0, 1.0f);
+    return;
+  }
+  zero_acc(acc);
+  pv_pass<kFwdVch>(Ps, Lp, base + 2 * C, L, C3, 0, C, Vs, acc);
+  __syncthreads();
+  acc_to_tile(acc, Ps, C, 1.0f);
+  __syncthreads();
+  attn_store_tile<256, 256>(Ps, ep, dst, n, q0, L, C, gridDim.x);
 }
 
 namespace x6 {
@@ -277,7 +300,8 @@
 }
 
 template <int kNst>
-__global__ __launch_bounds__(x6::kT) void attn_x6_kernel(const float* __restrict__ qkv, float* __restrict__ dst, int N, float scale) {
+__global__ __launch_bounds__(x6::kT) void attn_x6_kernel(const float* __restrict__ qkv, float* __restrict__ dst, int N, float scale,
+                                                         const AttnEpi ep) {
   using namespace x6;
   constexpr int C = 16 * kNst;
   SSDE_LDS(smem);
@@ -512,17 +536,17 @@
       SSDE_LDS_BARRIER();
     }
     if (w_on) {
-#pragma unroll
-      for (int b = 0; b < 2; ++b) {
-        float* out = dst + ((size_t)n * kL + q0) * C + wave * 64 + b * 32 + li;
+      float* out = ep.resid ? smem + wave * 64 + li : dst + ((size_t)n * kL + q0) * C + wave * 64 + li;
+      const size_t ldo = ep.resid ? (size_t)kLDP : (size_t)C;
+#pragma unroll
+      for (int b = 0; b < 2; ++b)
 #pragma unroll
         for (int a = 0; a < 2; ++a)
 #pragma unroll
           for (int r = 0; r < 16; ++r) {
             const int row = a * 32 + (r & 3) + 8 * (r >> 2) + 4 * lh;
-            out[(size_t)row * C] = acc[a][b][r];
+            out[(size_t)row * ldo + b * 32] = acc[a][b][r];
           }
-      }
     }
   } else {
     park_v(R[0], stage0);
@@ -544,6 +568,10 @@
     }
   }
 #undef SSDE_X6_WAIT
+  if (ep.resid) {
+    SSDE_LDS_BARRIER();
+    attn_store_tile<(C == 192 ? 256 : C), kT>(smem, ep, dst, n, q0, kL, C, kL / kRows);
+  }
 }
 
 
@@ -840,24 +868,21 @@
 
 }
 
-static int attn_route(const ssde_attn_args* a) {
+static int attn_route(const ssde_attn_args* a, bool fused) {
   SSDE_REQUIRE(a, "attention: null args");
   if (int rc = check_shape("attention", a->n, a->l, a->c)) return rc;
   if (a->l > kLMax || (a->flags & SSDE_ATTNF_STREAM)) {
+    SSDE_REQUIRE(!fused, "attention: the streaming kernels (more than %d tokens, or SSDE_ATTNF_STREAM) have no fused epilogue", kLMax);
     SSDE_REQUIRE(a->c <= kStreamCMax, "attention: the streaming kernels (more than %d tokens, or SSDE_ATTNF_STREAM) take at most %d channels (got %d)",
                  kLMax, kStreamCMax, a->c);
     return SSDE_ATTN_ROUTE_STREAM;
   }
+  SSDE_REQUIRE(!fused || a->c <= 256, "attention: the fused epilogue takes at most 256 channels (got %d)", a->c);
   if ((a->flags & SSDE_ATTNF_BF16X6) && a->l == x6::kL && a->c <= 256 && a->c % 64 == 0) return SSDE_ATTN_ROUTE_X6;
   return SSDE_ATTN_ROUTE_F32;
 }
 
-extern "C" int ssde_attention_route(const ssde_attn_args* a) { return attn_route(a); }
-
-extern "C" int ssde_attention(const ssde_attn_args* a, void* stream) {
-  SSDE_REQUIRE(a && a->qkv && a->dst, "attention: null args");
-  const int route = attn_route(a);
-  if (route < 0) return route;
+static int attn_launch(const ssde_attn_args* a, int route, const AttnEpi& ep, void* stream) {
   hipStream_t st = static_cast<hipStream_t>(stream);
   const dim3 grid(ssde_cdiv(a->l, kQB), a->n);
   if (route == SSDE_ATTN_ROUTE_STREAM) {
@@ -867,13 +892,43 @@
   if (route == SSDE_ATTN_ROUTE_X6) {
     const dim3 grid_x6(ssde_cdiv(a->n, 8) * 8 * 4);
     switch (a->c) {
-      case 64: return ssde_launch_lds<attn_x6_kernel<4>>("attention", grid_x6, x6::kT, x6::kLds, st, a->qkv, a->dst, a->n, a->scale);
-      case 128: return ssde_launch_lds<attn_x6_kernel<8>>("attention", grid_x6, x6::kT, x6::kLds, st, a->qkv, a->dst, a->n, a->scale);
-      case 192: return ssde_launch_lds<attn_x6_kernel<12>>("attention", grid_x6, x6::kT, x6::kLds, st, a->qkv, a->dst, a->n, a->scale);
-      default: return ssde_launch_lds<attn_x6_kernel<16>>("attention", grid_x6, x6::kT, x6::kLds, st, a->qkv, a->dst, a->n, a->scale);
-    }
-  }
-  return ssde_launch_lds<attn_kernel>("attention", grid, 256, kAttnLdsFloats * 4, st, a->qkv, a->dst, a->n, a->l, a->c, a->scale);
+      case 64: return ssde_launch_lds<attn_x6_kernel<4>>("attention", grid_x6, x6::kT, x6::kLds, st, a->qkv, a->dst, a->n, a->scale, ep);
+      case 128: return ssde_launch_lds<attn_x6_kernel<8>>("attention", grid_x6, x6::kT, x6::kLds, st, a->qkv, a->dst, a->n, a->scale, ep);
+      case 192: return ssde_launch_lds<attn_x6_kernel<12>>("attention", grid_x6, x6::kT, x6::kLds, st, a->qkv, a->dst, a->n, a->scale, ep);
+      default: return ssde_launch_lds<attn_x6_kernel<16>>("attention", grid_x6, x6::kT, x6::kLds, st, a->qkv, a->dst, a->n, a->scale, ep);
+    }
+  }
+  return ssde_launch_lds<attn_kernel>("attention", grid, 256, kAttnLdsFloats * 4, st, a->qkv, a->dst, a->n, a->l, a->c, a->scale, ep);
+}
+
+extern "C" int ssde_attention_route(const ssde_attn_args* a) { return attn_route(a, false); }
+
+extern "C" int ssde_attention(const ssde_attn_args* a, void* stream) {
+  SSDE_REQUIRE(a && a->qkv && a->dst, "attention: null args");
+  const int route = attn_route(a, false);
+  if (route < 0) return route;
+  return attn_launch(a, route, AttnEpi{nullptr, nullptr, nullptr, 1.0f}, stream);
+}
+
+static ssde_attn_args attn_core(const ssde_attn_fused_args* a) { return ssde_attn_args{a->qkv, a->dst, a->n, a->l, a->c, a->scale, a->flags, 0}; }
+
+extern "C" int ssde_attention_fused_route(const ssde_attn_fused_args* a) {
+  SSDE_REQUIRE(a && a->resid, "attention(fused): the residual is missing");
+  const ssde_attn_args core = attn_core(a);
+  const int route = attn_route(&core, true);
+  if (route < 0) return route;
+  const int slices = route == SSDE_ATTN_ROUTE_X6 ? (x6::kL / x6::kRows) * (x6::kT / 64) : ssde_cdiv(a->l, kQB) * 4;
+  SSDE_REQUIRE(!a->gn_part || a->gn_slices == slices, "attention(fused): this launch writes %d GroupNorm slices per image (gn_slices %d)", slices,
+               a->gn_slices);
+  return route;
+}
+
+extern "C" int ssde_attention_fused(const ssde_attn_fused_args* a, void* stream) {
+  SSDE_REQUIRE(a && a->qkv && a->dst, "attention(fused): null args");
+  const int route = ssde_attention_fused_route(a);
+  if (route < 0) return route;
+  const ssde_attn_args core = attn_core(a);
+  return attn_launch(&core, route, AttnEpi{a->resid, a->bias, a->gn_part, a->out_scale}, stream);
 }
 
 extern "C" int ssde_attention_bwd(const ssde_attn_bwd_args* a, void* stream) {
diff --git a/score_sde_pytorch_amd/csrc/backward.hip b/score_sde_pytorch_amd/csrc/backward.hip
--- a/score_sde_pytorch_amd/csrc/backward.hip
+++ b/score_sde_pytorch_amd/csrc/backward.hip
@@ -925,6 +925,31 @@
     d.dst[d.r_off + idx] = d.src[idx] + (d.src2 ? d.src2[idx] : 0.f);
 }
 
+__device__ __forceinline__ float pack_dot(const ssde_pack_desc& d, const float* a, size_t a_step, int j) {
+  const float* b = d.src2 + ((d.flags & 2) ? (size_t)j * d.cin_l : (size_t)j);
+  const size_t b_step = (d.flags & 2) ? 1 : (size_t)d.cin;
+  double acc = 0.0;
+  for (int k = 0; k < d.cin_l; ++k) acc += (double)a[k * a_step] * (double)b[k * b_step];
+  return (float)acc;
+}
+
+__global__ __launch_bounds__(256) void pack_matmul_kernel(const ssde_pack_desc* __restrict__ table) {
+  const ssde_pack_desc d = table[blockIdx.y];
+  const int ld = (d.cout_l + 63) / 64 * 64;
+  for (size_t idx = (size_t)blockIdx.x * 256 + threadIdx.x; idx < (size_t)d.n; idx += (size_t)gridDim.x * 256) {
+    const int i = (int)(idx / d.cin), j = (int)(idx % d.cin);
+    const float v = (d.flags & 1) ? pack_dot(d, d.src + i, (size_t)d.cout, j) : pack_dot(d, d.src + (size_t)i * d.cin_l, 1, j);
+    const int row = i + d.r_off, col = j + d.c_off;
+    d.dst[((size_t)(col >> 3) * ld + row) * 8 + (col & 7)] = v;
+  }
+}
+
+__global__ __launch_bounds__(256) void pack_vecmat_kernel(const ssde_pack_desc* __restrict__ table) {
+  const ssde_pack_desc d = table[blockIdx.y];
+  for (size_t idx = (size_t)blockIdx.x * 256 + threadIdx.x; idx < (size_t)d.n; idx += (size_t)gridDim.x * 256)
+    d.dst[d.r_off + idx] = pack_dot(d, d.src, 1, (int)idx);
+}
+
 }
 
 extern "C" int ssde_pack_weights(const ssde_pack_args* a, void* stream) {
@@ -941,6 +966,8 @@
     case SSDE_PACK_WINO4P: hipLaunchKernelGGL(pack_wino4_kernel<2>, grid, dim3(256), 0, st, a->table); break;
     case SSDE_PACK_MATRIX: hipLaunchKernelGGL(pack_matrix_kernel, grid, dim3(256), 0, st, a->table); break;
     case SSDE_PACK_VECTOR: hipLaunchKernelGGL(pack_vector_kernel, grid, dim3(256), 0, st, a->table); break;
+    case SSDE_PACK_MATMUL: hipLaunchKernelGGL(pack_matmul_kernel, grid, dim3(256), 0, st, a->table); break;
+    case SSDE_PACK_VECMAT: hipLaunchKernelGGL(pack_vecmat_kernel, grid, dim3(256), 0, st, a->table); break;
     default: ssde_set_error("pack_weights: unknown kind %d", a->kind); return SSDE_EINVAL;
   }
   SSDE_LAUNCH_CHECK();
diff --git a/score_sde_pytorch_amd/csrc/runtime.hip b/score_sde_pytorch_amd/csrc/runtime.hip
--- a/score_sde_pytorch_amd/csrc/runtime.hip
+++ b/score_sde_pytorch_amd/csrc/runtime.hip
@@ -60,7 +60,7 @@
     case SSDE_OP_CONV: return ssde_conv2d(&op.u.conv, stream);
     case SSDE_OP_GN_STATS: return ssde_groupnorm_stats(&op.u.gn, stream);
     case SSDE_OP_UPFIRDN: return ssde_upfirdn2d(&op.u.fir, stream);
-    case SSDE_OP_ATTN: return ssde_attention(&op.u.attn, stream);
+    case SSDE_OP_ATTN: return op.u.attn_fused.resid ? ssde_attention_fused(&op.u.attn_fused, stream) : ssde_attention(&op.u.attn, stream);
     case SSDE_OP_EMBED: return ssde_embed(&op.u.embed, stream);
     case SSDE_OP_TO_NHWC: return ssde_to_nhwc(&op.u.to_nhwc, stream);
     case SSDE_OP_TO_NCHW: return ssde_to_nchw(&op.u.to_nchw, stream);
diff --git a/score_sde_pytorch_amd/engine.py b/score_sde_pytorch_amd/engine.py
--- a/score_sde_pytorch_amd/engine.py
+++ b/score_sde_pytorch_amd/engine.py
@@ -474,6 +474,64 @@
             recipe = [dict(kind=L.PACK_VECTOR, src=d["param"], r_off=d["off"], n="src") for d in desc]
         return self.add(params, fn, dict(kind="vector", mode=mode, sources=list(params), parts=desc), recipe)
 
+    def matrix_with_products(self, parts):
+        def op(w, tr):
+            w = w.to(torch.float64)
+            return w.t() if tr else w
+
+        def logical(*ws):
+            ws, ms = list(ws), []
+            for part in parts:
+                if len(part) == 2:
+                    ms.append(op(ws.pop(0), part[1]).to(torch.float32))
+                else:
+                    ms.append((op(ws.pop(0), part[1]) @ op(ws.pop(0), part[3])).to(torch.float32))
+            return torch.cat(ms, dim=0)
+        params, recipe, rows = [], [], 0
+        total = sum((p[0].shape[1] if p[1] else p[0].shape[0]) for p in parts)
+        for part in parts:
+            if len(part) == 2:
+                p_, tr = part
+                n_rows = p_.shape[1] if tr else p_.shape[0]
+                params.append(p_)
+                recipe.append(dict(kind=L.PACK_MATRIX, src=p_, cout=p_.shape[0], cin=p_.shape[1], cout_l=total, cin_l=0, flags=int(tr),
+                                   r_off=rows, c_off=0, n="src"))
+            else:
+                a, ta, b_, tb = part
+                n_rows, inner = (a.shape[1], a.shape[0]) if ta else (a.shape[0], a.shape[1])
+                cols = b_.shape[0] if tb else b_.shape[1]
+                assert inner == (b_.shape[1] if tb else b_.shape[0])
+                params += [a, b_]
+                recipe.append(dict(kind=L.PACK_MATMUL, src=a, src2=b_, cout=n_rows, cin=cols, cout_l=total, cin_l=inner,
+                                   flags=int(ta) | 2 * int(tb), r_off=rows, c_off=0, n=n_rows * cols))
+            rows += n_rows
+        return self.add(params, lambda *ws: pack_matrix(logical(*ws)), None, recipe)
+
+    def vector_with_products(self, parts):
+        def fn(*vs):
+            vs, out = list(vs), []
+            for part in parts:
+                if isinstance(part, tuple):
+                    v, m = vs.pop(0).to(torch.float64), vs.pop(0).to(torch.float64)
+                    out.append((v @ (m.t() if part[2] else m)).to(torch.float32))
+                else:
+                    out.append(vs.pop(0).to(torch.float32))
+            return torch.cat(out)
+        params, recipe, off = [], [], 0
+        for part in parts:
+            if isinstance(part, tuple):
+                v, m, tb = part
+                cols = m.shape[0] if tb else m.shape[1]
+                assert v.numel() == (m.shape[1] if tb else m.shape[0])
+                params += [v, m]
+                recipe.append(dict(kind=L.PACK_VECMAT, src=v, src2=m, cin=cols, cin_l=v.numel(), flags=2 * int(tb), r_off=off, n=cols))
+            else:
+                cols = part.numel()
+                params.append(part)
+                recipe.append(dict(kind=L.PACK_VECTOR, src=part, r_off=off, n="src"))
+            off += cols
+        return self.add(params, fn, None, recipe)
+
     def derived(self, packed, route=None):
         meta = self.meta[id(packed)]
         key = (id(packed), route)
@@ -509,7 +567,7 @@
                 d.cout, d.cin = r.get("cout", 0), r.get("cin", 0)
                 d.cout_l, d.cin_l, d.flags = r.get("cout_l", 0), r.get("cin_l", 0), r.get("flags", 0)
                 d.r_off, d.c_off = r.get("r_off", 0), r.get("c_off", 0)
-                d.n = packed.numel() if r["n"] == "dst" else src.numel()
+                d.n = packed.numel() if r["n"] == "dst" else src.numel() if r["n"] == "src" else r["n"]
                 descs.setdefault(r["kind"], []).append(d)
         tables = []
         for kind, ds in sorted(descs.items()):
@@ -792,9 +850,10 @@
 class UNetEngine:
 
     def __init__(self, model, batch, height, width, device, vp_score=False, train=False, input_grad=False,
-                 finalize=True):
+                 finalize=True, fold_attn=False):
         L.load()
         self.train, self.input_grad = train, input_grad
+        self.fold_attn = fold_attn and not train and not input_grad and os.environ.get("SSDE_ATTN_FOLD", "1") != "0"
         self.model, self.n, self.h, self.w, self.device = model, batch, height, width, device
         cfg = model.config
         self.cfg = cfg
@@ -1118,18 +1177,33 @@
     def _attn(self, m, t, c, hh, ww):
         b, low, n = self.b, self.low, self.n
         gn = low.gn_stats(t, c, hh * ww, m.GroupNorm_0)
+        L_ = hh * ww
+        qkv = b.buf(n, hh, ww, 3 * c, name="qkv")
+        attn = dict(qkv=qkv, n=n, l=L_, c=c, scale=float(int(c) ** (-0.5)))
+        out_scale = INV_SQRT2 if m.skip_rescale else 1.0
+        flags = L.attn_route_flags()
+        slices = L.attn_fused_slices(n, L_, c, flags) if self.fold_attn else 0
+        if slices > 0:
+            wqkv = self.weights.matrix_with_products([(m.NIN_0.W, True), (m.NIN_1.W, True), (m.NIN_3.W, True, m.NIN_2.W, True)])
+            bqkv = self.weights.vector_with_products([m.NIN_0.b, m.NIN_1.b, (m.NIN_2.b, m.NIN_3.W, False)])
+            low.conv(qkv, hh, ww, 3 * c, aux=low.src(t, c, hh * ww, pro=L.PRO_GN, gn=gn), w_aux=wqkv, bias=bqkv)
+            out = b.buf(n, hh, ww, c, name="attn_out")
+            part = None
+            if os.environ.get("SSDE_GN_FUSE", "1") != "0":
+                part = b.buf(n, slices, c // 4, 3, name="gn_part")
+                low.parts[id(out)] = (part, slices, c)
+            b.add(L.OP_ATTN, dict(attn, dst=out, resid=t, bias=self.weights.vector([m.NIN_3.b]), out_scale=float(out_scale),
+                                  gn_part=part, gn_slices=slices if part is not None else 0, flags=flags), FC_ATTN,
+                  4.0 * n * L_ * L_ * c)
+            return out
         wqkv = self.weights.matrix([(m.NIN_0.W, True), (m.NIN_1.W, True), (m.NIN_2.W, True)])
         bqkv = self.weights.vector([m.NIN_0.b, m.NIN_1.b, m.NIN_2.b])
-        qkv = b.buf(n, hh, ww, 3 * c, name="qkv")
         low.conv(qkv, hh, ww, 3 * c, aux=low.src(t, c, hh * ww, pro=L.PRO_GN, gn=gn), w_aux=wqkv, bias=bqkv)
         ao = b.buf(n, hh, ww, c, name="attn_o")
-        L_ = hh * ww
-        b.add(L.OP_ATTN, dict(qkv=qkv, dst=ao, n=n, l=L_, c=c, scale=float(int(c) ** (-0.5))), FC_ATTN,
-              4.0 * n * L_ * L_ * c)
+        b.add(L.OP_ATTN, dict(attn, dst=ao), FC_ATTN, 4.0 * n * L_ * L_ * c)
         out = b.buf(n, hh, ww, c, name="attn_out")
         low.conv(out, hh, ww, c, aux=_src(ao, c), w_aux=self.weights.matrix([(m.NIN_3.W, True)]),
-                 bias=self.weights.vector([m.NIN_3.b]), resid=t,
-                 scale=INV_SQRT2 if m.skip_rescale else 1.0, stats=True)
+                 bias=self.weights.vector([m.NIN_3.b]), resid=t, scale=out_scale, stats=True)
         return out
 
     def load_inputs(self, x, cond):
@@ -1163,6 +1237,7 @@
                     raise L.SsdeError("op %d: %s" % (i, lib.ssde_last_error().decode()))
                 out.append(r)
             elif op.kind == L.OP_ATTN:
-                if lib.ssde_attention_route(C.byref(op.u.attn)) < 0:
+                query = lib.ssde_attention_fused_route if op.u.attn.resid else lib.ssde_attention_route
+                if query(C.byref(op.u.attn)) < 0:
                     raise L.SsdeError("op %d: %s" % (i, lib.ssde_last_error().decode()))
         return out
diff --git a/score_sde_pytorch_amd/hipops.py b/score_sde_pytorch_amd/hipops.py
--- a/score_sde_pytorch_amd/hipops.py
+++ b/score_sde_pytorch_amd/hipops.py
@@ -175,6 +175,22 @@
     return dst
 
 
+def attention_fused(qkv, channels, resid, bias=None, out_scale=1.0, flags=None):
+    _need_cuda(qkv, resid)
+    n, l = qkv.shape[0], qkv.shape[1]
+    flags = L.attn_route_flags() if flags is None else flags
+    slices = L.attn_fused_slices(n, l, channels, flags)
+    if slices <= 0:
+        raise L.SsdeError(L.load().ssde_last_error().decode())
+    dst = torch.empty(n, l, channels, device=qkv.device)
+    part = torch.empty(n, slices, channels // 4, 3, device=qkv.device)
+    a = L.AttnArgs()
+    a.qkv, a.dst, a.n, a.l, a.c, a.scale = _p(qkv), _p(dst), n, l, channels, float(int(channels) ** (-0.5))
+    a.resid, a.bias, a.out_scale, a.gn_part, a.gn_slices, a.flags = _p(resid), _p(bias), float(out_scale), _p(part), slices, flags
+    L.check(L.load().ssde_attention_fused(C.byref(a), _stream()), "ssde_attention_fused")
+    return dst, part
+
+
 def attention_route(n, l, channels, flags=None):
     a = L.AttnArgs()
     a.n, a.l, a.c, a.scale = n, l, channels, float(max(int(channels), 1) ** (-0.5))
diff --git a/score_sde_pytorch_amd/models/ncsnpp.py b/score_sde_pytorch_amd/models/ncsnpp.py
--- a/score_sde_pytorch_amd/models/ncsnpp.py
+++ b/score_sde_pytorch_amd/models/ncsnpp.py
@@ -147,7 +147,7 @@
         key = (x.device.index, x.shape[0], x.shape[2], x.shape[3])
         eng = self._engines.get(key)
         if eng is None:
-            eng = _engine.UNetEngine(self, batch=x.shape[0], height=x.shape[2], width=x.shape[3], device=x.device)
+            eng = _engine.UNetEngine(self, batch=x.shape[0], height=x.shape[2], width=x.shape[3], device=x.device, fold_attn=True)
             self._engines[key] = eng
         return eng
 
diff --git a/score_sde_pytorch_amd/ode.py b/score_sde_pytorch_amd/ode.py
--- a/score_sde_pytorch_amd/ode.py
+++ b/score_sde_pytorch_amd/ode.py
@@ -291,7 +291,7 @@
     def __init__(self, model, sde, shape, device):
         self.sde, self.shape = sde, tuple(shape)
         self.vp_like = isinstance(sde, (sde_lib.VPSDE, sde_lib.subVPSDE))
-        self.unet = E.UNetEngine(model, shape[0], shape[2], shape[3], device, vp_score=self.vp_like)
+        self.unet = E.UNetEngine(model, shape[0], shape[2], shape[3], device, vp_score=self.vp_like, fold_attn=True)
         self.n = int(torch.tensor(self.shape).prod())
         self.x32, self.n32 = self.unet.x_in.tensor[: self.n], self.n
         self._init_dyn(device)
diff --git a/score_sde_pytorch_amd/pc_engine.py b/score_sde_pytorch_amd/pc_engine.py
--- a/score_sde_pytorch_amd/pc_engine.py
+++ b/score_sde_pytorch_amd/pc_engine.py
@@ -95,7 +95,7 @@
         self.model, self.sde, self.plan, self.shape = model, sde, plan, tuple(shape)
         self.n_steps, self.device = n_steps, device
         B, Cc, H, W = self.shape
-        self.unet = E.UNetEngine(model, B, H, W, device, vp_score=plan["vp_like"])
+        self.unet = E.UNetEngine(model, B, H, W, device, vp_score=plan["vp_like"], fold_attn=True)
         tabs = step_tables(sde, plan, eps, probability_flow)
         self.tabs = {k: v.to(device) for k, v in tabs.items()}
         per = Cc * H * W
```

New measurement: 5.822 images/s, median of 6. 1.01x the previous value.
